# thanhndv212/figaroh-plus

Measured on AMD Instinct MI355X. Metric: samples/sec regressor build + TSQR solve, UR10 6-DoF, higher is better.
Workload: dtype f64

## Files before the change

### figaroh_plus_amd/_lib.py

```python
from __future__ import annotations

import ctypes as C
import os

import numpy as np

_HERE = os.path.dirname(os.path.abspath(__file__))
LIB_PATH = os.environ.get("FIGH_LIB_PATH") or os.path.join(_HERE, "libfigh.so")

ABI_VERSION = 113

FIGH_OK = 0
ERR_INVALID, ERR_NO_DEVICE, ERR_ALLOC, ERR_UNSUPPORTED, ERR_COMM = -1, -2, -3, -4, -5

MODE_JOINT_TORQUE, MODE_EXT_WRENCH = 0, 1
FLAG_FRICTION, FLAG_ACT_INERTIA, FLAG_OFFSET, FLAG_TX40, FLAG_GENERIC, FLAG_BLOCKED_INPUTS = 1, 2, 4, 8, 256, 512
FLAG_COMPACT_BLOCKS = 2048
FLAG_FORCE_COMPACT = 8192
FLAG_LINK_COMPACT = 4096
FLAG_ZEROS_PRESENT = 1024

_c_double_p = C.POINTER(C.c_double)
_c_int32_p = C.POINTER(C.c_int32)

SIGNATURES = {
    "figh_version": (C.c_int, []),
    "figh_last_error": (C.c_char_p, []),
    "figh_device_count": (C.c_int, [C.POINTER(C.c_int)]),
    "figh_device_set": (C.c_int, [C.c_int]),
    "figh_host_wait_mode": (C.c_int, [C.c_int]),
    "figh_tsqr_null_pivot_tol": (C.c_int, [C.c_double]),
    "figh_device_pci_bus_id": (C.c_int, [C.c_int, C.c_char_p, C.c_int]),
    "figh_device_info": (C.c_int, [C.c_char_p, C.c_int, C.POINTER(C.c_int), C.POINTER(C.c_size_t)]),
    "figh_malloc": (C.c_int, [C.POINTER(C.c_void_p), C.c_size_t]),
    "figh_free": (C.c_int, [C.c_void_p]),
    "figh_memcpy_h2d": (C.c_int, [C.c_void_p, C.c_void_p, C.c_size_t]),
    "figh_memcpy_d2h": (C.c_int, [C.c_void_p, C.c_void_p, C.c_size_t]),
    "figh_host_alloc": (C.c_int, [C.POINTER(C.c_void_p), C.c_size_t]),
    "figh_host_free": (C.c_int, [C.c_void_p]),
    "figh_memcpy_d2d": (C.c_int, [C.c_void_p, C.c_void_p, C.c_size_t]),
    "figh_memset": (C.c_int, [C.c_void_p, C.c_int, C.c_size_t]),
    "figh_synchronize": (C.c_int, []),
    "figh_profile_enable": (C.c_int, [C.c_int]),
    "figh_profile_reset": (C.c_int, []),
    "figh_profile_get": (C.c_int, [C.c_char_p, C.POINTER(C.c_int), _c_double_p]),
    "figh_model_create": (C.c_int, [C.c_int, _c_int32_p, _c_int32_p, _c_double_p, _c_double_p, _c_int32_p,
                                    _c_int32_p, _c_double_p, _c_int32_p, C.POINTER(C.c_void_p)]),
    "figh_model_destroy": (C.c_int, [C.c_void_p]),
    "figh_regressor_shape": (C.c_int, [C.c_void_p, C.c_int, C.c_int, C.POINTER(C.c_int), C.POINTER(C.c_int)]),
    "figh_regressor_build": (C.c_int, [C.c_void_p, C.c_int, C.c_int, C.c_int, C.c_int64, C.c_void_p, C.c_void_p,
                                       C.c_void_p, C.c_void_p, C.c_int64, C.c_void_p]),
    "figh_regressor_build_padded": (C.c_int, [C.c_void_p, C.c_int, C.c_int, C.c_int, C.c_int64, C.c_void_p, C.c_void_p,
                                              C.c_void_p, C.c_void_p, C.c_int64, C.c_void_p]),
    "figh_regressor_apply": (C.c_int, [C.c_void_p, C.c_int, C.c_int, C.c_int, C.c_int64, C.c_void_p, C.c_void_p, C.c_void_p,
                                       C.c_void_p, C.c_void_p]),
    "figh_repack_samples": (C.c_int, [C.c_void_p, C.c_int64, C.c_int, C.c_void_p]),
    "figh_coupling_tx40": (C.c_int, [C.c_int64, C.c_int, C.c_void_p, C.c_void_p, C.c_void_p]),
    "figh_colsq": (C.c_int, [C.c_void_p, C.c_int64, C.c_int, C.c_int64, C.c_void_p]),
    "figh_gather_cols": (C.c_int, [C.c_void_p, C.c_int64, C.c_int64, C.c_void_p, C.c_int, C.c_void_p, C.c_int64]),
    "figh_place_block": (C.c_int, [C.c_void_p, C.c_int64, C.c_int64, C.c_int64, C.c_double, C.c_void_p, C.c_int64]),
    "figh_matvec": (C.c_int, [C.c_void_p, C.c_int64, C.c_int64, C.c_void_p, C.c_int, C.c_void_p, C.c_void_p]),
    "figh_block_sqnorm": (C.c_int, [C.c_void_p, C.c_void_p, C.c_int64, C.c_int, C.c_void_p]),
    "figh_tsqr": (C.c_int, [C.c_void_p, C.c_int64, C.c_int64, C.c_void_p, C.c_int, C.c_void_p, _c_double_p, C.c_int,
                            C.c_void_p]),
    "figh_tsqr_structured": (C.c_int, [C.c_void_p, C.c_int64, C.c_int64, C.c_void_p, C.c_int, C.c_void_p, _c_double_p,
                                       C.c_int, _c_int32_p, C.c_int, C.c_void_p]),
    "figh_tsqr_merge": (C.c_int, [C.c_void_p, C.c_int, C.c_int, C.c_void_p]),
    "figh_select_columns": (C.c_int, [C.c_void_p, C.c_int, C.c_double, C.c_int, C.c_void_p]),
    "figh_tsqr_selected_wrench": (C.c_int, [C.c_void_p, C.c_int64, C.c_int64, C.c_void_p, C.c_int, C.c_double, C.c_int,
                                            C.c_int, C.c_int, C.c_void_p, C.c_double, C.c_void_p, C.c_void_p, C.c_void_p,
                                            C.c_int64]),
    "figh_regressor_force_layout": (C.c_int, [C.c_void_p, C.c_int, C.c_int, C.c_int, C.POINTER(C.c_int64)]),
    "figh_model_set_active_rows": (C.c_int, [C.c_void_p, _c_int32_p, C.c_int]),
    "figh_regressor_link_layout": (C.c_int, [C.c_void_p, C.c_int, C.c_int, C.c_int, _c_int32_p, C.POINTER(C.c_int)]),
    "figh_tsqr_selected_blocks": (C.c_int, [C.c_void_p, C.c_int64, C.c_int64, C.c_void_p, C.c_int, C.c_double, C.c_int,
                                            C.c_int, C.c_int, C.c_void_p, C.c_void_p, C.c_void_p, C.c_void_p, C.c_void_p,
                                            C.c_void_p, C.c_double, C.c_void_p, C.c_void_p, C.c_void_p]),
    "figh_block_rows_residuals": (C.c_int, [C.c_void_p, C.c_int, _c_int32_p, C.c_int, C.c_void_p, C.c_void_p]),
    "figh_tsqr_selected": (C.c_int, [C.c_void_p, C.c_int64, C.c_int64, C.c_void_p, C.c_int, C.c_double, C.c_int, C.c_int,
                                     C.c_int, C.c_void_p, C.c_double, C.c_void_p, C.c_void_p]),
    "figh_regressor_tsqr_fused": (C.c_int, [C.c_void_p, C.c_int, C.c_int64, C.c_void_p, C.c_void_p, C.c_void_p, C.c_void_p,
                                            C.c_int64, C.c_void_p, C.c_void_p, C.c_int, C.c_void_p, C.c_double,
                                            C.c_void_p]),
    "figh_chain_host_tail": (C.c_int, [C.c_void_p]),
    "figh_chain_pass_fused": (C.c_int, [C.c_void_p, C.c_int, C.c_int64, C.c_void_p, C.c_void_p, C.c_void_p, C.c_void_p,
                                        C.c_int64, C.c_void_p, C.c_int, C.c_void_p, C.c_double, C.c_double, C.c_void_p,
                                        C.c_void_p, C.c_size_t, C.c_void_p, C.POINTER(C.c_int), C.c_void_p]),
    "figh_tsqr_merge_base": (C.c_int, [C.c_void_p, C.c_int, C.c_int, C.c_int, C.c_double, C.c_void_p]),
    "figh_compact_rows": (C.c_int, [C.c_void_p, C.c_int64, C.c_int, C.c_int64, C.c_void_p, C.c_int, C.c_double, C.c_void_p,
                                    C.c_int64, C.c_void_p, C.POINTER(C.c_int64)]),
    "figh_base_permutation": (C.c_int, [C.c_void_p, C.c_int, C.c_int, C.c_double, C.c_void_p]),
    "figh_regressor_colsq": (C.c_int, [C.c_void_p, C.c_int, C.c_int, C.c_int, C.c_int64, C.c_void_p, C.c_void_p,
                                       C.c_void_p, C.c_int64, C.c_void_p]),
    "figh_regressor_tsqr": (C.c_int, [C.c_void_p, C.c_int, C.c_int, C.c_int, C.c_int64, C.c_void_p, C.c_void_p,
                                      C.c_void_p, C.c_void_p, C.c_int, C.c_void_p, _c_double_p, C.c_int, C.c_int64,
                                      C.c_void_p]),
    "figh_regressor_tsqr_norms": (C.c_int, [C.c_void_p, C.c_int, C.c_int, C.c_int, C.c_int64, C.c_void_p, C.c_void_p,
                                            C.c_void_p, C.c_void_p, C.c_int, C.c_void_p, _c_double_p, C.c_int, C.c_int64,
                                            C.c_void_p, C.c_void_p]),
    "figh_regressor_tsqr_batch": (C.c_int, [C.c_void_p, C.c_int, C.c_int, C.c_int, C.c_int64, C.c_int64, C.c_void_p,
                                            C.c_void_p, C.c_void_p, C.c_void_p, C.c_int, C.c_void_p, C.c_void_p]),
    "figh_regressor_tsqr_batch_fused": (C.c_int, [C.c_void_p, C.c_int, C.c_int64, C.c_int64, C.c_void_p, C.c_void_p,
                                                  C.c_void_p, C.c_void_p, C.c_int, C.c_void_p, C.c_void_p]),
    "figh_regressor_gram": (C.c_int, [C.c_void_p, C.c_int, C.c_int, C.c_int, C.c_int64, C.c_void_p, C.c_void_p,
                                      C.c_void_p, C.c_void_p, C.c_int, C.c_void_p, C.c_int64, _c_double_p, _c_double_p,
                                      _c_double_p]),
    "figh_filtfilt_cols": (C.c_int, [C.c_void_p, C.c_int64, C.c_int, C.c_int64, C.c_int, C.c_int, _c_double_p, _c_double_p,
                                     C.c_int, C.c_int, _c_double_p, C.c_int, C.c_int, C.c_void_p, C.c_int64,
                                     C.POINTER(C.c_int64)]),
    "figh_medfilt_cols": (C.c_int, [C.c_void_p, C.c_int64, C.c_int, C.c_int64, C.c_int, C.c_int, C.c_void_p, C.c_int64]),
    "figh_joint_difference": (C.c_int, [C.c_void_p, C.c_int64, C.c_void_p, C.c_double, C.c_void_p, C.c_void_p]),
    "figh_gradient_cols": (C.c_int, [C.c_void_p, C.c_int64, C.c_int, C.c_int64, C.c_int, C.c_double, C.c_void_p, C.c_void_p,
                                     C.c_int64]),
    "figh_spline_sample": (C.c_int, [C.c_void_p, C.c_int64, C.c_int, C.c_int, C.c_int64, C.c_double, _c_int32_p, _c_int32_p,
                                     _c_double_p, C.c_void_p, C.c_void_p, C.c_int64, C.c_void_p, C.c_int64, C.c_void_p,
                                     C.c_void_p, C.c_int64, C.c_void_p, C.c_void_p, C.c_int64]),
    "figh_excitation_constraints": (C.c_int, [C.c_void_p, C.c_int64, C.c_int64, C.c_int, _c_int32_p, _c_int32_p, C.c_int,
                                              _c_int32_p, C.c_void_p, C.c_int64, C.c_void_p, C.c_int64, C.c_void_p,
                                              C.c_void_p, C.c_int64]),
    "figh_kinematic_regressor": (C.c_int, [C.c_void_p, C.c_int64, C.c_void_p, C.c_int64, C.c_int, _c_double_p, C.c_int,
                                           _c_double_p, _c_int32_p, C.c_int, C.c_int, C.c_void_p, C.c_int64, C.c_void_p,
                                           C.c_int64, C.c_void_p, C.c_void_p]),
    "figh_calib_fkm_batch": (C.c_int, [C.c_void_p, C.c_int64, C.c_int64, C.c_void_p, C.c_int64, C.c_int, _c_int32_p,
                                       C.c_void_p, C.c_void_p, C.c_void_p, C.c_int, _c_double_p, C.c_int, _c_double_p,
                                       C.c_int, C.c_void_p, C.c_int64]),
    "figh_gather_rows": (C.c_int, [C.c_void_p, C.c_int64, C.c_int, C.c_void_p, C.c_int64, C.c_void_p, C.c_int64]),
    "figh_design_gram": (C.c_int, [C.c_void_p, C.c_int64, C.c_int64, C.c_int, C.c_int, C.c_void_p, _c_double_p]),
    "figh_design_scores": (C.c_int, [C.c_void_p, C.c_int64, C.c_int64, C.c_int, C.c_int, _c_double_p, C.c_void_p, C.c_void_p,
                                     C.c_void_p]),
    "figh_comm_available": (C.c_int, []),
    "figh_comm_unique_id": (C.c_int, [C.c_void_p]),
    "figh_comm_init": (C.c_int, [C.c_int, C.c_int, C.c_void_p]),
    "figh_comm_destroy": (C.c_int, []),
    "figh_comm_allgather": (C.c_int, [C.c_void_p, C.c_void_p, C.c_int64]),
    "figh_comm_allreduce_sum": (C.c_int, [C.c_void_p, C.c_int64]),
}


class FighError(RuntimeError):
    def __init__(self, code, msg):
        super().__init__("libfigh error %d: %s" % (code, msg))
        self.code = code


_lib = None


def load():
    global _lib
    if _lib is None:
        if not os.path.exists(LIB_PATH):
            raise ImportError(
                "libfigh.so not found at %s -- build the HIP extension first "
                "(python -c 'import __graft_entry__ as g; g.build()'); there is no CPU fallback" % LIB_PATH)
        lib = C.CDLL(LIB_PATH)
        for name, (res, args) in SIGNATURES.items():
            fn = getattr(lib, name)
            fn.restype = res
            fn.argtypes = args
        have = lib.figh_version()
        if have != ABI_VERSION:
            raise ImportError("%s implements ABI %d, this package is written against %d (include/figh.h FIGH_ABI_VERSION): "
                              "rebuild it (make -C figaroh_plus_amd/csrc)" % (LIB_PATH, have, ABI_VERSION))
        _lib = lib
    return _lib


def check(rc):
    if rc != FIGH_OK:
        msg = load().figh_last_error()
        raise FighError(rc, msg.decode() if msg else "")
    return rc


def device_count():
    n = C.c_int(0)
    check(load().figh_device_count(C.byref(n)))
    return n.value


def device_info():
    name = C.create_string_buffer(256)
    cus = C.c_int(0)
    mem = C.c_size_t(0)
    check(load().figh_device_info(name, 256, C.byref(cus), C.byref(mem)))
    return {"name": name.value.decode(), "cu_count": cus.value, "hbm_bytes": mem.value}


def synchronize():
    check(load().figh_synchronize())


class DeviceArray:

    def __init__(self, shape, dtype=np.float64):
        self.shape = (shape,) if np.isscalar(shape) else tuple(int(s) for s in shape)
        self.dtype = np.dtype(dtype)
        self.size = int(np.prod(self.shape)) if len(self.shape) else 1
        self.nbytes = self.size * self.dtype.itemsize
        p = C.c_void_p()
        check(load().figh_malloc(C.byref(p), max(self.nbytes, 8)))
        self.ptr = p.value

    @classmethod
    def from_host(cls, arr, dtype=None):
        arr = np.ascontiguousarray(arr, dtype=dtype if dtype is not None else arr.dtype)
        d = cls(arr.shape, arr.dtype)
        if arr.nbytes:
            check(load().figh_memcpy_h2d(d.ptr, arr.ctypes.data, arr.nbytes))
        return d

    def to_host(self, out=None):
        if out is None:
            out = np.empty(self.shape, dtype=self.dtype)
        assert out.nbytes == self.nbytes and out.flags["C_CONTIGUOUS"]
        if self.nbytes:
            check(load().figh_memcpy_d2h(out.ctypes.data, self.ptr, self.nbytes))
        return out

    def zero_(self):
        check(load().figh_memset(self.ptr, 0, self.nbytes))
        return self

    def free(self):
        if getattr(self, "ptr", None):
            load().figh_free(self.ptr)
            self.ptr = None

    def __del__(self):
        try:
            self.free()
        except Exception:
            pass


_null_tol = 0.0


def tsqr_null_pivot_tol(tol):
    global _null_tol
    check(load().figh_tsqr_null_pivot_tol(float(tol)))
    prev, _null_tol = _null_tol, float(tol)
    return prev


class null_pivots:

    def __init__(self, tol_qr):
        self.tol = None if tol_qr is None else max(float(tol_qr), 0.0) / 64.0

    def __enter__(self):
        self.prev = None if self.tol is None else tsqr_null_pivot_tol(self.tol)
        return self

    def __exit__(self, *exc):
        if self.prev is not None:
            tsqr_null_pivot_tol(self.prev)
        return False


def profile_enable(on=True, level=2):
    check(load().figh_profile_enable(int(level) if on else 0))


def profile_reset():
    check(load().figh_profile_reset())


def profile_get(name):
    n = C.c_int(0)
    ms = C.c_double(0.0)
    check(load().figh_profile_get(name.encode(), C.byref(n), C.byref(ms)))
    return n.value, ms.value


def _i32(a):
    return np.ascontiguousarray(a, dtype=np.int32)


def _f64(a):
    return np.ascontiguousarray(a, dtype=np.float64)


class ModelHandle:

    def __init__(self, flat):
        n = int(flat["njoints"])
        self.njoints, self.nq, self.nv = n, int(flat["nq"]), int(flat["nv"])
        parents, jtype = _i32(flat["parents"]), _i32(flat["jtype"])
        idx_q, idx_v = _i32(flat["idx_q"]), _i32(flat["idx_v"])
        axis, placement, gravity = _f64(flat["axis"]), _f64(flat["placement"]), _f64(flat["gravity"])
        body_mask = _i32(np.asarray(flat["mass"], dtype=float) != 0.0)
        h = C.c_void_p()
        check(load().figh_model_create(
            n, parents.ctypes.data_as(_c_int32_p), jtype.ctypes.data_as(_c_int32_p),
            axis.ctypes.data_as(_c_double_p), placement.ctypes.data_as(_c_double_p),
            idx_q.ctypes.data_as(_c_int32_p), idx_v.ctypes.data_as(_c_int32_p),
            gravity.ctypes.data_as(_c_double_p), body_mask.ctypes.data_as(_c_int32_p), C.byref(h)))
        self.handle = h.value
        self._chain = n - 1 <= 8 and all(int(jtype[i]) == 0 and int(parents[i]) == i - 1 for i in range(1, n))

    def is_chain(self):
        return self._chain

    def set_active_rows(self, rows=None):
        if rows is None or len(rows) == 0:
            check(load().figh_model_set_active_rows(self.handle, None, 0))
        else:
            arr = np.ascontiguousarray(rows, dtype=np.int32)
            check(load().figh_model_set_active_rows(self.handle, arr.ctypes.data_as(_c_int32_p), len(arr)))

    def shape(self, mode, flags):
        r, c = C.c_int(0), C.c_int(0)
        check(load().figh_regressor_shape(self.handle, mode, flags, C.byref(r), C.byref(c)))
        return r.value, c.value

    def destroy(self):
        if getattr(self, "handle", None):
            load().figh_model_destroy(self.handle)
            self.handle = None

    def __del__(self):
        try:
            self.destroy()
        except Exception:
            pass


def regressor_build(model, mode, flags, ft_mask, N, d_q, d_v, d_a, d_W, ldw, d_colsq=None):
    check(load().figh_regressor_build(model.handle, mode, flags, ft_mask, N, d_q.ptr, d_v.ptr, d_a.ptr, d_W.ptr, ldw,
                                      d_colsq.ptr if d_colsq is not None else None))


def regressor_build_padded(model, mode, flags, ft_mask, N, d_q, d_v, d_a, d_W, ldw, d_colsq=None):
    check(load().figh_regressor_build_padded(model.handle, mode, flags, ft_mask, N, d_q.ptr, d_v.ptr, d_a.ptr,
                                             d_W.ptr if d_W is not None else None, ldw,
                                             d_colsq.ptr if d_colsq is not None else None))


APPLY_WAVES_PER_CU = 8


def regressor_apply_waves(N):
    return max(1, min((int(N) + 63) // 64, APPLY_WAVES_PER_CU * device_info()["cu_count"]))


def regressor_apply(model, mode, flags, ft_mask, N, d_q, d_v, d_a, d_phi, d_tau):
    rc = load().figh_regressor_apply(model.handle if model is not None else None, mode, flags, ft_mask, N, d_q.ptr, d_v.ptr,
                                     d_a.ptr, d_phi.ptr, d_tau.ptr)
    if rc == ERR_UNSUPPORTED:
        return False
    check(rc)
    return True


def coupling_tx40(N, nv, d_v, d_a, d_out):
    check(load().figh_coupling_tx40(N, nv, d_v.ptr, d_a.ptr, d_out.ptr))


def colsq(d_W, rows, cols, ldw, d_out):
    check(load().figh_colsq(d_W.ptr, rows, cols, ldw, d_out.ptr))


def gather_cols(d_W, rows, ldw, d_idx, n, d_out, ldo):
    check(load().figh_gather_cols(d_W.ptr, rows, ldw, d_idx.ptr, n, d_out.ptr, ldo))


def place_block(src_ptr, ld_src, rows, cols, scale, dst_ptr, ld_dst):
    check(load().figh_place_block(src_ptr, ld_src, rows, cols, scale, dst_ptr, ld_dst))


def matvec(d_W, rows, ldw, d_idx, n, d_x, d_y):
    check(load().figh_matvec(d_W.ptr, rows, ldw, d_idx.ptr if d_idx is not None else None, n, d_x.ptr, d_y.ptr))


def block_sqnorm(d_a, d_b, rows, nblocks, d_out):
    check(load().figh_block_sqnorm(d_a.ptr, d_b.ptr if d_b is not None else None, rows, nblocks, d_out.ptr))


def tsqr(d_W, rows, ldw, d_idx, n, d_tau, block_weight, d_R, first_cols=None):
    bw = None
    nb = 0
    if block_weight is not None:
        bwa = _f64(block_weight)
        bw = bwa.ctypes.data_as(_c_double_p)
        nb = len(bwa)
    if first_cols is not None:
        fc = _i32(first_cols)
        check(load().figh_tsqr_structured(d_W.ptr, rows, ldw, d_idx.ptr if d_idx is not None else None, n,
                                          d_tau.ptr if d_tau is not None else None, bw, nb,
# ... 15 lines not shown
        bwa = _f64(block_weight)
        bw, nb = bwa.ctypes.data_as(_c_double_p), len(bwa)
    args = (model.handle, mode, flags, ft_mask, N, d_q.ptr, d_v.ptr, d_a.ptr, d_idx.ptr if d_idx is not None else None, n,
            d_tau.ptr if d_tau is not None else None, bw, nb, chunk_samples, d_R.ptr)
    if d_colsq is not None:
        check(load().figh_regressor_tsqr_norms(*args, d_colsq.ptr))
    else:
        check(load().figh_regressor_tsqr(*args))


class PinnedArray:

    def __init__(self, n):
        self._ptr = C.c_void_p()
        check(load().figh_host_alloc(C.byref(self._ptr), 8 * int(n)))
        self.size = int(n)
        self.array = np.ctypeslib.as_array(C.cast(self._ptr, C.POINTER(C.c_double)), shape=(self.size,))

    def free(self):
        if self._ptr:
            self.array = None
            check(load().figh_host_free(self._ptr))
            self._ptr = C.c_void_p()

    def __del__(self):
        try:
            self.free()
        except Exception:
            pass


def regressor_tsqr_batch(model, mode, flags, ft_mask, B, n_per, d_q, d_v, d_a, d_idx, n, d_R_stack, d_R):
    check(load().figh_regressor_tsqr_batch(model.handle, mode, flags, ft_mask, B, n_per, d_q.ptr, d_v.ptr, d_a.ptr,
                                           d_idx.ptr if d_idx is not None else None, n,
                                           d_R_stack.ptr if d_R_stack is not None else None, d_R.ptr))


def regressor_tsqr_batch_fused(model, flags, B, n_per, d_q, d_v, d_a, d_idx, n, d_R_stack, d_R):
    rc = load().figh_regressor_tsqr_batch_fused(model.handle, flags, B, n_per, d_q.ptr, d_v.ptr, d_a.ptr, d_idx.ptr, n,
                                                d_R_stack.ptr if d_R_stack is not None else None, d_R.ptr)
    if rc == ERR_UNSUPPORTED:
        return False
    check(rc)
    return True


def regressor_gram(model, mode, flags, ft_mask, N, d_q, d_v, d_a, d_idx, n, d_tau=None, chunk_samples=0):
    G = np.empty((n, n))
    g = np.empty(n) if d_tau is not None else None
    tt = C.c_double(0.0)
    check(load().figh_regressor_gram(model.handle, mode, flags, ft_mask, N, d_q.ptr, d_v.ptr, d_a.ptr,
                                     d_idx.ptr if d_idx is not None else None, n,
                                     d_tau.ptr if d_tau is not None else None, chunk_samples,
                                     G.ctypes.data_as(_c_double_p),
                                     g.ctypes.data_as(_c_double_p) if g is not None else None,
                                     C.byref(tt) if d_tau is not None else None))
    return G, g, (tt.value if d_tau is not None else None)


def filtfilt_cols(d_X, rows, cols, ldx, nblocks, form, b, a, zi, padlen, q, d_Y, ldy):
    b, a, zi = _f64(b), _f64(a), _f64(zi)
    nsec = b.shape[0] if form == 0 else 1
    order = 2 if form == 0 else b.size - 1
    out = C.c_int64(0)
    check(load().figh_filtfilt_cols(d_X.ptr, rows, cols, ldx, nblocks, form, b.ctypes.data_as(_c_double_p),
                                    a.ctypes.data_as(_c_double_p), nsec, order, zi.ctypes.data_as(_c_double_p), padlen, q,
                                    d_Y.ptr, ldy, C.byref(out)))
    return out.value


def medfilt_cols(X_ptr, rows, cols, ldx, nblocks, kernel_size, Y_ptr, ldy):
    check(load().figh_medfilt_cols(X_ptr, rows, cols, ldx, nblocks, kernel_size, Y_ptr, ldy))


def joint_difference_tile(nq, nv):
    per_row = 8 * ((nq | 1) + (nv | 1))
    return 64 * min(4, (65536 - 8 * (nq | 1)) // (64 * per_row))


def joint_difference(model, N, q_ptr, ts, dt_ptr, dq_ptr):
    check(load().figh_joint_difference(model.handle, N, q_ptr, float(ts), dt_ptr, dq_ptr))


def gradient_cols(F_ptr, rows, cols, ld, ncols_active, h, h_ptr, G_ptr, ldg):
    check(load().figh_gradient_cols(F_ptr, rows, cols, ld, ncols_active, float(h), h_ptr, G_ptr, ldg))


def spline_sample(model, B, n_wps, n_per, freq, act_idxq, act_idxv, tps, d_wps, d_vel_wps, vel_stride, d_acc_wps, acc_stride,
                  d_q0, q_ptr, ldq, v_ptr, a_ptr, ldv):
    iq, iv, tps = _i32(act_idxq), _i32(act_idxv), _f64(tps).reshape(-1)
    if len(tps) != n_wps or len(iv) != len(iq) or d_wps.size < B * len(iq) * n_wps or d_q0.size < model.nq:
        raise ValueError("spline_sample: %d time points, %d / %d active indices and %d waypoint entries for B = %d, n_wps = %d"
                         % (len(tps), len(iq), len(iv), d_wps.size, B, n_wps))
    for d, stride in ((d_vel_wps, vel_stride), (d_acc_wps, acc_stride)):
        if d.size < (B - 1) * stride + len(iq) * n_wps:
            raise ValueError("spline_sample: a velocity / acceleration waypoint buffer is shorter than its stride asks for")
    check(load().figh_spline_sample(model.handle, B, n_wps, len(iq), n_per, float(freq), iq.ctypes.data_as(_c_int32_p),
                                    iv.ctypes.data_as(_c_int32_p), tps.ctypes.data_as(_c_double_p), d_wps.ptr, d_vel_wps.ptr,
                                    vel_stride, d_acc_wps.ptr, acc_stride, d_q0.ptr, q_ptr, ldq, v_ptr, a_ptr, ldv))


def excitation_constraints(model, B, n_per, act_idxq, act_idxv, idx_waypoints, q_ptr, ldq, v_ptr, ldv, d_tau, out_ptr, ld_out):
    iq, iv, iw = _i32(act_idxq), _i32(act_idxv), _i32(idx_waypoints).reshape(-1)
    if len(iv) != len(iq) or d_tau.size < model.nv * B * n_per:
        raise ValueError("excitation_constraints: %d / %d active indices, tau of %d entries for %d x %d samples of %d efforts"
                         % (len(iq), len(iv), d_tau.size, B, n_per, model.nv))
    check(load().figh_excitation_constraints(model.handle, B, n_per, len(iq), iq.ctypes.data_as(_c_int32_p),
                                             iv.ctypes.data_as(_c_int32_p), len(iw), iw.ctypes.data_as(_c_int32_p), q_ptr, ldq,
                                             v_ptr, ldv, d_tau.ptr, out_ptr, ld_out))


def _ptr(x):
    return x.ptr if hasattr(x, "ptr") else x


def kinematic_regressor(model, N, q_ptr, ldq, end_joint, end_placement, start_joint, start_placement, support, meas_mask,
                        R_ptr, ldr, J_ptr, ldj, rowsq_R_ptr=None, rowsq_J_ptr=None):
    ep = _f64(end_placement).reshape(-1)
    sp = _f64(start_placement).reshape(-1) if start_placement is not None else None
    sup = _i32(support).reshape(-1)
    if ep.size != 12 or (sp is not None and sp.size != 12):
        raise ValueError("kinematic_regressor: a placement is 12 doubles (rotation row-major, translation)")
    check(load().figh_kinematic_regressor(model.handle, N, _ptr(q_ptr), ldq, int(end_joint), ep.ctypes.data_as(_c_double_p),
                                          int(start_joint), sp.ctypes.data_as(_c_double_p) if sp is not None else None,
                                          sup.ctypes.data_as(_c_int32_p), len(sup), int(meas_mask), _ptr(R_ptr), ldr,
                                          _ptr(J_ptr), ldj, _ptr(rowsq_R_ptr), _ptr(rowsq_J_ptr)))


def calib_fkm_batch(model, B, N, q_ptr, ldq, chain, d_placements, d_wMo, d_eeMf, end_joint, end_placement, start_joint,
                    start_placement, meas_mask, out_ptr, ld_out):
    ep = _f64(end_placement).reshape(-1)
    sp = _f64(start_placement).reshape(-1) if start_placement is not None else None
    ch = _i32(chain).reshape(-1)
    if ep.size != 12 or (sp is not None and sp.size != 12):
        raise ValueError("calib_fkm_batch: a placement is 12 doubles (rotation row-major, translation)")
    if d_placements.size < B * len(ch) * 12 or d_wMo.size < 12 * B or d_eeMf.size < 12 * B:
        raise ValueError("calib_fkm_batch: placements / wMo / eeMf hold fewer than B x n_chain x 12 / B x 12 doubles")
    check(load().figh_calib_fkm_batch(model.handle, B, N, _ptr(q_ptr), ldq, len(ch), ch.ctypes.data_as(_c_int32_p),
                                      d_placements.ptr, d_wMo.ptr, d_eeMf.ptr, int(end_joint),
                                      ep.ctypes.data_as(_c_double_p), int(start_joint),
                                      sp.ctypes.data_as(_c_double_p) if sp is not None else None, int(meas_mask),
                                      _ptr(out_ptr), ld_out))


def gather_rows(W_ptr, ldw, cols, d_idx, n, out_ptr, ld_out):
    if d_idx.size < n:
        raise ValueError("gather_rows: %d indices for n = %d" % (d_idx.size, n))
    check(load().figh_gather_rows(_ptr(W_ptr), ldw, cols, d_idx.ptr, n, _ptr(out_ptr), ld_out))


def design_gram(R_ptr, ldr, N, c, n, w_ptr=None):
    M = np.empty((max(int(n), 0), max(int(n), 0)))
    check(load().figh_design_gram(_ptr(R_ptr), ldr, N, c, n, _ptr(w_ptr), M.ctypes.data_as(_c_double_p)))
    return M


def design_scores(R_ptr, ldr, N, c, n, L, trace_ptr, det_add_ptr, det_rm_ptr):
    L = _f64(L)
    if L.shape != (n, n):
        raise ValueError("design_scores: L is %r, expected (%d, %d)" % (L.shape, n, n))
    check(load().figh_design_scores(_ptr(R_ptr), ldr, N, c, n, L.ctypes.data_as(_c_double_p), _ptr(trace_ptr),
                                    _ptr(det_add_ptr), _ptr(det_rm_ptr)))


def compact_rows(W_ptr, rows, cols, ldw, tau_ptr, key_col, threshold, Wout_ptr, ld_out, tauout_ptr):
    out = C.c_int64(0)
    check(load().figh_compact_rows(W_ptr, rows, cols, ldw, tau_ptr, key_col, threshold, Wout_ptr, ld_out, tauout_ptr,
                                   C.byref(out)))
    return out.value


def base_permutation(d_R, nc, n, tol_qr, d_perm):
    check(load().figh_base_permutation(d_R.ptr, nc, n, tol_qr, d_perm.ptr))


def tsqr_merge(d_Rs, count, nc, d_R):
    check(load().figh_tsqr_merge(d_Rs.ptr, count, nc, d_R.ptr))


def select_columns(d_colsq, ncols, tol_e, link_stride, d_sel):
    check(load().figh_select_columns(d_colsq.ptr, ncols, tol_e, link_stride, d_sel.ptr))


def tsqr_selected(d_W, rows, ldw, d_colsq, ncols, tol_e, link_stride, nblocks, n_expected, d_tau, tol_qr, d_sel, d_R):
    check(load().figh_tsqr_selected(d_W.ptr, rows, ldw, d_colsq.ptr, ncols, tol_e, link_stride, nblocks, n_expected,
                                    d_tau.ptr if d_tau is not None else None, tol_qr, d_sel.ptr,
                                    d_R.ptr if d_R is not None else None))


def tsqr_selected_wrench(d_W, rows, ldw, d_colsq, ncols, tol_e, link_stride, n_expected, nf_expected, d_tau, tol_qr, d_sel,
                         d_R, d_link_pos=None, ld_force=0):
    check(load().figh_tsqr_selected_wrench(d_W.ptr, rows, ldw, d_colsq.ptr, ncols, tol_e, link_stride, n_expected,
                                           nf_expected, d_tau.ptr if d_tau is not None else None, tol_qr, d_sel.ptr,
                                           d_R.ptr if d_R is not None else None,
                                           d_link_pos.ptr if d_link_pos is not None else None, int(ld_force)))


def regressor_force_layout(model, mode, flags, ft_mask):
    ldf = C.c_int64(0)
    rc = load().figh_regressor_force_layout(model.handle, mode, flags, ft_mask, C.byref(ldf))
    if rc == ERR_UNSUPPORTED:
        return 0
    check(rc)
    return int(ldf.value)


def regressor_link_layout(model, mode, flags, ft_mask):
    nlinks = model.njoints - 1
    pos = np.zeros(nlinks, dtype=np.int32)
    nlive = C.c_int(0)
    rc = load().figh_regressor_link_layout(model.handle, mode, flags, ft_mask, pos.ctypes.data_as(_c_int32_p), C.byref(nlive))
    if rc == ERR_UNSUPPORTED:
        return None
    check(rc)
    return pos, int(nlive.value)


def tsqr_selected_blocks(d_W, rows, ldw, d_colsq, ncols, tol_e, link_stride, n_expected, counts, d_cols, d_pos, d_tau,
                         tol_qr, d_sel, d_R, block_off=None, block_ld=None, d_block_tri=None):
    counts = np.ascontiguousarray(counts, dtype=np.int32)
    off = ld = None
    if block_off is not None:
        off = np.ascontiguousarray(block_off, dtype=np.int64)
        ld = np.ascontiguousarray(block_ld, dtype=np.int32)
    check(load().figh_tsqr_selected_blocks(d_W.ptr, rows, ldw, d_colsq.ptr, ncols, tol_e, link_stride, n_expected,
                                           len(counts), counts.ctypes.data, d_cols.ptr, d_pos.ptr,
                                           off.ctypes.data if off is not None else None,
                                           ld.ctypes.data if ld is not None else None,
                                           d_tau.ptr if d_tau is not None else None, tol_qr, d_sel.ptr, d_R.ptr,
                                           d_block_tri.ptr if d_block_tri is not None else None))


def block_rows_residuals(d_rows, row_off, nc, d_v, d_r2):
    ro = _i32(row_off)
    check(load().figh_block_rows_residuals(d_rows.ptr, len(ro) - 1, ro.ctypes.data_as(_c_int32_p), nc, d_v.ptr, d_r2.ptr))


def regressor_tsqr_fused(model, flags, N, d_q, d_v, d_a, d_W, ldw, d_colsq, d_kept, n, d_tau, tol_qr, d_R):
    rc = load().figh_regressor_tsqr_fused(model.handle, flags, N, d_q.ptr, d_v.ptr, d_a.ptr, d_W.ptr, ldw, d_colsq.ptr,
                                          d_kept.ptr, n, d_tau.ptr if d_tau is not None else None, tol_qr, d_R.ptr)
    if rc == ERR_UNSUPPORTED:
        return False
    check(rc)
    return True


TAIL_OK, TAIL_SINGULAR = 0, 1


class _HostTailStruct(C.Structure):
    _fields_ = [("rows_k", C.c_void_p), ("n", C.c_int32), ("with_tau", C.c_int32), ("tol_qr", C.c_double),
                ("total_rows", C.c_int64), ("pieces", C.c_int64), ("null_rule", C.c_int32), ("n_cached_base", C.c_int32),
                ("cached_base", C.c_void_p), ("bounds", C.c_void_p), ("idx", C.c_void_p), ("absdiag", C.c_void_p),
                ("beta", C.c_void_p), ("phi_ls", C.c_void_p), ("phi_b", C.c_void_p), ("residual_norm", C.c_double),
                ("n_base", C.c_int32), ("status", C.c_int32), ("certified", C.c_int32), ("bounds_recomputed", C.c_int32)]


class HostTail:

    def __init__(self, n, with_tau):
        self.n, self.with_tau = int(n), bool(with_tau)
        self.idx = np.zeros(self.n, dtype=np.int32)
        self.cached_base = np.zeros(self.n, dtype=np.int32)
        self.absdiag, self.phi_ls, self.phi_b = np.zeros(self.n), np.zeros(self.n), np.zeros(self.n)
        self.beta = np.zeros(self.n * self.n)
        self.bounds = np.zeros(self.n + 2)
        self.cache_of = None
        s = self.s = _HostTailStruct()
        s.n, s.with_tau, s.n_cached_base = self.n, int(self.with_tau), -1
        for name in ("cached_base", "bounds", "idx", "absdiag", "beta", "phi_ls", "phi_b"):
            setattr(s, name, getattr(self, name).ctypes.data)
        self.ref = C.addressof(s)

    def keep_bounds(self, owner):
        r = self.s.n_base
        self.cached_base[:r] = self.idx[:r]
        self.s.n_cached_base = r
        self.cache_of = owner

    def bounds_tuple(self):
        if self.bounds[self.n + 1] == 0.0:
            return None
        r = self.s.n_base
        return self.bounds[:r].copy(), self.bounds[r:self.n].copy(), float(self.bounds[self.n])


def chain_host_tail(tail, rows_k):
    tail.s.rows_k = rows_k.ctypes.data
    check(load().figh_chain_host_tail(tail.ref))


def chain_pass_fused(model, flags, N, d_q, d_v, d_a, d_W, ldw, d_kept, n, d_tau, tol_qr, tol_e, d_pack, h_pack, pack_bytes,
                     kept_mask_u8, tail):
    changed = C.c_int(0)
    rc = load().figh_chain_pass_fused(model.handle, flags, N, d_q.ptr, d_v.ptr, d_a.ptr, d_W.ptr, ldw, d_kept.ptr, n,
                                      d_tau.ptr if d_tau is not None else None, tol_qr, tol_e, d_pack.ptr, h_pack, pack_bytes,
                                      kept_mask_u8.ctypes.data, C.byref(changed), tail.ref)
    if rc == ERR_UNSUPPORTED:
        return None
    check(rc)
    return not changed.value


def tsqr_merge_base(d_Rs, count, nc, n_free, tol_qr, d_Rk):
    check(load().figh_tsqr_merge_base(d_Rs.ptr, count, nc, n_free, tol_qr, d_Rk.ptr))


def repack_samples(d_src, N, width):
    d_dst = DeviceArray((((N + 63) // 64) * 64 * width,), np.float64)
    check(load().figh_repack_samples(d_src.ptr, N, width, d_dst.ptr))
    return d_dst
```

### figaroh_plus_amd/csrc/figh_fused.hip

```cpp
#include <algorithm>
#include <cmath>
#include <cstdlib>
#include <string>
#include <type_traits>

#include "figh_internal.h"
#include "figh_spatial.h"
#include "figh_chain.h"
#include "figh_wave.h"
#include "figh_tsqr_narrow.h"

namespace figh {

typedef double f64x2 __attribute__((ext_vector_type(2)));

struct FusedCtrl {
    int produced;
    int taken;
    int claimed;
    int pad[5];
};

__device__ __forceinline__ int lds_peek(const int *p) {
    return __hip_atomic_load(p, __ATOMIC_RELAXED, __HIP_MEMORY_SCOPE_WORKGROUP);
}
__device__ __forceinline__ void lds_post(int *p, int v) {
    asm volatile("" ::: "memory");
    __hip_atomic_store(p, v, __ATOMIC_RELAXED, __HIP_MEMORY_SCOPE_WORKGROUP);
    asm volatile("" ::: "memory");
}

__device__ __forceinline__ double opaque_s(double x) {
    asm volatile("" : "+s"(x));
    return x;
}

__device__ __forceinline__ double opaque_v(double x) {
    asm volatile("" : "+v"(x));
    return x;
}

template <int NJ>
constexpr int fused_row_of(int jo) { return (jo & 1) ? NJ - 1 - (jo >> 1) : (jo >> 1); }

template <int NJ>
struct FusedGeom {
    static constexpr int NC = 14 * NJ;
    static constexpr int LDT = NC + 2;
    static constexpr int CH = NC / 2;
    static constexpr int NPROD = 2;
    static constexpr int TILE = 64 * LDT;
    static constexpr int TAU0 = TILE;
    static constexpr int QD0 = TAU0 + 64 * NJ;
    static constexpr int CS0 = QD0 + 2 * 64 * NJ;
    static constexpr int CTRL0 = CS0 + ((NC + 7) / 8) * 8;
    static constexpr int PSIZE = CTRL0 + (int)(sizeof(FusedCtrl) / sizeof(double));
    static constexpr int CONS0 = NPROD * PSIZE;
};

template <int NJ, bool TRAJ = false>
__global__ __launch_bounds__(512) void fused_chain_tsqr_kernel(
    const ChainParams<NJ> P, const int flags, const long N, const double *__restrict__ q, const double *__restrict__ v,
    const double *__restrict__ a, double *__restrict__ W, const double *__restrict__ tau, const int *__restrict__ col_idx,
    const int n, const int nc, double *__restrict__ colsq_part, double *__restrict__ Rws, const int ncons,
    const int tri_doubles, const double null2) {
    using G = FusedGeom<NJ>;
    constexpr int NC = G::NC, LDT = G::LDT, CH = G::CH;
    constexpr int NCC = 4, NRC = 4, RPL = 16;
    extern __shared__ __attribute__((aligned(16))) double lds[];
    const int lane = threadIdx.x & 63;
    const int wave = __builtin_amdgcn_readfirstlane((int)(threadIdx.x >> 6));
    const long ntiles_s = (N + 63) / 64;
    const long b = blockIdx.x, Gd = gridDim.x;
    long wg = b;
    if constexpr (TRAJ) {
        const long first = (long)blockIdx.y * N * NJ;
        q += first;
        v += first;
        a += first;
        wg = (long)blockIdx.y * Gd + b;
    }
    const long count_s = b < ntiles_s ? (ntiles_s - b + Gd - 1) / Gd : 0;
    const int T0 = (int)(((count_s + 1) / 2) * NJ), T1 = (int)((count_s / 2) * NJ);

    for (int pz = 0; pz < G::NPROD; ++pz)
        for (int e = pz * G::PSIZE + G::CS0 + threadIdx.x; e < (pz + 1) * G::PSIZE; e += blockDim.x) lds[e] = 0.0;
    for (int e = G::CONS0 + threadIdx.x; e < G::CONS0 + ncons * tri_doubles; e += blockDim.x) lds[e] = 0.0;
    __syncthreads();

    if (wave < G::NPROD) {
        __builtin_amdgcn_s_setprio(3);
        const bool fric = flags & FIGH_FLAG_FRICTION, actin = flags & FIGH_FLAG_ACT_INERTIA, offs = flags & FIGH_FLAG_OFFSET;
        double *tile = lds + wave * G::PSIZE;
        FusedCtrl *ctrl = reinterpret_cast<FusedCtrl *>(tile + G::CTRL0);
        double *my = tile + lane * LDT;
        double *stau = tile + G::TAU0, *sqd = tile + G::QD0, *cacc = tile + G::CS0;
        int t = 0;
        auto sample_tile = [&](auto FAST_T, const long s) {
            constexpr bool FAST = decltype(FAST_T)::value;
            const long i0 = s * 64;
            const int nvalid = FAST ? 64 : (int)((N - i0) < 64 ? (N - i0) : 64);
            const bool live = FAST || lane < nvalid;
            const long is = i0 + (live ? lane : nvalid - 1);
            double cs[NJ], sn[NJ];
            double acc[NJ][3], dw[NJ][3], w[NJ][3];
            {
                double pq[NJ], pqd[NJ], pqdd[NJ];
#pragma unroll
                for (int k = 0; k < NJ; ++k) {
                    pq[k] = q[is * NJ + k];
                    pqd[k] = v[is * NJ + k];
                    pqdd[k] = a[is * NJ + k];
                }
                if (!TRAJ && tau) {
#pragma unroll
                    for (int j = 0; j < NJ; ++j) {
                        const double tv = tau[(long)j * N + is];
                        stau[64 * j + lane] = live ? tv : 0.0;
                    }
                }
#pragma unroll
                for (int k = 0; k < NJ; ++k) {
                    sqd[64 * (2 * k) + lane] = pqd[k];
                    sqd[64 * (2 * k + 1) + lane] = pqdd[k];
                }
                double vl[3] = {0, 0, 0}, om[3] = {0, 0, 0}, da[3] = {0, 0, 0};
                double al[3] = {opaque_v(-P.g[0]), opaque_v(-P.g[1]), opaque_v(-P.g[2])};
#pragma unroll
                for (int k = 0; k < NJ; ++k) {
                    double s_, c_;
                    sincos_angle(pq[k], &s_, &c_);
                    cs[k] = c_;
                    sn[k] = s_;
                    double Rj[9], R[9];
                    const double ax[3] = {opaque_s(P.axis[k][0]), opaque_s(P.axis[k][1]), opaque_s(P.axis[k][2])};
                    rodrigues(ax, c_, s_, Rj);
                    matmul3(P.Rp[k], Rj, R);
                    double t1[3], t2[3], nvl[3], nom[3], nal[3], nda[3];
                    cross3(P.pp[k], om, t1);
#pragma unroll
                    for (int d = 0; d < 3; ++d) t2[d] = vl[d] - t1[d];
                    rotT(R, t2, nvl);
                    rotT(R, om, nom);
                    cross3(P.pp[k], da, t1);
#pragma unroll
                    for (int d = 0; d < 3; ++d) t2[d] = al[d] - t1[d];
                    rotT(R, t2, nal);
                    rotT(R, da, nda);
                    double vj[3] = {P.axis[k][0] * pqd[k], P.axis[k][1] * pqd[k], P.axis[k][2] * pqd[k]};
#pragma unroll
                    for (int d = 0; d < 3; ++d) nom[d] += vj[d];
                    cross3(nvl, vj, t1);
                    cross3(nom, vj, t2);
#pragma unroll
                    for (int d = 0; d < 3; ++d) {
                        nal[d] += t1[d];
                        nda[d] += P.axis[k][d] * pqdd[k] + t2[d];
                        vl[d] = nvl[d];
                        om[d] = nom[d];
                        al[d] = nal[d];
                        da[d] = nda[d];
                    }
                    cross3(om, vl, t1);
#pragma unroll
                    for (int d = 0; d < 3; ++d) {
                        acc[k][d] = al[d] + t1[d];
                        dw[k][d] = da[d];
                        w[k][d] = om[d];
                    }
                }
            }
#pragma unroll
            for (int jo = 0; jo < NJ; ++jo) {
                const int j = fused_row_of<NJ>(jo), jprev = fused_row_of<NJ>(jo == 0 ? NJ - 1 : jo - 1);
                while (lds_peek(&ctrl->taken) < t) __builtin_amdgcn_s_sleep(1);
                asm volatile("" ::: "memory");
                if (j > jprev) {
#pragma unroll
                    for (int c = 14 * jprev; c < 14 * j; c += 2) *reinterpret_cast<f64x2 *>(my + c) = f64x2{0.0, 0.0};
                }
                double Jl[3] = {0, 0, 0}, Ja[3] = {opaque_v(P.axis[j][0]), opaque_v(P.axis[j][1]), opaque_v(P.axis[j][2])};
#pragma unroll
                for (int k = j; k < NJ; ++k) {
                    if (k > j) {
                        asm volatile("" : "+v"(cs[k]), "+v"(sn[k]));
                        double Rj[9], R[9];
                        const double ax[3] = {opaque_s(P.axis[k][0]), opaque_s(P.axis[k][1]), opaque_s(P.axis[k][2])};
                        rodrigues(ax, cs[k], sn[k], Rj);
                        matmul3(P.Rp[k], Rj, R);
                        double t1[3], t2[3], nJl[3], nJa[3];
                        cross3(P.pp[k], Ja, t1);
#pragma unroll
                        for (int d = 0; d < 3; ++d) t2[d] = Jl[d] - t1[d];
                        rotT(R, t2, nJl);
                        rotT(R, Ja, nJa);
#pragma unroll
                        for (int d = 0; d < 3; ++d) {
                            Jl[d] = nJl[d];
                            Ja[d] = nJa[d];
                        }
                    }
                    double o[14];
                    o[9] = Jl[0] * acc[k][0] + Jl[1] * acc[k][1] + Jl[2] * acc[k][2];
                    double h1[3], h2[3], h3[3], h4[3];
                    cross3(Jl, dw[k], h1);
                    cross3(w[k], Jl, h2);
                    cross3(w[k], h2, h3);
                    cross3(acc[k], Ja, h4);
                    o[6] = h1[0] + h3[0] + h4[0];
                    o[7] = h1[1] + h3[1] + h4[1];
                    o[8] = h1[2] + h3[2] + h4[2];
                    double u[3];
                    cross3(w[k], Ja, u);
                    const double *x = dw[k], *z = w[k];
                    o[0] = x[0] * Ja[0] - z[0] * u[0];
                    o[1] = x[1] * Ja[0] + x[0] * Ja[1] - (z[1] * u[0] + z[0] * u[1]);
                    o[3] = x[1] * Ja[1] - z[1] * u[1];
                    o[2] = x[2] * Ja[0] + x[0] * Ja[2] - (z[2] * u[0] + z[0] * u[2]);
                    o[4] = x[2] * Ja[1] + x[1] * Ja[2] - (z[2] * u[1] + z[1] * u[2]);
                    o[5] = x[2] * Ja[2] - z[2] * u[2];
                    if (k == j) {
                        const double qdk = sqd[64 * (2 * k) + lane], qddk = sqd[64 * (2 * k + 1) + lane];
                        o[10] = actin ? qddk : 0.0;
                        o[11] = fric ? qdk : 0.0;
                        o[12] = fric ? sgn(qdk) : 0.0;
                        o[13] = offs ? 1.0 : 0.0;
                    } else {
                        o[10] = o[11] = o[12] = o[13] = 0.0;
                    }
                    double *dst = my + 14 * k;
#pragma unroll
                    for (int c = 0; c < 14; ++c) dst[c] = live ? o[c] : 0.0;
                }
                if constexpr (!TRAJ) my[NC] = tau ? stau[64 * j + lane] : 0.0;
                lds_post(&ctrl->produced, t + 1);
                ++t;
                if constexpr (TRAJ) continue;

                double *dstW = W + ((long)j * N + i0) * NC;
                const char *tbase = reinterpret_cast<const char *>(tile);
                if constexpr (FAST) {
                    constexpr int RG = 128 / CH;
                    constexpr int NG = 64 / RG;
                    constexpr int LEFT = 64 - NG * RG;
                    static_assert(CH <= 64 && RG * CH > 64 && 128 - RG * CH <= CH && LEFT <= 1, "R rows per two passes");
                    constexpr int ROWB = LDT * 8;
                    const unsigned sa = lane, sb = lane + 64;
                    const unsigned ra = sa / CH, rb = sb / CH;
                    const unsigned la = ra * ROWB + 16u * (sa - ra * CH);
                    const unsigned lb = rb * ROWB + 16u * (sb - rb * CH);
                    char *gbase = reinterpret_cast<char *>(dstW) + 16 * lane;
                    constexpr int GRP = RG * CH * 16;
                    constexpr int BATCH = NG % 3 == 0 ? 3 : 4;
                    static_assert(NG % BATCH == 0, "row groups per batch");
#pragma unroll
                    for (int g0 = 0; g0 < NG; g0 += BATCH) {
                        f64x2 va[BATCH], vb[BATCH];
#pragma unroll
                        for (int u = 0; u < BATCH; ++u) {
                            va[u] = *reinterpret_cast<const f64x2 *>(tbase + la + (g0 + u) * RG * ROWB);
                            vb[u] = *reinterpret_cast<const f64x2 *>(tbase + lb + (g0 + u) * RG * ROWB);
                        }
#pragma unroll
                        for (int u = 0; u < BATCH; ++u) {
                            *reinterpret_cast<f64x2 *>(gbase + (g0 + u) * GRP) = va[u];
                            if (LEFT > 0 || g0 + u + 1 < NG || sb < (unsigned)(RG * CH))
                                *reinterpret_cast<f64x2 *>(gbase + (g0 + u) * GRP + 1024) = vb[u];
                        }
                    }
                    if constexpr (LEFT > 0) {
                        if (lane < CH) {
                            const f64x2 vc = *reinterpret_cast<const f64x2 *>(tbase + 63 * ROWB + 16 * lane);
                            *reinterpret_cast<f64x2 *>(gbase + NG * GRP) = vc;
                        }
                    }
                } else {
                    constexpr unsigned MAGIC = ((1u << 20) + CH - 1) / CH;
                    static_assert(64 * CH <= 4096, "magic division range");
                    const int total = nvalid * CH;
                    for (int id = lane; id < total; id += 64) {
                        const unsigned r = ((unsigned)id * MAGIC) >> 20;
                        const double2 val = *reinterpret_cast<const double2 *>(tbase + 16u * (id + r));
                        *reinterpret_cast<double2 *>(reinterpret_cast<char *>(dstW) + 16 * id) = val;
                    }
                }
                {
                    const int lo = 14 * j, width = NC - lo;
                    constexpr int RB = NJ >= 6 ? 8 : 16;
                    auto column_sum = [&](const double *col) {
                        double t0 = 0.0, t1 = 0.0, t2 = 0.0, t3 = 0.0;
#pragma unroll
                        for (int r0 = 0; r0 < 64; r0 += RB) {
                            double x[RB];
#pragma unroll
                            for (int r = 0; r < RB; ++r) x[r] = col[(r0 + r) * LDT];
#pragma unroll
                            for (int r = 0; r < RB; ++r) asm volatile("" : "+v"(x[r]));
#pragma unroll
                            for (int r = 0; r < RB; r += 4) {
                                t0 += x[r] * x[r];
                                t1 += x[r + 1] * x[r + 1];
                                t2 += x[r + 2] * x[r + 2];
                                t3 += x[r + 3] * x[r + 3];
                            }
                        }
                        return (t0 + t1) + (t2 + t3);
                    };
                    if (lane < width) cacc[lo + lane] += column_sum(tile + lo + lane);
                    if (width > 64 && lane + 64 < width) cacc[lo + 64 + lane] += column_sum(tile + lo + 64 + lane);
                }
            }
        };
        for (long s = b + wave * Gd; s < ntiles_s; s += G::NPROD * Gd) {
            if ((s + 1) * 64 <= N) sample_tile(std::true_type{}, s);
            else sample_tile(std::false_type{}, s);
        }
        asm volatile("" ::: "memory");
        if constexpr (!TRAJ)
            for (int c = lane; c < NC; c += 64) colsq_part[(b * G::NPROD + wave) * NC + c] = cacc[c];
        return;
    }
    const int c_id = wave - G::NPROD;
    const int pad = 16 * NCC - nc;
    Tsqr2State<NCC, NRC, true> S;
    tsqr2_state_init(S, lds + G::CONS0 + c_id * tri_doubles, lane, nc, null2);
    bool wlive[NCC];
    int loff[NCC];
#pragma unroll
    for (int cc = 0; cc < NCC; ++cc) {
        const int col = 16 * cc + S.lane_c - pad;
        wlive[cc] = col >= 0 && col < nc;
        const int src = (col >= 0 && col < n) ? col_idx[col] : NC;
        loff[cc] = S.lane_g * LDT + src;
    }
    int fpos[NJ];
#pragma unroll
    for (int j = 0; j < NJ; ++j) fpos[j] = pad;
    for (int e = 0; e < n; ++e) {
        const int c = col_idx[e];
#pragma unroll
        for (int j = 1; j < NJ; ++j) fpos[j] += (c < 14 * j) ? 1 : 0;
    }
#pragma unroll
    for (int j = 0; j < NJ; ++j) fpos[j] = __builtin_amdgcn_readfirstlane(fpos[j]);
    FusedCtrl *ctrl0 = reinterpret_cast<FusedCtrl *>(lds + G::CTRL0);
    FusedCtrl *ctrl1 = reinterpret_cast<FusedCtrl *>(lds + G::PSIZE + G::CTRL0);

    int pref = c_id & 1;
    int absorbed = 0;
    for (;;) {
        int pick = -2, tpick = 0;
        while (pick == -2) {
            int res = -2, tres = 0;
            if (lane == 0) {
                bool done = true;
#pragma unroll
                for (int tr = 0; tr < 2; ++tr) {
                    const int pb = pref ^ tr;
                    FusedCtrl *cp = pb ? ctrl1 : ctrl0;
                    const int Tp = pb ? T1 : T0;
                    int cl = lds_peek(&cp->claimed);
                    if (cl < Tp) {
                        done = false;
                        if (res == -2 && lds_peek(&cp->produced) > cl &&
                            __hip_atomic_compare_exchange_strong(&cp->claimed, &cl, cl + 1, __ATOMIC_RELAXED, __ATOMIC_RELAXED,
                                                                 __HIP_MEMORY_SCOPE_WORKGROUP)) {
                            res = pb;
                            tres = cl;
                        }
                    }
                }
                if (done) res = -1;
            }
            pick = __builtin_amdgcn_readfirstlane(res);
            tpick = __builtin_amdgcn_readfirstlane(tres);
            if (pick == -2) __builtin_amdgcn_s_sleep(1);
        }
        if (pick < 0) break;
        pref = pick ^ 1;
        asm volatile("" ::: "memory");
        const double *tile = lds + pick * G::PSIZE;
        FusedCtrl *ctrl = pick ? ctrl1 : ctrl0;
        const int jrow = fused_row_of<NJ>(tpick % NJ);
        int first_nz = fpos[0];
#pragma unroll
        for (int j = 1; j < NJ; ++j) first_nz = jrow == j ? fpos[j] : first_nz;
        first_nz = __builtin_amdgcn_readfirstlane(first_nz);
#pragma unroll
        for (int cc = 0; cc < NCC; ++cc) {
#pragma unroll
            for (int i = 0; i < RPL; ++i) S.T[cc][i] = 0.0;
            if (wlive[cc] && 16 * cc + 15 >= first_nz) {
#pragma unroll
                for (int i = 0; i < RPL; ++i) S.T[cc][i] = tile[(16 * (i >> 2) + 4 * (i & 3)) * LDT + loff[cc]];
            }
        }
#pragma unroll
        for (int cc = 0; cc < NCC; ++cc)
#pragma unroll
            for (int i = 0; i < RPL; ++i) asm volatile("" : "+v"(S.T[cc][i]));
        lds_post(&ctrl->taken, tpick + 1);
        S.null2 = tsqr2_null2_at(absorbed, 64, nc, null2);
        ++absorbed;
        tsqr2_panels<0, NCC, NRC, false, true>(S, first_nz, [](auto) {});
    }
    tsqr2_store_triangle(S, Rws + (wg * ncons + c_id) * (long)nc * nc, nc, pad, lane);
}

__global__ __launch_bounds__(512) void fused_batch_merge_kernel(const double *__restrict__ Rs, const long rows,
                                                                const double *__restrict__ extra, const int nc,
                                                                double *__restrict__ Rout) {
    const double *mine = Rs + (long)blockIdx.y * rows * nc;
    const long rows_all = rows + (extra ? nc : 0);
    double *Rg = Rout + ((long)blockIdx.y * gridDim.x + blockIdx.x) * nc * nc;
    tsqr_coop_factor<4, 8>((long)blockIdx.x, nc, Rg, [&](const long row, const int col) {
        const bool ok = row < rows_all && col >= 0;
        const double *src = row < rows ? mine + row * nc : extra + (row - rows) * nc;
        return ok ? src[col] : 0.0;
    });
}

template <int NJ>
struct FusedPlan {
    ChainParams<NJ> P;
    int tri, ncons;
    size_t lds;
};

template <int NJ, bool TRAJ>
static int fused_plan(const figh_model_s *m, int nc, FusedPlan<NJ> *plan) {
    constexpr size_t fixed = FusedGeom<NJ>::CONS0, budget = (160 * 1024) / sizeof(double);
    const size_t tri = (size_t)tsqr2_tri_doubles(4, nc, true);
    const int ncons = (int)std::min<size_t>(6, (budget - fixed) / tri);
    if (ncons < 3) {
        set_error(std::string(TRAJ ? "fused batch regressor + TSQR" : "fused regressor + TSQR") +
                  ": the triangles of three consumer waves do not fit next to the tile");
        return FIGH_ERR_UNSUPPORTED;
    }
    static bool attr_set = false;
    if (!attr_set) {
        FIGH_HIP(hipFuncSetAttribute(reinterpret_cast<const void *>(&fused_chain_tsqr_kernel<NJ, TRAJ>),
                                     hipFuncAttributeMaxDynamicSharedMemorySize, 160 * 1024));
        attr_set = true;
    }
    plan->P = chain_params<NJ>(m);
    plan->tri = (int)tri;
    plan->ncons = ncons;
    plan->lds = sizeof(double) * (fixed + (size_t)ncons * tri);
    return FIGH_OK;
}

template <int NJ>
static int launch_fused(const figh_model_s *m, int flags, long N, const double *q, const double *v, const double *a,
                        double *W, const double *tau, const int *d_kept, int n, double *d_colsq, double **Rws_out,
                        long *count_out) {
    using G = FusedGeom<NJ>;
    const int nc = n + (tau ? 1 : 0);
    FusedPlan<NJ> pl;
    if (int rc = fused_plan<NJ, false>(m, nc, &pl)) return rc;
    const int cus = cu_count(), ncons = pl.ncons;
    const long ntiles_s = (N + 63) / 64;
    long grid = cus < ntiles_s / 2 ? cus : ntiles_s / 2;
    double *part = static_cast<double *>(workspace(sizeof(double) * grid * G::NPROD * G::NC, kWsRegressorNorms));
    double *Rws = static_cast<double *>(workspace(sizeof(double) * (size_t)nc * nc * (grid * ncons + 1), kWsLevel0TriOrWrench));
    if (!part || !Rws) return FIGH_ERR_ALLOC;
    {
        ProfileScope scope("fused_chain_tsqr", true);
        FIGH_LAUNCH_TIMED((fused_chain_tsqr_kernel<NJ, false>), dim3((unsigned)grid), dim3(64 * (G::NPROD + ncons)), pl.lds,
                          pl.P, flags, N, q, v, a, W, tau, d_kept, n, nc, part, Rws, ncons, pl.tri, null_pivot_sq());
    }
    launch_reduce_partials(part, (int)(grid * G::NPROD), G::NC, d_colsq);
    FIGH_HIP(hipGetLastError());
    *Rws_out = Rws;
    *count_out = grid * ncons;
    return FIGH_OK;
}

static long fused_batch_slices(long B, long n_per, int cus) {
    const long tiles = (n_per + 63) / 64;
    return std::max(1L, std::min(tiles, (long)cus / B));
}

template <int NJ>
static int launch_fused_batch(const figh_model_s *m, int flags, long B, long n_per, const double *q, const double *v,
                              const double *a, const int *d_cols, int n, const double *d_R_stack, double *d_R_out) {
    using G = FusedGeom<NJ>;
    const int nc = n;
    FusedPlan<NJ> pl;
    if (int rc = fused_plan<NJ, true>(m, nc, &pl)) return rc;
    const int ncons = pl.ncons;
    const long S = fused_batch_slices(B, n_per, cu_count());
    const size_t tsz = sizeof(double) * (size_t)nc * nc;
    double *Rws = static_cast<double *>(workspace(tsz * (size_t)(B * S * ncons), kWsFusedBatchTri));
    if (!Rws) return FIGH_ERR_ALLOC;
    {
        ProfileScope scope("fused_chain_tsqr_batch", true);
        FIGH_LAUNCH_TIMED((fused_chain_tsqr_kernel<NJ, true>), dim3((unsigned)S, (unsigned)B), dim3(64 * (G::NPROD + ncons)),
                          pl.lds, pl.P, flags, n_per, q, v, a, (double *)nullptr, (const double *)nullptr, d_cols, n, nc,
                          (double *)nullptr, Rws, ncons, pl.tri, null_pivot_sq());
    }
    FIGH_HIP(hipGetLastError());
    const double *cur = Rws, *extra = d_R_stack;
    long cnt = S * ncons;
    WorkspaceSlot slot = kWsMergeA;
    for (;;) {
        ProfileScope scope("tsqr_reduce");
        const long rows = cnt * nc;
        const long nb = (rows + (extra ? nc : 0) + 511) / 512;
        double *dst = nb == 1 ? d_R_out : static_cast<double *>(workspace(tsz * (size_t)(B * nb), slot));
        if (!dst) return FIGH_ERR_ALLOC;
        hipLaunchKernelGGL(fused_batch_merge_kernel, dim3((unsigned)nb, (unsigned)B), dim3(512), 0, stream(), cur, rows, extra,
                           nc, dst);
        FIGH_HIP(hipGetLastError());
        if (nb == 1) return FIGH_OK;
        cur = dst;
        cnt = nb;
        extra = nullptr;
        slot = slot == kWsMergeA ? kWsMergeB : kWsMergeA;
    }
}

}

using namespace figh;

static int fused_pass_launch(figh_model_t model, int flags, int64_t N, const double *d_q, const double *d_v, const double *d_a,
                             double *d_W, int64_t ldw, double *d_colsq, const int32_t *d_kept, int n, const double *d_tau,
                             double **Rws, long *count) {
    FIGH_REQUIRE(N >= 0 && n >= 1, "bad shape");
    const DevModel &h = model->host;
    const int nc = n + (d_tau ? 1 : 0);
    const int ncols = 14 * h.nlinks;
    if (!model->is_chain || (flags & (FIGH_FLAG_TX40 | FIGH_FLAG_GENERIC | FIGH_FLAG_BLOCKED_INPUTS)) || ldw != ncols ||
        (reinterpret_cast<uintptr_t>(d_W) % 16) != 0 || nc > 64 || n > ncols || N < 4096) {
        set_error("fused regressor + TSQR: serial chain, joint-torque mode, packed 16-byte aligned W, at most 64 columns "
                  "(tau included) and at least 4096 samples");
        return FIGH_ERR_UNSUPPORTED;
    }
    if (int rc = ensure_device()) return rc;
    const int f = flags & 7;
    switch (h.nlinks) {
        case 5:
            return launch_fused<5>(model, f, (long)N, d_q, d_v, d_a, d_W, d_tau, d_kept, n, d_colsq, Rws, count);
        case 6:
            return launch_fused<6>(model, f, (long)N, d_q, d_v, d_a, d_W, d_tau, d_kept, n, d_colsq, Rws, count);
        case 7:
            return launch_fused<7>(model, f, (long)N, d_q, d_v, d_a, d_W, d_tau, d_kept, n, d_colsq, Rws, count);
        default:
            set_error("fused regressor + TSQR: serial chains of 5 to 7 joints (LDS: two tile buffers + three consumer triangles)");
            return FIGH_ERR_UNSUPPORTED;
    }
}

extern "C" int figh_regressor_tsqr_fused(figh_model_t model, int flags, int64_t N, const double *d_q, const double *d_v,
                                         const double *d_a, double *d_W, int64_t ldw, double *d_colsq,
                                         const int32_t *d_kept, int n, const double *d_tau, double tol_qr,
                                         double *d_R_out) {
    FIGH_REQUIRE(model && d_q && d_v && d_a && d_W && d_colsq && d_kept && d_R_out, "NULL pointer");
    double *Rws = nullptr;
    long count = 0;
    if (int rc = fused_pass_launch(model, flags, N, d_q, d_v, d_a, d_W, ldw, d_colsq, d_kept, n, d_tau, &Rws, &count))
        return rc;
    return tsqr_reduce_stack(Rws, count, n + (d_tau ? 1 : 0), n, tol_qr, d_R_out);
}

extern "C" int figh_chain_pass_fused(figh_model_t model, int flags, int64_t N, const double *d_q, const double *d_v,
                                     const double *d_a, double *d_W, int64_t ldw, const int32_t *d_kept, int n,
                                     const double *d_tau, double tol_qr, double tol_e, double *d_pack, double *h_pack,
                                     size_t pack_bytes, const uint8_t *h_kept_mask, int *changed, figh_host_tail_t *tail) {
    FIGH_REQUIRE(model && d_q && d_v && d_a && d_W && d_kept && d_pack && h_pack && h_kept_mask && changed && tail,
                 "NULL pointer");
    FIGH_REQUIRE(tol_qr >= 0.0, "figh_chain_pass_fused: the rank decision needs tol_qr >= 0");
    const int ncols = 14 * model->host.nlinks, nc = n + (d_tau ? 1 : 0);
    const size_t sel_words = (size_t)(2 + 2 * ncols + 1) / 2;
    const size_t words = (size_t)ncols + sel_words + (size_t)(nc > 0 ? (nc + 1) * nc : 0);
    FIGH_REQUIRE(n >= 1 && pack_bytes >= sizeof(double) * words, "figh_chain_pass_fused: the pack is [colsq | sel | rows]");
    FIGH_REQUIRE(tail->n == n && (tail->with_tau != 0) == (d_tau != nullptr), "figh_chain_pass_fused: tail of another shape");
    double *d_colsq = d_pack, *d_rows = d_pack + ncols + sel_words;
    int32_t *d_sel = reinterpret_cast<int32_t *>(d_pack + ncols);
    double *Rws = nullptr;
    long count = 0;
    if (int rc = fused_pass_launch(model, flags, N, d_q, d_v, d_a, d_W, ldw, d_colsq, d_kept, n, d_tau, &Rws, &count)) return rc;
    if (int rc = tsqr_reduce_stack(Rws, count, nc, n, tol_qr, d_rows)) return rc;
    if (int rc = figh_select_columns(d_colsq, ncols, tol_e, 14, d_sel)) return rc;
    FIGH_HIP(hipMemcpyAsync(h_pack, d_pack, sizeof(double) * words, hipMemcpyDeviceToHost, stream()));
    FIGH_HIP(hipStreamSynchronize(stream()));
    const int32_t *mask_now = reinterpret_cast<const int32_t *>(h_pack + ncols) + 2 + ncols;
    *changed = 0;
    for (int c = 0; c < ncols; ++c)
        if ((mask_now[c] != 0) != (h_kept_mask[c] != 0)) {
            *changed = 1;
            return FIGH_OK;
        }
    tail->rows_k = h_pack + ncols + sel_words;
    return figh_chain_host_tail(tail);
}

static constexpr int64_t kFusedBatchMinSamples = 64;

extern "C" int figh_regressor_tsqr_batch_fused(figh_model_t model, int flags, int64_t B, int64_t n_per, const double *d_q,
                                               const double *d_v, const double *d_a, const int32_t *d_col_idx, int n,
                                               const double *d_R_stack, double *d_R_out) {
    FIGH_REQUIRE(model && d_q && d_v && d_a && d_col_idx && d_R_out, "NULL pointer");
    FIGH_REQUIRE(B >= 1 && n_per >= 1 && n >= 1, "figh_regressor_tsqr_batch_fused: at least one trajectory, sample and column");
    const DevModel &h = model->host;
    if (!model->is_chain || h.nlinks < 5 || h.nlinks > 7) {
        set_error("fused batch regressor + TSQR: serial chains of 5 to 7 joints (LDS: two tile buffers + three consumer triangles)");
        return FIGH_ERR_UNSUPPORTED;
    }
    if (flags & (FIGH_FLAG_TX40 | FIGH_FLAG_GENERIC | FIGH_FLAG_BLOCKED_INPUTS)) {
        set_error("fused batch regressor + TSQR: joint-torque mode of the chain kernel only (no TX40 coupling, generic kernel or "
                  "tile-blocked inputs)");
        return FIGH_ERR_UNSUPPORTED;
    }
    if (n > 64) {
        set_error("fused batch regressor + TSQR: at most 64 columns");
        return FIGH_ERR_UNSUPPORTED;
    }
    if (n_per < kFusedBatchMinSamples) {
        set_error("fused batch regressor + TSQR: at least 64 samples (one full sample tile) per trajectory");
        return FIGH_ERR_UNSUPPORTED;
    }
    if (B > 65535) {
        set_error("fused batch regressor + TSQR: at most 65535 trajectories (one grid row each)");
        return FIGH_ERR_UNSUPPORTED;
    }
    if (int rc = ensure_device()) return rc;
    const int f = flags & 7;
    switch (h.nlinks) {
        case 5:
            return launch_fused_batch<5>(model, f, (long)B, (long)n_per, d_q, d_v, d_a, d_col_idx, n, d_R_stack, d_R_out);
        case 6:
            return launch_fused_batch<6>(model, f, (long)B, (long)n_per, d_q, d_v, d_a, d_col_idx, n, d_R_stack, d_R_out);
        case 7:
            return launch_fused_batch<7>(model, f, (long)B, (long)n_per, d_q, d_v, d_a, d_col_idx, n, d_R_stack, d_R_out);
        default:
            return FIGH_ERR_UNSUPPORTED;
    }
}
```

### figaroh_plus_amd/csrc/figh_host_tail.hip

```cpp
#include <cmath>
#include <cstring>

#include "figh_internal.h"

namespace figh {

static constexpr int kTailMax = 80;
static constexpr double kNullRuleFold = 64.0;

static inline double round6(double x) { return std::nearbyint(x * 1e6) / 1e6; }

static inline double tail_triangles(int64_t rows, int64_t pieces) {
    const int64_t t = (rows + 31) / 32 + (pieces > 1 ? pieces : 1);
    return (double)(t > 1 ? t : 1);
}

int host_tail(figh_host_tail_t *t) {
    FIGH_REQUIRE(t && t->rows_k && t->idx && t->absdiag && t->beta && t->phi_ls && t->phi_b && t->bounds,
                 "figh_chain_host_tail: NULL pointer");
    const int n = t->n, with_tau = t->with_tau ? 1 : 0, nc = n + with_tau;
    FIGH_REQUIRE(n >= 1 && n <= kTailMax, "figh_chain_host_tail: 1 .. 80 columns");
    FIGH_REQUIRE(t->n_cached_base < 0 || t->cached_base, "figh_chain_host_tail: cached bounds without their base columns");
    const double *rows = t->rows_k, *diag = rows + (size_t)nc * nc;
    const double tol = t->tol_qr;
    int base[kTailMax], rest[kTailMax], r = 0, d = 0;
    for (int k = 0; k < n; ++k) {
        const double a = std::fabs(diag[k]);
        t->absdiag[k] = a;
        if (a > tol) base[r++] = k;
        else rest[d++] = k;
    }
    for (int k = 0; k < r; ++k) t->idx[k] = base[k];
    for (int k = 0; k < d; ++k) t->idx[r + k] = rest[k];
    t->n_base = r;
    t->status = FIGH_TAIL_OK;
    t->certified = 0;
    t->bounds_recomputed = 0;
    t->residual_norm = with_tau ? std::fabs(rows[(size_t)n * nc + n]) : 0.0;

    static thread_local double U[kTailMax * kTailMax], X[kTailMax * kTailMax], B[kTailMax * (kTailMax + 1)];
    const int nb = d + with_tau;
    for (int a = 0; a < r; ++a) {
        const double *row = rows + (size_t)base[a] * nc;
        for (int b = a; b < r; ++b) U[a * kTailMax + b] = row[base[b]];
        for (int c = 0; c < d; ++c) B[a * (kTailMax + 1) + c] = row[rest[c]];
        if (with_tau) B[a * (kTailMax + 1) + d] = row[n];
    }
    auto R1 = [&](int a, int b) { return U[a * kTailMax + b]; };
    bool singular = false, finite = true;
    for (int k = 0; k < r; ++k) singular = singular || R1(k, k) == 0.0;
    if (!singular) {
        for (int j = 0; j < r; ++j) {
            double *x = X + (size_t)j * kTailMax;
            x[j] = 1.0 / R1(j, j);
            for (int i = j - 1; i >= 0; --i) {
                const double *u = U + i * kTailMax;
                double s = 0.0;
                for (int k = i + 1; k <= j; ++k) s += u[k] * x[k];
                x[i] = -s / u[i];
            }
            for (int i = 0; i <= j; ++i) finite = finite && std::isfinite(x[i]);
        }
    }
    auto Xe = [&](int i, int j) { return X[(size_t)j * kTailMax + i]; };
    auto product_row = [&](int i, double *out) {
        for (int c = 0; c < nb; ++c) out[c] = 0.0;
        for (int k = i; k < r; ++k) {
            const double x = Xe(i, k);
            const double *b = B + k * (kTailMax + 1);
            for (int c = 0; c < nb; ++c) out[c] += x * b[c];
        }
    };

    double *A_base = t->bounds, *A_dep = t->bounds + r, *xnorm = t->bounds + n, *valid = t->bounds + n + 1;
    if (t->null_rule) {
        bool cached = t->n_cached_base == r;
        for (int k = 0; cached && k < r; ++k) cached = t->cached_base[k] == base[k];
        if (!cached) {
            t->bounds_recomputed = 1;
            if (singular || !finite) {
                *valid = 0.0;
            } else {
                double rowsum[kTailMax];
                for (int i = 0; i < r; ++i) rowsum[i] = 0.0;
                for (int k = 0; k < r; ++k) {
                    double s = 0.0;
                    for (int i = 0; i < k; ++i) s += std::fabs(Xe(i, k));
                    A_base[k] = std::fabs(R1(k, k)) * s;
                    for (int i = 0; i <= k; ++i) rowsum[i] += std::fabs(Xe(i, k));
                }
                double xn = 0.0;
                for (int i = 0; i < r; ++i) xn = rowsum[i] > xn ? rowsum[i] : xn;
                double prod[kTailMax + 1];
                for (int c = 0; c < d; ++c) A_dep[c] = 0.0;
                for (int i = 0; i < r; ++i) {
                    product_row(i, prod);
                    for (int c = 0; c < d; ++c) A_dep[c] += std::fabs(prod[c]);
                }
                *xnorm = r ? xn : 0.0;
                *valid = 1.0;
            }
        }
    }
    if (singular) {
        t->status = FIGH_TAIL_SINGULAR;
        return FIGH_OK;
    }

    for (int i = 0; i < r; ++i) {
        double prod[kTailMax + 1];
        product_row(i, prod);
        for (int c = 0; c < d; ++c) t->beta[(size_t)i * d + c] = round6(prod[c]);
        if (with_tau) {
            t->phi_ls[i] = prod[d];
            t->phi_b[i] = round6(prod[d]);
        }
    }

    if (!t->null_rule) return FIGH_OK;
    if (*valid == 0.0) return FIGH_OK;
    const double fold = 2.0 * tol / kNullRuleFold;
    if (with_tau) {
        double sum = 0.0, mx = 0.0;
        for (int i = 0; i < r; ++i) {
            const double p = std::fabs(t->phi_ls[i]);
            if (!std::isfinite(p)) return FIGH_OK;
            sum += p;
            mx = p > mx ? p : mx;
        }
        if (*xnorm * (tol / kNullRuleFold) * sum > 1e-7 * (mx > 1.0 ? mx : 1.0)) return FIGH_OK;
    }
    for (int k = 0; k < n; ++k)
        if (!std::isfinite(t->absdiag[k])) return FIGH_OK;
    for (int c = 0; c < d; ++c)
        if (t->absdiag[rest[c]] > tol / 8.0) return FIGH_OK;
    const double fold_base = fold * std::sqrt(tail_triangles(t->total_rows, t->pieces));
    for (int k = 0; k < r; ++k)
        if (!(t->absdiag[base[k]] - tol > (1.0 + A_base[k]) * fold_base)) return FIGH_OK;
    for (int c = 0; c < d; ++c)
        if (!(tol - t->absdiag[rest[c]] > (1.0 + A_dep[c]) * fold)) return FIGH_OK;
    t->certified = 1;
    return FIGH_OK;
}

}

extern "C" int figh_chain_host_tail(figh_host_tail_t *t) { return figh::host_tail(t); }
```

### figaroh_plus_amd/csrc/figh_internal.h

```cpp
#pragma once

#include <hip/hip_runtime.h>
#include <hip/hip_ext.h>

#include <cstdint>
#include <cstdio>
#include <string>

#include "figh.h"

namespace figh {

constexpr int kMaxJoints = 64;

struct DevModel {
    int njoints, nq, nv, nlinks;
    int parents[kMaxJoints];
    int jtype[kMaxJoints];
    int idx_q[kMaxJoints];
    int idx_v[kMaxJoints];
    int body_mask[kMaxJoints];
    int depth[kMaxJoints];
    double axis[kMaxJoints][3];
    double placement[kMaxJoints][12];
    double gravity[3];
};

}

struct figh_model_s {
    figh::DevModel host;
    figh::DevModel *dev = nullptr;
    bool is_chain = false;
    int max_depth = 0;
    unsigned long long active_rows = ~0ull;
};

namespace figh {

void set_error(const std::string &msg);
double null_pivot_sq();
hipStream_t stream();
int ensure_device();
int cu_count();

struct ProfileScope {
    explicit ProfileScope(const char *name, bool at_launch = false);
    ~ProfileScope();
    const char *name_;
    hipEvent_t e0_ = nullptr, e1_ = nullptr;
    bool at_launch_ = false;
};
struct LaunchEvents {
    hipEvent_t start = nullptr, stop = nullptr;
};
LaunchEvents take_launch_events();

#define FIGH_LAUNCH_TIMED(kernel, grid, block, lds, ...)                                                        \
    do {                                                                                                        \
        const figh::LaunchEvents ev_ = figh::take_launch_events();                                              \
        hipExtLaunchKernelGGL(kernel, grid, block, lds, figh::stream(), ev_.start, ev_.stop, 0, __VA_ARGS__);    \
    } while (0)

enum WorkspaceSlot {
    kWsRegressorNorms,
    kWsColsqParts,
    kWsMergeA,
    kWsMergeB,
    kWsBlockWeights,
    kWsLevel0TriOrWrench,
    kWsHintFirst,
    kWsChunkW,
    kWsChunkNormsOrCols,
    kWsChunkTau,
    kWsChunkStack,
    kWsGramR,
    kWsWideBlkOrFilter,
    kWsTileHint,
    kWsZeroHint,
    kWsOneTri,
    kWsRevealPerm,
    kWsRevealR,
    kWsSelectedHint,
    kWsBatchPair,
    kWsChunkNormsFused,
    kWsForceCols,
    kWsForceOrBlockTri,
    kWsForceOrBlockR,
    kWsChunkForceStack,
    kWsBlockStack,
    kWsCompactCounts,
    kWsCompactTotal,
    kWsGroupTri,
    kWsGroupJobs,
    kWsGroupZeros,
    kWsStacksA,
    kWsStacksB,
    kWsStacksBlk,
    kWsStacksJobs,
    kWsBlocksWideTri,
    kWsLinkPos,
    kWsBlocksMidTri,
    kWsFusedBatchTri,
    kWsDynamicsState,
    kWsSplineTable,
    kWsConstraintIdx,
    kWsKinematicJacobian,
    kWsDesignPartials,
    kWsDesignGram,
    kWsDesignFactor,
    kWorkspaceSlots
};

inline unsigned capped_grid(const long items, const long per_group, const long cap) {
    const long g = (items + per_group - 1) / per_group;
    return (unsigned)(g < 1 ? 1 : g > cap ? cap : g);
}
inline unsigned capped_grid_rows(const long batch) { return (unsigned)(batch < 65535 ? batch : 65535); }

void *workspace(size_t bytes, WorkspaceSlot slot);

struct SideStream {
    SideStream();
    ~SideStream();
    hipEvent_t finish();
    bool ok() const { return ok_; }
    bool ok_ = false, open_ = false;
    hipStream_t main_ = nullptr;
};
void stream_wait(hipEvent_t ev);

struct Level0Options {
    const int *hint = nullptr;
    long chain_wgs = 0;
    int chain_flags = 0;
};
int tsqr_level0(const double *d_W, int64_t rows, int64_t ldw, const int32_t *d_col_idx, int n, const double *d_tau,
                const double *h_block_weight, int nblocks, double *d_tri_out, int64_t capacity, int64_t *count_out,
                double **ws_out, const Level0Options &opt = {});
int64_t tsqr_level0_capacity(int nc);
int tile_hint(const int32_t *h_first_col, int nfirst, int64_t rows, int n, int nc, const int **out);

void launch_reduce_partials(const double *part, int nblocks, int ncols, double *out);

int launch_regressor_tree(const figh_model_s *m, int mode, int flags, int ft_mask, long N, const double *q,
                          const double *v, const double *a, double *W, long ldw, int ncols, int link_stride,
                          double *d_colsq, int *colsq_done);
void forget_tapes(const figh_model_s *m);
int launch_inverse_dynamics(const figh_model_s *m, int mode, int flags, int ft_mask, long N, const double *q, const double *v,
                            const double *a, const double *phi, double *tau);
int tree_link_positions(const figh_model_s *m, int mode, int flags, int ft_mask, int *pos);
long tree_force_ld(const figh_model_s *m, int mode, int flags, int ft_mask);

long tsqr_wide_workgroups(int nc, int cus);
int launch_tsqr_wide(const double *W, long rows, long ldw, const int *col_idx, int n, const double *tau,
                     const double *d_blkw, long rows_per_blk, int nc, long nwg, double *Rws_out, int chain_flags = 0);
int split_force_columns(const int *d_kept, int n, int link_stride, int *d_fsel, int force_compact = 0);
int embed_force_triangle(const double *d_Rf, int ncf, int nf, const int *d_fpos, int nc, int n, double *d_out);
struct Tsqr2Job {
    const double *W;
    const double *tau;
    const int *col_idx;
    const int *pos;
    double *tri;
    double *lvl[3];
    double *out;
    long rows, ldw;
    int n, nc;
    int wave0, nwaves;
    int wg0[3], nb[3];
    int nlevels;
    int tall;
};
struct WyPairJob {
    const double *stack;
    double *Rblk;
    double *Rout;
    long count;
    int nc;
    int wg0;
};
}
#include <vector>
namespace figh {
struct WyPairStack {
    const double *tri;
    long count;
    int nc;
    double *out;
};
int reduce_wide_stacks(std::vector<WyPairStack> &stacks);
struct GroupEmbed {
    const void *jobs = nullptr;
    int njobs = 0, ncfull = 0, nfull = 0;
};
int launch_tsqr_group(std::vector<Tsqr2Job> &jobs, int ncfull, int nfull, int cus, GroupEmbed *later = nullptr);
int launch_tsqr_group_embed(const GroupEmbed &e);
int tsqr_reduce_stack(const double *d_Rs, long count, int nc, int n_free, double tol_qr, double *d_out);
int launch_tsqr_wide_pairs(const double *stack, long count, int nc, double *Rws_out);
int launch_tsqr_wide_single(const double *W, long rows, long ldw, const int *col_idx, int n, int nc, double *R_out);
int launch_tsqr_wide_batch(const double *W, long ldw, const int *col_idx, int n, int nc, long B, long n_per, int rps,
                           long seg_stride, long wgs, double *Rws_out);
int tsqr_wide_tile_rows(int nc);
int launch_tsqr_wide_chain(const double *W, long rows, long ldw, const int *col_idx, int n, const double *tau,
                           const double *d_blkw, long rows_per_blk, int nc, long nwg, double *Rws_out);

int launch_tsqr_tree(const double *Rs, long count, int nc, int n_free, double tol, double *d_out, double *d_rows_out);

int launch_tsqr_stream(const double *Rs, long count, int nc, int n_free, double tol, double *d_out, double *d_rows_out);

#define FIGH_HIP(expr)                                                                          \
    do {                                                                                        \
        hipError_t _e = (expr);                                                                 \
        if (_e != hipSuccess) {                                                                 \
            figh::set_error(std::string(#expr) + ": " + hipGetErrorString(_e));                 \
            return FIGH_ERR_NO_DEVICE;                                                          \
        }                                                                                       \
    } while (0)

#define FIGH_REQUIRE(cond, msg)              \
    do {                                     \
        if (!(cond)) {                       \
            figh::set_error(msg);            \
            return FIGH_ERR_INVALID;         \
        }                                    \
    } while (0)

}
```

### figaroh_plus_amd/csrc/figh_linalg.hip

```cpp
#include <cstdlib>
#include <algorithm>
#include <cstdio>
#include <type_traits>
#include <vector>

#include "figh_internal.h"
#include "figh_wave.h"
#include "figh_tsqr_narrow.h"
#include "figh_tsqr_narrow_kernel.h"

namespace figh {


template <int NCC, int NRC, bool LDSRED, bool RLAST = false>
__global__ __launch_bounds__(64, (NCC <= 4 || RLAST) ? 2 : 1) void tsqr2_kernel(
    const double *__restrict__ W, const long rows, const long ldw, const int *__restrict__ col_idx, const int n,
    const double *__restrict__ tau, const double *__restrict__ blkw, const long rows_per_blk,
    double *__restrict__ Rws, const int nc, const int *__restrict__ tile_first, const double null2) {
    tsqr2_level0_body<NCC, NRC, LDSRED, RLAST>(W, rows, ldw, col_idx, n, tau, blkw, rows_per_blk, Rws, nc, tile_first,
                                        (long)blockIdx.x, (long)gridDim.x, null2);
}



template <int NCC, int NW>
__global__ __launch_bounds__(64 * NW) void tsqr_coop_kernel(const double *__restrict__ Rs, const long rows, const int nc,
                                                            double *__restrict__ Rout) {
    tsqr_coop_factor<NCC, NW>((long)blockIdx.x, nc, Rout + (long)blockIdx.x * nc * nc, CoopStackRows{Rs, rows, nc});
}


__global__ __launch_bounds__(256) void colsq_kernel(const double *__restrict__ W, long rows, int cols, long ldw,
                                                    long rows_per_block, double *__restrict__ part) {
    const long rb = (long)blockIdx.x * rows_per_block;
    const long re = rb + rows_per_block < rows ? rb + rows_per_block : rows;
    for (int c = threadIdx.x; c < cols; c += blockDim.x) {
        double s0 = 0.0, s1 = 0.0;
        long r = rb;
        for (; r + 1 < re; r += 2) {
            const double x0 = W[r * ldw + c], x1 = W[(r + 1) * ldw + c];
            s0 += x0 * x0;
            s1 += x1 * x1;
        }
        if (r < re) {
            const double x0 = W[r * ldw + c];
            s0 += x0 * x0;
        }
        part[(long)blockIdx.x * cols + c] = s0 + s1;
    }
}

__global__ __launch_bounds__(256) void reduce_partials_kernel(const double *__restrict__ part, int nblocks, int ncols,
                                                              double *__restrict__ out) {
    __shared__ double sm[256];
    const int c = blockIdx.x;
    double s = 0.0;
    for (int b = threadIdx.x; b < nblocks; b += 256) s += part[(long)b * ncols + c];
    sm[threadIdx.x] = s;
    __syncthreads();
    for (int w = 128; w > 0; w >>= 1) {
        if ((int)threadIdx.x < w) sm[threadIdx.x] += sm[threadIdx.x + w];
        __syncthreads();
    }
    if (threadIdx.x == 0) out[c] = sm[0];
}

void launch_reduce_partials(const double *part, int nblocks, int ncols, double *out) {
    hipLaunchKernelGGL(reduce_partials_kernel, dim3(ncols), dim3(256), 0, stream(), part, nblocks, ncols, out);
}

__global__ __launch_bounds__(256) void gather_cols_kernel(const double *__restrict__ W, long rows, long ldw,
                                                          const int *__restrict__ col_idx, int n,
                                                          double *__restrict__ out, long ldo) {
    const long total = rows * n;
    for (long e = (long)blockIdx.x * blockDim.x + threadIdx.x; e < total; e += (long)gridDim.x * blockDim.x) {
        const long r = e / n;
        const int c = (int)(e - r * n);
        out[r * ldo + c] = W[r * ldw + col_idx[c]];
    }
}

__global__ __launch_bounds__(256) void place_block_kernel(const double *__restrict__ src, long lds, long rows, long cols,
                                                          double scale, double *__restrict__ dst, long ldd) {
    const long total = rows * cols;
    for (long e = (long)blockIdx.x * blockDim.x + threadIdx.x; e < total; e += (long)gridDim.x * blockDim.x) {
        const long r = e / cols;
        const long c = e - r * cols;
        dst[r * ldd + c] = scale * src[r * lds + c];
    }
}

__global__ __launch_bounds__(64) void base_permutation_kernel(const double *__restrict__ R, const int nc, const int n,
                                                              const double tol, int *__restrict__ perm) {
    const int lane = threadIdx.x;
    int nbase = 0;
    for (int i0 = 0; i0 < n; i0 += 64) {
        const int i = i0 + lane;
        const bool big = i < n && fabs(R[(long)i * nc + i]) > tol;
        nbase += __popcll(__ballot(big));
    }
    int pb = 0, pr = nbase;
    for (int i0 = 0; i0 < n; i0 += 64) {
        const int i = i0 + lane;
        const bool in = i < n;
        const bool big = in && fabs(R[(long)i * nc + i]) > tol;
        const unsigned long long mb = __ballot(big), mr = __ballot(in && !big);
        const unsigned long long below = (1ull << lane) - 1ull;
        if (big) perm[pb + __popcll(mb & below)] = i;
        else if (in) perm[pr + __popcll(mr & below)] = i;
        pb += __popcll(mb);
        pr += __popcll(mr);
    }
    for (int i = n + lane; i < nc; i += 64) perm[i] = i;
}

__global__ __launch_bounds__(256) void matvec_kernel(const double *__restrict__ W, long rows, long ldw,
                                                     const int *__restrict__ col_idx, int n,
                                                     const double *__restrict__ x, double *__restrict__ y) {
    const int lane = threadIdx.x & 63;
    const long wave = ((long)blockIdx.x * blockDim.x + threadIdx.x) >> 6;
    const long nwaves = ((long)gridDim.x * blockDim.x) >> 6;
    for (long r = wave; r < rows; r += nwaves) {
        double s = 0.0;
        for (int c = lane; c < n; c += 64) s += W[r * ldw + (col_idx ? col_idx[c] : c)] * x[c];
#pragma unroll
        for (int off = 32; off > 0; off >>= 1) s += __shfl_down(s, off, 64);
        if (lane == 0) y[r] = s;
    }
}

__global__ __launch_bounds__(256) void block_sqnorm_kernel(const double *__restrict__ a, const double *__restrict__ b,
                                                           long rows_per_block, double *__restrict__ out) {
    __shared__ double sm[256];
    const long base = (long)blockIdx.x * rows_per_block;
    double s = 0.0;
    for (long r = threadIdx.x; r < rows_per_block; r += 256) {
        const double d = a[base + r] - (b ? b[base + r] : 0.0);
        s += d * d;
    }
    sm[threadIdx.x] = s;
    __syncthreads();
    for (int w = 128; w > 0; w >>= 1) {
        if ((int)threadIdx.x < w) sm[threadIdx.x] += sm[threadIdx.x + w];
        __syncthreads();
    }
    if (threadIdx.x == 0) out[blockIdx.x] = sm[0];
}

__global__ __launch_bounds__(256) void select_columns_kernel(const double *__restrict__ colsq, const int ncols,
                                                             const double tol_e, const int link_stride, const int nblocks,
                                                             const long rows, const long rows_per_block,
                                                             const long ntiles, int *__restrict__ sel,
                                                             int *__restrict__ tile_first,
                                                             const int *__restrict__ link_pos = nullptr) {
    __shared__ int kept[1024];
    __shared__ int first[kMaxJoints];
    const int tid = threadIdx.x;
    for (int c = tid; c < ncols; c += 256) kept[c] = !(colsq[c] < tol_e);
    __syncthreads();
    if (tile_first) {
        for (int b = tid; b < nblocks; b += 256) {
            const int lim = 14 * b < ncols ? 14 * b : ncols;
            int f = 0;
            for (int c = 0; c < lim; ++c) f += kept[c];
            first[b] = f;
        }
        __syncthreads();
        const long t = (long)blockIdx.x * 256 + tid;
        if (t < ntiles) {
            const long r0 = t * 64, r1 = (r0 + 63 < rows ? r0 + 63 : rows - 1);
            int f = first[r0 / rows_per_block];
            for (long b = r0 / rows_per_block + 1; b <= r1 / rows_per_block; ++b) f = min(f, first[b]);
            tile_first[t] = f;
        }
    }
    if (blockIdx.x != 0) return;
    int total = 0;
    for (int c = 0; c < ncols; ++c) total += kept[c];
    for (int c = tid; c < ncols; c += 256) {
        int pos = 0;
        for (int e = 0; e < c; ++e) pos += kept[e];
        if (kept[c]) sel[2 + pos] = (link_pos ? max(link_pos[c / 14], 0) : c / 14) * link_stride + c % 14;
        if (c >= total) sel[2 + c] = 0;
        sel[2 + ncols + c] = kept[c];
    }
    if (tid == 0) {
        sel[0] = total;
        sel[1] = ncols;
    }
}

__global__ __launch_bounds__(256) void split_force_columns_kernel(const int *__restrict__ kept, const int n,
                                                                  const int link_stride, int *__restrict__ fsel,
                                                                  const int force_compact) {
    __shared__ int flag[1024];
    const int tid = threadIdx.x;
    for (int c = tid; c < n; c += 256) flag[c] = (kept[c] % link_stride) >= 6;
    __syncthreads();
    for (int c = tid; c < n; c += 256) {
        if (!flag[c]) continue;
        int pos = 0;
        for (int e = 0; e < c; ++e) pos += flag[e];
        const int p = kept[c] / link_stride, s = kept[c] % link_stride;
        fsel[pos] = force_compact ? 16 * (p >> 2) + 4 * (p & 3) + (s - 6) : kept[c];
        fsel[n + pos] = c;
    }
}

__global__ __launch_bounds__(1024) void embed_force_triangle_kernel(const double *__restrict__ Rf, const int ncf,
                                                                    const int nf, const int *__restrict__ fpos,
                                                                    const int nc, const int n, double *__restrict__ out) {
    for (int e = threadIdx.x; e < nc * nc; e += 1024) out[e] = 0.0;
    __syncthreads();
    for (int e = threadIdx.x; e < ncf * ncf; e += 1024) {
        const int r = e / ncf, c = e - r * ncf;
        if (c < r) continue;
        int col = c < nf ? fpos[c] : n;
        col = col < 0 ? 0 : (col >= nc ? nc - 1 : col);
        out[(long)r * nc + col] = Rf[e];
    }
}

int split_force_columns(const int *d_kept, int n, int link_stride, int *d_fsel, int force_compact) {
    FIGH_HIP(hipMemsetAsync(d_fsel, 0, sizeof(int) * 2 * (size_t)n, stream()));
    hipLaunchKernelGGL(split_force_columns_kernel, dim3(1), dim3(256), 0, stream(), d_kept, n, link_stride, d_fsel, force_compact);
    FIGH_HIP(hipGetLastError());
    return FIGH_OK;
}
int embed_force_triangle(const double *d_Rf, int ncf, int nf, const int *d_fpos, int nc, int n, double *d_out) {
    hipLaunchKernelGGL(embed_force_triangle_kernel, dim3(1), dim3(1024), 0, stream(), d_Rf, ncf, nf, d_fpos, nc, n, d_out);
    FIGH_HIP(hipGetLastError());
    return FIGH_OK;
}

__global__ __launch_bounds__(256) void scatter_regrouped_kernel(const double *__restrict__ R, const double *__restrict__ Rr,
                                                                const int *__restrict__ perm, const int nc, const int n,
                                                                const double tol, double *__restrict__ out) {
    if (blockIdx.x == gridDim.x - 1) {
        if (n != nc - 1) return;
        __shared__ double part[256];
        __shared__ int cnt[256];
        int c = 0;
        for (int k = threadIdx.x; k < n; k += 256) c += fabs(R[(long)k * nc + k]) > tol;
        cnt[threadIdx.x] = c;
        __syncthreads();
        for (int s = 128; s > 0; s >>= 1) {
            if ((int)threadIdx.x < s) cnt[threadIdx.x] += cnt[threadIdx.x + s];
            __syncthreads();
        }
        const int r = cnt[0];
        double ss = 0.0;
        for (int k = r + threadIdx.x; k < nc; k += 256) ss += Rr[(long)k * nc + n] * Rr[(long)k * nc + n];
        part[threadIdx.x] = ss;
        __syncthreads();
        for (int s = 128; s > 0; s >>= 1) {
            if ((int)threadIdx.x < s) part[threadIdx.x] += part[threadIdx.x + s];
            __syncthreads();
        }
        if (threadIdx.x == 0) out[(long)perm[nc - 1] * nc + perm[nc - 1]] = sqrt(part[0]);
        return;
    }
    const int nb = gridDim.x - 1;
    for (int e = blockIdx.x * 256 + threadIdx.x; e < nc * nc; e += nb * 256) {
        const int i = e / nc, j = e - i * nc;
        const int pi = perm[i], pj = perm[j];
        const bool base_row = pi >= n || fabs(R[(long)pi * nc + pi]) > tol;
        const double val = (base_row && j >= i) ? Rr[e] : 0.0;
        if (!(n == nc - 1 && e == nc * nc - 1)) out[(long)pi * nc + pj] = val;
        if (i == 0) out[(long)nc * nc + j] = R[(long)j * nc + j];
    }
}

__global__ __launch_bounds__(256) void compact_count_kernel(const double *__restrict__ W, const long rows, const long ldw,
                                                            const int key_col, const double thr, int *__restrict__ cnt) {
    const long r = (long)blockIdx.x * 256 + threadIdx.x;
    const bool keep = r < rows && fabs(W[r * ldw + key_col]) >= thr;
    const unsigned long long m = __ballot(keep);
    if ((threadIdx.x & 63) == 0) cnt[r >> 6] = __popcll(m);
}
__global__ __launch_bounds__(1024) void compact_scan_kernel(int *__restrict__ cnt, const long ngroups, long *__restrict__ total) {
    __shared__ long part[1024];
    const long per = (ngroups + 1023) / 1024;
    const long lo = threadIdx.x * per, hi = lo + per < ngroups ? lo + per : ngroups;
    long s = 0;
    for (long i = lo; i < hi; ++i) s += cnt[i];
    part[threadIdx.x] = s;
    __syncthreads();
    if (threadIdx.x == 0) {
        long run = 0;
        for (int i = 0; i < 1024; ++i) {
            const long v = part[i];
            part[i] = run;
            run += v;
        }
        *total = run;
    }
    __syncthreads();
    long run = part[threadIdx.x];
    for (long i = lo; i < hi; ++i) {
        const int v = cnt[i];
        cnt[i] = (int)run;
        run += v;
    }
}
__global__ __launch_bounds__(256) void compact_copy_kernel(const double *__restrict__ W, const long rows, const int cols,
                                                           const long ldw, const double *__restrict__ tau, const int key_col,
                                                           const double thr, const int *__restrict__ off,
                                                           double *__restrict__ Wo, const long ldo, double *__restrict__ tauo) {
    const int lane = threadIdx.x & 63;
    const long grp = ((long)blockIdx.x * 256 + threadIdx.x) >> 6;
    const long r = grp * 64 + lane;
    if (grp * 64 >= rows) return;
    const bool keep = r < rows && fabs(W[r * ldw + key_col]) >= thr;
    unsigned long long m = __ballot(keep);
    long dst = off[grp];
    if (keep && tau) tauo[dst + __popcll(m & ((1ull << lane) - 1ull))] = tau[r];
    while (m) {
        const int src = __ffsll((long long)m) - 1;
        m &= m - 1;
        const double *in = W + (grp * 64 + src) * ldw;
        double *out = Wo + dst * ldo;
        for (int c = lane; c < cols; c += 64) out[c] = in[c];
        ++dst;
    }
}

static size_t tsqr2_lds_bytes(int ncc, int nc, bool rlast = false) { return sizeof(double) * tsqr2_tri_doubles(ncc, nc, rlast); }

__global__ __launch_bounds__(256) void tile_hint_kernel(const int *__restrict__ first, const long hint_rows,
                                                        const long rows, const long ntiles, int *__restrict__ out) {
    const long t = (long)blockIdx.x * 256 + threadIdx.x;
    if (t >= ntiles) return;
    const long r0 = t * 64, r1 = (r0 + 63 < rows ? r0 + 63 : rows - 1);
    int f = first[r0 / hint_rows];
    for (long b = r0 / hint_rows + 1; b <= r1 / hint_rows; ++b) f = min(f, first[b]);
    out[t] = f;
}

static const int *zero_tile_hint(long ntiles) {
    static size_t zeroed = 0;
    const size_t need = sizeof(int) * (size_t)(ntiles + 1);
    int *z = static_cast<int *>(workspace(need, kWsZeroHint));
    if (z && zeroed < need) {
        if (hipMemsetAsync(z, 0, need, stream()) != hipSuccess) return nullptr;
        zeroed = need;
    }
    return z;
}

static int tsqr_level(const double *W, long rows, long ldw, const int *col_idx, int n, const double *tau,
                      const double *d_blkw, long rows_per_blk, int nc, long target_wgs, double *Rws_out, long *nw_out,
                      const int *hint, long chain_wgs = 0, int chain_flags = 0) {
    const long ntiles = (rows + 63) / 64;
    long nw = target_wgs < ntiles ? target_wgs : ntiles;
    if (nw < 1) nw = 1;
    if (nc > 80 && chain_wgs > 0) nw = chain_wgs;
    *nw_out = nw;
    if (nc > 80)
        return launch_tsqr_wide(W, rows, ldw, col_idx, n, tau, d_blkw, rows_per_blk, nc, nw, Rws_out,
                                chain_wgs > 0 ? chain_flags : 0);
    if (nw > 8 && nw % 8 == 0) nw -= 1;
    *nw_out = nw;
    const int *th = hint ? hint : zero_tile_hint(ntiles);
    if (!th) return FIGH_ERR_ALLOC;
    dim3 grid((unsigned)nw), block(64);
    const bool tall48 = nc > 64 && !hint && rows >= 6L * nc * cu_count() * 8;
    if (nc <= 64)
        FIGH_LAUNCH_TIMED((tsqr2_kernel<4, 4, true>), grid, block, tsqr2_lds_bytes(4, nc), W, rows, ldw, col_idx, n, tau,
                          d_blkw, rows_per_blk, Rws_out, nc, th, null_pivot_sq());
    else if (!tall48)
        FIGH_LAUNCH_TIMED((tsqr2_kernel<5, 4, false>), grid, block, tsqr2_lds_bytes(5, nc), W, rows, ldw, col_idx, n, tau,
// ... 670 lines not shown
```

### figaroh_plus_amd/pipeline.py

```python
import numpy as np

from . import _lib
from .device import GpuMatrix
from .tools import qrdecomposition as qrd
from .tools.regressor import build_regressor_device


class Exchange:

    world_size = 1
    rank = 0

    @property
    def collective(self):
        return self.world_size > 1

    def sum_columns(self, d_colsq, ncols):
        return d_colsq.to_host()

    def sum_columns_device(self, d_colsq, ncols):
        if self.world_size > 1:
            total = np.ascontiguousarray(self.sum_columns(d_colsq, ncols), dtype=np.float64)
            _lib.check(_lib.load().figh_memcpy_h2d(d_colsq.ptr, total.ctypes.data, total.nbytes))

    def stack_triangles(self, d_R, nc):
        return d_R, 1


class _View:

    def __init__(self, base, byte_offset):
        self.ptr = base.ptr + int(byte_offset)


from ._host import relative_percent as _relative_percent
from ._host import single_threaded_blas as _single_threaded_blas


def _grown(buf, size, alloc):
    return buf if buf is not None and buf.size >= size else alloc(size)


def _dtrtri(R1):
    from scipy.linalg.lapack import dtrtri
    return dtrtri(R1, lower=0)


_dtrsm = None


def _solve_upper(R1, B):
    global _dtrsm
    if _dtrsm is None:
        from scipy.linalg.blas import dtrsm
        _dtrsm = dtrsm
    if R1.shape[0] and not np.diag(R1).all():
        raise np.linalg.LinAlgError("Singular matrix")
    return _dtrsm(1.0, R1, B, side=0, lower=0, trans_a=0, diag=0)


class IdentificationPipeline:

    def __init__(self, robot, param, params_std=None, coupling=False, tol_e=1e-6, tol_qr=qrd.TOL_QR, exchange=None,
                 chunk_samples=None, placement_trials=1, structural_zeros="every-pass", w_layout="dense", fuse=True, null_pivots=True,
                 row_blocks=None, native_tail=True):
        self.chunk_samples = chunk_samples
        self.native_tail = bool(native_tail)
        self.row_blocks = None if row_blocks is None else [int(b) for b in row_blocks]
        self._fuse_requested = bool(fuse)
        self._null_pivots_requested = bool(null_pivots)
        if structural_zeros not in ("every-pass", "once"):
            raise ValueError("structural_zeros must be 'every-pass' or 'once'")
        self.structural_zeros = structural_zeros
        if w_layout not in ("dense", "block-compact", "link-padded", "link-compact"):
            raise ValueError("w_layout must be 'dense', 'block-compact', 'link-padded' or 'link-compact'")
        self.w_layout = w_layout
        self.placement_trials = max(1, int(placement_trials))
        self.robot, self.param, self.coupling = robot, param, coupling
        self.tol_e, self.tol_qr = tol_e, tol_qr
        self.params_std = params_std if params_std is not None else robot.get_standard_parameters(param)
        self.names = list(self.params_std.keys())
        self.exchange = exchange or Exchange()
        self._init_samples()
        self._init_layout()
        self.forget()
        self._init_pass()
        self._host_pack = self._d_kept_buf = self._d_block_tri = self._host_tail = self._own_handle = None
        self._dc_colsq = self._dc_idx = self._dc_R = self._d_tailpack = self._host_tailpack = None
        self._strings_memo = self._force_slot_mask = self._ancestors = None
        self._scratch = {}
        self.fused_passes = self.prefix_passes = self.null_rule_fallbacks = self.strings_memo_hits = 0
        self.placement_report = self._cert_failed = None
        self._no_force_compact = False

    def _init_samples(self, N=0, d_q=None, d_v=None, d_a=None, d_tau=None, in_flags=0, repack_ms=0.0):
        self.N, self.d_q, self.d_v, self.d_a, self.d_tau = N, d_q, d_v, d_a, d_tau
        self._in_flags, self.repack_ms = in_flags, repack_ms
        self.fuse = self._fuse_requested
        self.null_pivots = self._null_pivots_requested
        self._force_compact_ok = False

    def _init_layout(self):
        self.W = self._compact = self._link_pos = self._d_link_pos = None
        self._padded = self._zeros_once = self._wrench_split = self._tree_blocks = False
        self._force_ld = self._sel_words = self._hint_blocks = self._padded_flags = 0
        self._d_pack = self._d_colsq = self._d_sel = self._d_rows = self._d_R = None

    def _init_pass(self):
        self._have_block_tri, self._beta_later, self._cert_args = False, None, None

    def _collective(self):
        ex = self.exchange
        return getattr(ex, "collective", True)

    def _handle(self):
        if self.row_blocks is None:
            return self.robot.device_model()
        if self._own_handle is None:
            m = self.robot.model
            if sorted(set(self.row_blocks)) != sorted(self.row_blocks) or not all(0 <= b < m.nv for b in self.row_blocks):
                raise ValueError("row_blocks must be distinct dof indices in [0, %d)" % m.nv)
            self._own_handle = _lib.ModelHandle(m.to_flat())
            self._own_handle.set_active_rows(self.row_blocks)
        return self._own_handle

    def set_samples(self, q, v, a, tau=None):
        from .tools.regressor import _samples_to_device, regressor_flags
        mode, _, _ = regressor_flags(self.param, self.coupling)
        rps = self.robot.model.nv if mode == _lib.MODE_JOINT_TORQUE else 6
        if self.row_blocks is not None:
            if mode != _lib.MODE_JOINT_TORQUE or self.coupling or self.chunk_samples:
                raise NotImplementedError("row_blocks: joint-torque regressor of a tree, W resident (no chunk_samples)")
            rps_in = len(self.row_blocks)
        else:
            rps_in = rps
        tau_resident = tau is not None and (isinstance(tau, _lib.DeviceArray) or hasattr(tau, "ptr"))
        if tau_resident and self.row_blocks is not None:
            raise NotImplementedError("row_blocks: tau is re-laid per active dof on the host; pass a host array")
        if tau is not None:
            if not tau_resident:
                tau = np.ascontiguousarray(tau, dtype=np.float64).reshape(-1)
            if int(tau.size) != rps_in * len(q):
                raise ValueError("tau must have rows_per_sample * N = %d * %d = %d entries; got %d"
                                 % (rps_in, len(q), rps_in * len(q), int(tau.size)))
            if self.row_blocks is not None:
                full = np.zeros(rps * len(q))
                for i, b in enumerate(self.row_blocks):
                    full[b * len(q):(b + 1) * len(q)] = tau[i * len(q):(i + 1) * len(q)]
                tau = full
        N, d_q, d_v, d_a = _samples_to_device(self.robot.model, q, v, a)
        d_tau = None if tau is None else tau if tau_resident else _lib.DeviceArray.from_host(tau)
        borrowed = [x.buf for x in (q, v, a) if isinstance(x, GpuMatrix)]
        in_flags, repack_ms = 0, 0.0
        m = self.robot.model
        if N > 0 and not (self._handle().is_chain() and mode == _lib.MODE_JOINT_TORQUE) and not self.coupling:
            import time
            _lib.synchronize()
            t0 = time.perf_counter()
            blocked = [_lib.repack_samples(d, N, w) for d, w in ((d_q, m.nq), (d_v, m.nv), (d_a, m.nv))]
            _lib.synchronize()
            repack_ms = 1e3 * (time.perf_counter() - t0)
            for d in (d_q, d_v, d_a):
                if not any(d is b for b in borrowed):
                    d.free()
            d_q, d_v, d_a = blocked
            in_flags = _lib.FLAG_BLOCKED_INPUTS
            if self.chunk_samples:
                self.chunk_samples = max(64, (int(self.chunk_samples) // 64) * 64)
        self._init_samples(N, d_q, d_v, d_a, d_tau, in_flags, repack_ms)
        self._init_layout()
        self._cert_cache = None
        ncols_ref = self._handle().shape(mode, self._flags()[1])[1] if N > 0 else 0
        self._force_compact_ok = N >= 64 and 3 * N >= 16 * (ncols_ref + 1)
        ex = self.exchange
        if self._collective() and ex.world_size > 1:
            flag = _lib.DeviceArray.from_host(np.array([0.0 if N >= 4096 else 1.0, 0.0 if self._force_compact_ok else 1.0]))
            agreed = np.asarray(ex.sum_columns(flag, 2)).reshape(-1)
            self.fuse = self.fuse and float(agreed[0]) == 0.0
            self._force_compact_ok = float(agreed[1]) == 0.0
            flag.free()

    def _flags(self):
        from .tools.regressor import regressor_flags
        mode, flags, ft_mask = regressor_flags(self.param, self.coupling)
        return mode, flags | self._in_flags, ft_mask

    def _chunks(self):
        c = self.chunk_samples
        return [(lo, min(lo + c, self.N)) for lo in range(0, self.N, c)]

    def _chunked(self):
        return bool(self.chunk_samples) and self.N > self.chunk_samples

    def _build_chunk(self, lo, hi, W, d_colsq):
        mode, flags, ft_mask = self._flags()
        m = self.robot.model
        _lib.regressor_build(self.robot.device_model(), mode, flags, ft_mask, hi - lo, _View(self.d_q, lo * m.nq * 8),
                             _View(self.d_v, lo * m.nv * 8), _View(self.d_a, lo * m.nv * 8), W.buf, W.ld, d_colsq)

    def _tau_chunk(self, lo, hi, rps, d_out, scatter=False):
        lib, nch = _lib.load(), hi - lo
        for j in range(rps):
            full, part = self.d_tau.ptr + (j * self.N + lo) * 8, d_out.ptr + j * nch * 8
            _lib.check(lib.figh_memcpy_d2d(full, part, nch * 8) if scatter else lib.figh_memcpy_d2d(part, full, nch * 8))

    def set_tau_from_parameters(self, phi, noise_std=0.0, seed=0):
        if self._chunked():
            mode, flags, _ = self._flags()
            rps, ncols = self.robot.device_model().shape(mode, flags)
            d_phi = _lib.DeviceArray.from_host(np.ascontiguousarray(phi, dtype=np.float64))
            self.d_tau = _lib.DeviceArray((rps * self.N,), np.float64)
            Wc = GpuMatrix.empty(rps * self.chunk_samples, ncols)
            d_t = _lib.DeviceArray((rps * self.chunk_samples,), np.float64)
            for lo, hi in self._chunks():
                self._build_chunk(lo, hi, Wc, None)
                _lib.matvec(Wc.buf, rps * (hi - lo), Wc.ld, None, ncols, d_phi, d_t)
                self._tau_chunk(lo, hi, rps, d_t, scatter=True)
            self.d_tau = self._with_noise(self.d_tau, noise_std, seed)
            return self.d_tau
        W, _ = build_regressor_device(self.robot, self.d_q, self.d_v, self.d_a, self.N, self.param, self.coupling,
                                      extra_flags=self._in_flags)
        d_phi = _lib.DeviceArray.from_host(np.ascontiguousarray(phi, dtype=np.float64))
        d_tau = _lib.DeviceArray((W.rows,), np.float64)
        _lib.matvec(W.buf, W.rows, W.ld, None, W.cols, d_phi, d_tau)
        self.d_tau = d_tau = self._with_noise(d_tau, noise_std, seed)
        W.buf.free()
        return d_tau

    @staticmethod
    def _with_noise(d_tau, noise_std, seed):
        if noise_std > 0.0:
            tau = d_tau.to_host()
            tau += np.random.default_rng(seed).standard_normal(tau.shape[0]) * noise_std
            d_tau = _lib.DeviceArray.from_host(tau)
        return d_tau

    def _run_chunked(self, strings):
        ex, lib = self.exchange, _lib.load()
        mode, flags, ft_mask = self._flags()
        dm = self.robot.device_model()
        rps, ncols = dm.shape(mode, flags)
        if self._dc_colsq is None or self._dc_colsq.size != ncols:
            cap = ncols + 1
            self._dc_colsq = _lib.DeviceArray((ncols,), np.float64)
            self._dc_idx = _lib.DeviceArray((cap,), np.int32)
            self._dc_R = _lib.DeviceArray((cap * cap,), np.float64)
            self._chunk_kept = None
        with_tau = self.d_tau is not None
        d_R = self._dc_R
        cached = self._chunk_kept
        if cached is not None and cached[0] == ncols:
            kept = cached[1]
            n = len(kept)
            _lib.regressor_tsqr(dm, mode, flags, ft_mask, self.N, self.d_q, self.d_v, self.d_a, self._dc_idx, n,
                                self.d_tau if with_tau else None, None, d_R, chunk_samples=self.chunk_samples,
                                d_colsq=self._dc_colsq)
            col_norm = ex.sum_columns(self._dc_colsq, ncols)
            if np.array_equal(np.flatnonzero(~(col_norm < self.tol_e)), cached[2]):
                nc = n + (1 if with_tau else 0)
                idx_e, params_r = list(cached[3]), list(cached[4])
                d_stack, count = ex.stack_triangles(d_R, nc)
                return self._tail(d_stack, count, n, nc, params_r, idx_e, col_norm, with_tau,
                                  rps * self.N * ex.world_size, strings)
            self._chunk_kept = None
        _lib.regressor_colsq(dm, mode, flags, ft_mask, self.N, self.d_q, self.d_v, self.d_a, self._dc_colsq,
                             chunk_samples=self.chunk_samples)
        col_norm = ex.sum_columns(self._dc_colsq, ncols)
        idx_e = [i for i in range(ncols) if col_norm[i] < self.tol_e]
        kept = [i for i in range(ncols) if not col_norm[i] < self.tol_e]
        params_r = [self.names[i] for i in kept]
        n = len(kept)
        nc = n + (1 if with_tau else 0)
        kept_i32 = np.asarray(kept, dtype=np.int32)
        _lib.check(lib.figh_memcpy_h2d(self._dc_idx.ptr, kept_i32.ctypes.data, kept_i32.nbytes))
        self._chunk_kept = (ncols, kept, np.asarray(kept, dtype=np.int64), list(idx_e), list(params_r))
        _lib.regressor_tsqr(dm, mode, flags, ft_mask, self.N, self.d_q, self.d_v, self.d_a, self._dc_idx, n,
                            self.d_tau if with_tau else None, None, d_R, chunk_samples=self.chunk_samples)
        d_stack, count = ex.stack_triangles(d_R, nc)
        return self._tail(d_stack, count, n, nc, params_r, idx_e, col_norm, with_tau, rps * self.N * ex.world_size, strings)

    def run(self, strings=True, wls=False):
        for _ in range(2):
            fused_before = self.fused_passes
            with _lib.null_pivots(self.tol_qr if self.null_pivots else None):
                out = self._run_once(strings, wls)
            if self.null_pivots and not out.get("null_rule_certified", True):
                self.null_pivots = False
                self.fused_passes = fused_before
                self.null_rule_fallbacks += 1
                self._cert_failed = (self._cert_cache, out["absdiagR"].copy(), list(out["idx_base"]))
                self._cert_cache = None
                continue
            return out
        return out

    def _run_once(self, strings, wls):
        self._init_pass()
        if self._chunked():
            if wls:
                raise NotImplementedError("wls=True needs the regressor resident in HBM (no chunk_samples)")
            return self._run_chunked(strings)
        if wls and not self._no_force_compact:
            self._no_force_compact = True
            if self._force_ld and self.W is not None:
                self._drop_resident()
        out = self._run_resident(strings and not wls, wls)
        if wls and out.get("null_rule_certified", True):
            self._wls(out, strings)
        return out

    def _drop_resident(self):
        self.W.buf.free()
        self._init_layout()

    def _allocate_resident(self, handle, mode, flags, ft_mask):
        self._init_layout()
        self._forget_columns()
        rows_per_sample, ncols = handle.shape(mode, flags)
        self._padded = not (handle.is_chain() and mode == _lib.MODE_JOINT_TORQUE) and not self.coupling
        m = self.robot.model
        wcols = 16 * (m.njoints - 1) if self._padded else ncols
        if self._padded and self.w_layout != "link-padded":
            layout = _lib.regressor_link_layout(handle, mode, flags & 7, ft_mask)
            if layout is not None and 0 < layout[1] < m.njoints - 1:
                self._link_pos = layout[0].astype(np.int64)
                self._d_link_pos = _lib.DeviceArray.from_host(layout[0])
                wcols = 16 * layout[1]
        if (self._padded and self.w_layout in ("dense", "block-compact") and not self._no_force_compact
                and self._force_compact_ok):
            self._force_ld = _lib.regressor_force_layout(handle, mode, flags & 7, ft_mask)
        if (self.w_layout == "block-compact" and self._padded and mode == _lib.MODE_JOINT_TORQUE
                and m.nv == m.njoints - 1 and self.N >= 64):
            sizes = self._subtree_sizes()
            j, k = np.nonzero(self._ancestor_matrix())
            if not ((j <= k) & (k < j + sizes[j])).all():
                raise RuntimeError("block-compact W needs depth-first joint numbering")
            ld = 16 * sizes
            if self.row_blocks is not None:
                keep = np.zeros(m.nv, dtype=bool)
                keep[self.row_blocks] = True
                ld = np.where(keep, ld, 0)
            off = self.N * np.concatenate([[0], np.cumsum(ld)[:-1]])
            self._compact = (off.astype(np.int64), ld.astype(np.int32))
            self.W = GpuMatrix(_lib.DeviceArray((int(self.N * ld.sum()),), np.float64), rows_per_sample * self.N, wcols,
                               wcols)
            self.W.compact = self._compact
        elif self._force_ld:
            half = (rows_per_sample // 2) * self.N
            self.W = GpuMatrix(_lib.DeviceArray((half * (self._force_ld + wcols),), np.float64), rows_per_sample * self.N,
                               wcols, wcols)
            self.W.force_ld = self._force_ld
        else:
            self.W = self._place_W(rows_per_sample * self.N, wcols, handle, mode, flags, ft_mask)
        self.W.ref_cols = ncols
        self._zeros_once = (self.structural_zeros == "once" and self._padded and mode == _lib.MODE_JOINT_TORQUE
                            and self._compact is None)
        if self._zeros_once:
            _lib.check(_lib.load().figh_memset(self.W.buf.ptr, 0, self.W.rows * self.W.ld * 8))
        self._padded_flags = (flags | (_lib.FLAG_ZEROS_PRESENT if self._zeros_once else 0)
                              | (_lib.FLAG_COMPACT_BLOCKS if self._compact is not None else 0)
                              | (_lib.FLAG_LINK_COMPACT if self._link_pos is not None else 0)
                              | (_lib.FLAG_FORCE_COMPACT if self._force_ld else 0))
        cap = ncols + 1
        self._sel_words = (2 + 2 * ncols + 1) // 2
        self._d_pack = _lib.DeviceArray((ncols + self._sel_words + (cap + 1) * cap,), np.float64)
        self._d_colsq = _View(self._d_pack, 0)
        self._d_sel = _View(self._d_pack, ncols * 8)
        self._d_rows = _View(self._d_pack, (ncols + self._sel_words) * 8)
        self._d_R = _lib.DeviceArray((cap * cap,), np.float64)
        structured = mode == _lib.MODE_JOINT_TORQUE and m.nv == m.njoints - 1 and self.N >= 64
        self._hint_blocks = m.nv if structured else 0
        from .model import JT_FREEFLYER
        self._wrench_split = (mode == _lib.MODE_EXT_WRENCH and rows_per_sample == 6 and len(m.joints) > 1 and
                              m.joints[1].jtype == JT_FREEFLYER and not self.coupling)
        self._tree_blocks = bool(structured and self._padded)
        if self._compact is not None and not self._tree_blocks:
            raise RuntimeError("block-compact W needs the per-row-block TSQR")
        if self.row_blocks is not None and not self._tree_blocks:
            raise NotImplementedError("row_blocks needs the per-row-block TSQR: joint-torque regressor of a tree of "
                                      "single-dof joints with at least 64 samples")

    def _run_resident(self, strings, wls):
        ex = self.exchange
        mode, flags, ft_mask = self._flags()
        handle = self._handle()
        if self.W is None:
            self._allocate_resident(handle, mode, flags, ft_mask)
        W, d_colsq = self.W, self._d_colsq
        if (self.fuse and self._fused_kept is None and not self._padded and self.N >= 4096
                and handle.is_chain() and mode == _lib.MODE_JOINT_TORQUE and not self.coupling):
            self._learn_kept_set(handle, mode, flags, ft_mask)
        if self.fuse and self._fused_kept is not None and not self._padded:
            out = self._run_fused(handle, flags, strings)
            if out is not None:
                return out
        if self._padded:
            _lib.regressor_build_padded(handle, mode, self._padded_flags, ft_mask, self.N, self.d_q, self.d_v, self.d_a,
                                        W.buf, W.ld, d_colsq)
        else:
            _lib.regressor_build(handle, mode, flags, ft_mask, self.N, self.d_q, self.d_v, self.d_a, W.buf, W.ld, d_colsq)
        ex.sum_columns_device(d_colsq, W.ref_cols)
        ncols, with_tau = W.ref_cols, self.d_tau is not None
        stride = 16 if self._padded else 14
        split, local = self._wrench_split, not self._collective()
        tol_rank, d_out = (self.tol_qr, self._d_rows) if local else (-1.0, self._d_R)
        for attempt in range(4):
            n = self._n_expected
            nf = self._nf_expected if split else 0
            nc = n + (1 if with_tau else 0)
            blocks = None
            if self._tree_blocks and (nc > 80 or self._compact is not None or self.row_blocks is not None):
                blocks = self._block_lists(ncols, stride)
                if blocks is None and self.row_blocks is not None and n > 0:
                    raise RuntimeError("row_blocks: no kept mask to build the column lists from")
            if self._compact is not None and blocks is None and n > 0:
                raise RuntimeError("block-compact W: no kept mask to build the column lists from")
            if split or self._link_pos is not None or self._force_ld:
                try:
                    _lib.tsqr_selected_wrench(W.buf, W.rows, W.ld, d_colsq, ncols, self.tol_e, stride, n, nf, self.d_tau,
                                              tol_rank, self._d_sel, d_out, d_link_pos=self._d_link_pos, ld_force=self._force_ld)
                except _lib.FighError as e:
                    if not (self._force_ld and e.code == _lib.ERR_UNSUPPORTED):
                        raise
                    self._no_force_compact = True
                    self._drop_resident()
                    return self._run_resident(strings, wls)
            elif blocks is not None:
                coff, cld = self._compact if self._compact is not None else (None, None)
                _lib.tsqr_selected_blocks(W.buf, W.rows, W.ld, d_colsq, ncols, self.tol_e, stride, n, blocks[1],
                                          blocks[4] if coff is not None else blocks[2], blocks[3], self.d_tau, tol_rank,
                                          self._d_sel, d_out, block_off=coff, block_ld=cld,
                                          d_block_tri=self._block_tri(wls, len(blocks[1]), nc))
            else:
                _lib.tsqr_selected(W.buf, W.rows, W.ld, d_colsq, ncols, self.tol_e, stride, self._hint_blocks, n, self.d_tau,
                                   tol_rank, self._d_sel, d_out)
            self._have_block_tri = bool(wls and blocks is not None and not split)
            if not local:
                if n > 0:
                    d_stack, count = ex.stack_triangles(self._d_R, nc)
                    _lib.tsqr_merge_base(d_stack, count, nc, n, self.tol_qr, self._d_rows)
            norms, sel, mask_now, rows_k = self._fetch_pack(ncols, n, nc)
            nf_now = 0
            if split:
                nf_now = int(np.count_nonzero(sel[2 + ncols:2 + 2 * ncols][self._force_slots(ncols)]))
            if int(sel[0]) == n and nf_now == nf and (blocks is None or np.array_equal(mask_now, blocks[0])):
                break
            self._mask_expected = mask_now.copy()
            self._n_expected = int(sel[0])
            self._nf_expected = nf_now
            if self._n_expected == 0:
                raise ValueError("every column of the regressor was eliminated")
        else:
            raise RuntimeError("the number of kept columns did not settle")
        col_norm = norms.copy()
        kept_mask = mask_now
        idx_e, params_r = self._kept_lists(kept_mask)
        if self.fuse and not self._padded and self._compact is None and (
                self._fused_kept is None or not np.array_equal(self._fused_kept[0], kept_mask)):
            self._remember_fused_kept(kept_mask, ncols)
        rows_mine = W.rows if self.row_blocks is None else len(self.row_blocks) * self.N
        return self._finish(rows_k, n, nc, params_r, idx_e, col_norm, with_tau, rows_mine * ex.world_size, strings,
                            defer_beta=wls and with_tau)

    def forget(self):
        self._forget_columns()
        self._fused_kept = self._chunk_kept = self._cert_cache = None

    def _forget_columns(self):
        self._kept_cache = self._mask_expected = self._block_cache = None
        self._n_expected = self._nf_expected = -1

    def _fetch_pack(self, ncols, n, nc):
        words = ncols + self._sel_words + ((nc + 1) * nc if n > 0 else 0)
        host = self._landing().array[:words]
        _lib.check(_lib.load().figh_memcpy_d2h(host.ctypes.data, self._d_pack.ptr, host.nbytes))
        sel = host[ncols:ncols + self._sel_words].view(np.int32)
        rows_k = host[ncols + self._sel_words:].reshape(nc + 1, nc) if n > 0 else None
        return host[:ncols], sel, sel[2 + ncols:2 + 2 * ncols] != 0, rows_k

    def _landing(self):
        pin = self._host_pack = _grown(self._host_pack, self._d_pack.size, _lib.PinnedArray)
        return pin

    def _kept_lists(self, mask):
        cached = self._kept_cache
        if cached is None or not np.array_equal(cached[0], mask):
            idx_e = np.flatnonzero(~mask).tolist()
            params_r = [self.names[i] for i in np.flatnonzero(mask).tolist()]
            cached = self._kept_cache = (mask.copy(), idx_e, params_r)
        return list(cached[1]), list(cached[2])

    def _remember_fused_kept(self, mask, ncols):
        kept = np.flatnonzero(mask).astype(np.int32)
        buf = self._d_kept_buf = _grown(self._d_kept_buf, ncols, lambda k: _lib.DeviceArray((k,), np.int32))
        _lib.check(_lib.load().figh_memcpy_h2d(buf.ptr, kept.ctypes.data, kept.nbytes))
        self._fused_kept = (mask.copy(), buf, len(kept))

    PREFIX_SAMPLES = 4096

    def _learn_kept_set(self, handle, mode, flags, ft_mask):
        ex, W = self.exchange, self.W
        n0 = min(self.N, self.PREFIX_SAMPLES)
        _lib.regressor_build(handle, mode, flags, ft_mask, n0, self.d_q, self.d_v, self.d_a, W.buf, W.ld, self._d_colsq)
        ex.sum_columns_device(self._d_colsq, W.ref_cols)
        _lib.select_columns(self._d_colsq, W.ref_cols, self.tol_e, 14, self._d_sel)
        sel = np.empty(2 + 2 * W.ref_cols, dtype=np.int32)
        _lib.check(_lib.load().figh_memcpy_d2h(sel.ctypes.data, self._d_sel.ptr, sel.nbytes))
        mask = sel[2 + W.ref_cols:] != 0
        if not mask.any():
            return
        self._remember_fused_kept(mask, W.ref_cols)
        self.prefix_passes += 1

    def _run_fused(self, handle, flags, strings):
        ex, W = self.exchange, self.W
        self._have_block_tri = False
        mask, d_kept, n = self._fused_kept
        ncols, with_tau = W.ref_cols, self.d_tau is not None
        nc = n + (1 if with_tau else 0)
        local = not self._collective()
        if local and self.native_tail and nc <= 80:
            return self._run_fused_native(handle, flags, strings, mask, d_kept, n, nc, with_tau)
        if not _lib.regressor_tsqr_fused(handle, flags, self.N, self.d_q, self.d_v, self.d_a, W.buf, W.ld, self._d_colsq,
                                         d_kept, n, self.d_tau, self.tol_qr if local else -1.0,
                                         self._d_rows if local else self._d_R):
            self.fuse = False
            return None
        ex.sum_columns_device(self._d_colsq, ncols)
        _lib.select_columns(self._d_colsq, ncols, self.tol_e, 14, self._d_sel)
        if not local:
            d_stack, count = ex.stack_triangles(self._d_R, nc)
            _lib.tsqr_merge_base(d_stack, count, nc, n, self.tol_qr, self._d_rows)
        norms, _, mask_now, rows_k = self._fetch_pack(ncols, n, nc)
        if not np.array_equal(mask_now, mask):
            self._fused_kept = None
            return None
        self.fused_passes += 1
        self._n_expected = n
        idx_e, params_r = self._kept_lists(mask)
        return self._finish(rows_k, n, nc, params_r, idx_e, norms.copy(), with_tau, W.rows * ex.world_size, strings)

    def _run_fused_native(self, handle, flags, strings, mask, d_kept, n, nc, with_tau):
        ex, W = self.exchange, self.W
        ncols = W.ref_cols
        pin = self._landing()
        total_rows = W.rows * ex.world_size
        tail = self._tail_args(n, with_tau, total_rows)
        ok = _lib.chain_pass_fused(handle, flags, self.N, self.d_q, self.d_v, self.d_a, W.buf, W.ld, d_kept, n, self.d_tau,
                                   self.tol_qr, self.tol_e, self._d_pack, pin.array.ctypes.data, 8 * pin.size,
                                   mask.view(np.uint8), tail)
        if ok is None:
            self.fuse = False
            return None
        if not ok:
            self._fused_kept = None
            return None
        self.fused_passes += 1
        self._n_expected = n
        idx_e, params_r = self._kept_lists(mask)
        out = self._native_out(tail, n, params_r, idx_e, pin.array[:ncols].copy(), with_tau, total_rows, strings)
        with _single_threaded_blas(n):
            pass
        return out

    def _tail_args(self, n, with_tau, total_rows):
        tail = self._host_tail
        if tail is None or tail.n != n or tail.with_tau != bool(with_tau):
            tail = self._host_tail = _lib.HostTail(n, with_tau)
        s = tail.s
        s.tol_qr, s.total_rows, s.pieces = self.tol_qr, int(total_rows), self._level0_pieces(total_rows)
        s.null_rule = int(self.null_pivots)
        if self._cert_cache is None or tail.cache_of is not self._cert_cache:
            s.n_cached_base = -1
        return tail

    def _native_out(self, tail, n, params_r, idx_e, col_norm, with_tau, total_rows, strings):
        s = tail.s
        r = s.n_base
        assert len(params_r) == n, "params_r does not have same length with R"
        if self.null_pivots and s.bounds_recomputed:
            self._cert_cache = ((n, tail.idx[:r].astype(np.int64).tobytes()), tail.bounds_tuple())
            tail.keep_bounds(self._cert_cache)
        if s.status == _lib.TAIL_SINGULAR:
            raise np.linalg.LinAlgError("Singular matrix")
        idx = tail.idx.tolist()
        idx_base, idx_regroup = idx[:r], idx[r:]
        beta = tail.beta[:r * (n - r)].reshape(r, n - r).copy()
        absdiag = tail.absdiag.copy()
        out = {
            "idx_e": idx_e, "params_r": params_r, "idx_base": idx_base, "beta": beta,
            "col_norm": col_norm, "absdiagR": absdiag, "rows": total_rows,
        }
        if self.null_pivots:
            from . import _host
            self._cert_args = (absdiag.copy(), idx_base, idx_regroup, self._cert_cache[1])
            out["null_rule_certified"] = _host.null_rule_certified(*self._cert_args, self.tol_qr, rows=total_rows, pieces=s.pieces,
                                                                   native_verdict=s.certified)
        if strings:
            out["params_base"] = self._expressions_memo(params_r, tail.idx.tobytes() + bytes((r,)), idx_base, idx_regroup, beta)
        if with_tau:
            out["phi_b"] = tail.phi_b[:r].copy()
            out["phi_ls"] = tail.phi_ls[:r].copy()
            out["residual_norm"] = float(s.residual_norm)
        return out

    def _expressions_memo(self, params_r, idx_key, idx_base, idx_regroup, beta):
        memo = self._strings_memo
        beta_key = (beta + 0.0).tobytes()
        if memo is not None and memo[1] == idx_key and memo[2] == beta_key and memo[0] == params_r:
            self.strings_memo_hits += 1
            return list(memo[3])
        exprs = qrd._expressions([params_r[i] for i in idx_base], [params_r[i] for i in idx_regroup], beta)
        self._strings_memo = (list(params_r), idx_key, beta_key, list(exprs))
        return exprs

    def _block_tri(self, wls, nblocks, nc):
        if not wls:
            return None
        need = (nblocks + 2) * nc * nc
        buf = self._d_block_tri = _grown(self._d_block_tri, need, lambda k: _lib.DeviceArray((k,), np.float64))
        return buf

    def _sb(self, name, count, dtype=np.float64):
        pool = self._scratch
        buf = pool.get(name)
        if buf is None or buf.size != int(count) or buf.dtype != np.dtype(dtype):
            if buf is not None:
                buf.free()
            buf = pool[name] = _lib.DeviceArray((int(count),), dtype)
        return buf

    def _up(self, name, host):
        host = np.ascontiguousarray(host)
        buf = self._sb(name, host.size, host.dtype)
        _lib.check(_lib.load().figh_memcpy_h2d(buf.ptr, host.ctypes.data, host.nbytes))
        return buf

    def _wls(self, out, strings=False):
        if self.d_tau is None:
            raise ValueError("wls=True needs tau")
        ex, W = self.exchange, self.W
        n = len(out["params_r"])
        nc = n + 1
        base = np.asarray(out["idx_base"], dtype=np.int64)
        nb_par = len(base)
        phi_b = np.ascontiguousarray(out["phi_b"], dtype=np.float64)
        mode, _, _ = self._flags()
        nblocks = self.robot.model.nv if mode == _lib.MODE_JOINT_TORQUE else 6
        rows_blk = W.rows // nblocks
        d_r2 = self._sb("wls_r2", nblocks + 1)
        _rows = np.array([float(rows_blk)])
        _lib.check(_lib.load().figh_memcpy_h2d(d_r2.ptr + 8 * nblocks, _rows.ctypes.data, 8))
        d_Rw = self._sb("wls_Rw", (nb_par + 1) * (nb_par + 1))
        kept = np.flatnonzero(self._kept_cache[0])
        if self._have_block_tri:
            tri = self._d_block_tri
            counts = np.asarray(self._block_cache[1], dtype=np.int64) + 1
            row_off = np.concatenate([[0], np.cumsum(counts)])
            v = np.zeros(nc)
            v[base] = phi_b
            v[n] = -1.0
            _lib.block_rows_residuals(tri, row_off, nc, self._up("wls_v", v), d_r2)
            r2 = np.asarray(ex.sum_columns(d_r2, nblocks + 1))
            sig2 = r2[:nblocks] / r2[nblocks]
            if self.row_blocks is not None:
                inactive = counts == 0
                sig2 = np.where(inactive, 1.0, sig2)
            d_cols = self._up("wls_cols", np.r_[base, n].astype(np.int32))
            _lib.tsqr(tri, int(row_off[-1]), nc, d_cols, nb_par + 1, None, np.repeat(1.0 / np.sqrt(sig2), counts), d_Rw)
            if self.row_blocks is not None:
                sig2 = sig2[self.row_blocks]
            source = "per-row-block triangles"
        else:
            if self._compact is not None or self.row_blocks is not None:
                raise RuntimeError("block-compact W / row_blocks without per-row-block triangles")
            d_cols = self._up("wls_cols", np.asarray(self.device_columns(kept[base]), dtype=np.int32))
            d_est = self._sb("wls_est", W.rows)
            _lib.matvec(W.buf, W.rows, W.ld, d_cols, nb_par, self._up("wls_phi", phi_b), d_est)
            _lib.block_sqnorm(self.d_tau, d_est, W.rows, nblocks, d_r2)
            r2 = np.asarray(ex.sum_columns(d_r2, nblocks + 1))
            sig2 = r2[:nblocks] / r2[nblocks]
            _lib.tsqr(W.buf, W.rows, W.ld, d_cols, nb_par, self.d_tau, 1.0 / np.sqrt(sig2), d_Rw)
            source = "second pass over W"
        if self._collective() and ex.world_size > 1:
            d_stack, count = ex.stack_triangles(d_Rw, nb_par + 1)
            d_one = self._sb("wls_one", (nb_par + 1) * (nb_par + 1))
            _lib.tsqr_merge(d_stack, count, nb_par + 1, d_one)
            d_Rw = d_one
        self._finish_beta(out)
        if strings and "params_base" not in out:
            params_r = out["params_r"]
            regroup = np.setdiff1d(np.arange(n), base).tolist()
            out["params_base"] = qrd._expressions([params_r[i] for i in base.tolist()], [params_r[i] for i in regroup],
                                                  out["beta"])
        Rw = d_Rw.to_host().reshape(nb_par + 1, nb_par + 1)
        R, z = np.triu(Rw[:nb_par, :nb_par]), Rw[:nb_par, nb_par]
        with _single_threaded_blas(nb_par):
            phi = np.around(_solve_upper(np.asfortranarray(R), np.asfortranarray(z.reshape(-1, 1)))[:, 0], 6)
            R_inv, info = _dtrtri(np.ascontiguousarray(R))
            if info != 0:
                raise np.linalg.LinAlgError("Singular matrix")
            std = _relative_percent(np.sqrt(np.einsum("ij,ij->i", R_inv, R_inv)), phi)
        out["phi_wls"], out["std_wls"], out["sigma2_joint"], out["wls_source"] = phi, std, sig2, source
        return out

    def _finish_beta(self, out):
        later = self._beta_later
        if later is None or out.get("beta") is not None:
            return
        R1, R2, _, _ = later
        self._beta_later = None
        with _single_threaded_blas(len(R1)):
            out["beta"] = np.around(_solve_upper(R1, np.asfortranarray(R2)), 6)

    def _block_lists(self, ncols, stride):
        mask = self._mask_expected
        if mask is None or len(mask) != ncols:
            return None
        cached = self._block_cache
        if cached is not None and np.array_equal(cached[0], mask):
            return cached
        nb, anc = self.robot.model.nv, self._ancestor_matrix()
        kept = np.flatnonzero(mask)
        link, slot = kept // 14, kept % 14
        counts, cols, pos, ccols = [], [], [], []
        active = None if self.row_blocks is None else set(self.row_blocks)
        for j in range(nb):
            if active is not None and j not in active:
                counts.append(-1)
                continue
            in_block = (anc[j][np.minimum(link, nb - 1)] & (link < nb) & (slot < 10)) | ((link == j) & (slot >= 10))
            p = np.flatnonzero(in_block)
            counts.append(len(p))
            pos.append(p)
            cols.append(link[p] * stride + slot[p])
            ccols.append((link[p] - j) * 16 + slot[p])
        pad = [np.zeros(1, dtype=np.int64)]
        d_cols = _lib.DeviceArray.from_host(np.concatenate(cols + pad).astype(np.int32))
        d_pos = _lib.DeviceArray.from_host(np.concatenate(pos + pad).astype(np.int32))
        d_ccols = _lib.DeviceArray.from_host(np.concatenate(ccols + pad).astype(np.int32))
        self._block_cache = (mask.copy(), np.asarray(counts, dtype=np.int32), d_cols, d_pos, d_ccols)
        return self._block_cache

    def _subtree_sizes(self):
        return self._ancestor_matrix().sum(axis=1, dtype=np.int64)

    def _ancestor_matrix(self):
        anc = self._ancestors
        if anc is None:
            m = self.robot.model
            parents = list(m.parents)
            anc = self._ancestors = np.zeros((m.nv, m.nv), dtype=bool)
            for k in range(m.nv):
                jid = k + 1
                while jid > 0:
                    anc[jid - 1, k] = True
                    jid = parents[jid]
        return anc

    def _force_slots(self, ncols):
        m = self._force_slot_mask
        if m is None or len(m) != ncols:
            m = self._force_slot_mask = (np.arange(ncols) % 14) >= 6
        return m

    def device_columns(self, ref_cols):
        if self._compact is not None:
            raise ValueError("block-compact W has no global column numbering: row block j is its own N x 16 |subtree_j| "
                             "matrix (pipe.W.compact = (element offsets, leading dimensions))")
        c = np.asarray(ref_cols, dtype=np.int64)
        if self._force_ld:
            raise ValueError("force-compact W is two matrices (force rows: pipe.W.force_ld columns, torque rows behind them): "
                             "no single column numbering; IdentificationPipeline(w_layout='link-compact') keeps one")
        if self._link_pos is not None:
            pos = self._link_pos[c // 14]
            if (pos < 0).any():
                raise ValueError("link-compact W holds no columns for links without entries (structural zeros)")
            return pos * 16 + c % 14
        return (c // 14) * 16 + c % 14 if self._padded else c

    def _place_W(self, rows, cols, handle, mode, flags, ft_mask):
        import time
        nbytes = rows * cols * 8
        trials = self.placement_trials
        if trials > 1:
            trials = max(1, min(trials, int(0.5 * _lib.device_info()["hbm_bytes"] // max(nbytes, 1))))
        if trials <= 1:
            return GpuMatrix.empty(rows, cols)
        d_cs = _lib.DeviceArray((cols,), np.float64)
        build = _lib.regressor_build_padded if self._padded else _lib.regressor_build
        cands, times = [], []
        for _ in range(trials):
            W = GpuMatrix.empty(rows, cols)
            for rep in range(4):
                if rep == 1:
                    _lib.synchronize()
                    t0 = time.perf_counter()
                build(handle, mode, flags, ft_mask, self.N, self.d_q, self.d_v, self.d_a, W.buf, W.ld, d_cs)
            _lib.synchronize()
            cands.append(W)
            times.append((time.perf_counter() - t0) / 3)
        best = int(np.argmin(times))
        for i, W in enumerate(cands):
            if i != best:
                W.buf.free()
        self.placement_report = {"trials": trials, "k1_ms": [round(1e3 * t, 4) for t in times], "kept": best}
        return cands[best]

    def _tail(self, d_stack, count, n, nc, params_r, idx_e, col_norm, with_tau, total_rows, strings):
        lib = _lib.load()
        pack = self._d_tailpack = _grown(self._d_tailpack, (nc + 1) * nc, lambda k: _lib.DeviceArray((k,), np.float64))
        _lib.tsqr_merge_base(d_stack, count, nc, n, self.tol_qr, pack)
        pin = self._host_tailpack = _grown(self._host_tailpack, (nc + 1) * nc, _lib.PinnedArray)
        host = pin.array[:(nc + 1) * nc]
        _lib.check(lib.figh_memcpy_d2h(host.ctypes.data, pack.ptr, host.nbytes))
        return self._finish(host.reshape(nc + 1, nc), n, nc, params_r, idx_e, col_norm, with_tau, total_rows, strings)

    def _level0_pieces(self, total_rows):
        N = max(1, int(self.N))
        chunks = -(-N // int(self.chunk_samples)) if self.chunk_samples else 1
        return max(1, int(total_rows) // N) * chunks

    def _finish(self, rows_k, n, nc, params_r, idx_e, col_norm, with_tau, total_rows, strings, defer_beta=False):
        if self.native_tail and 1 <= n <= 80:
            tail = self._tail_args(n, with_tau, total_rows)
# ... 53 lines not shown
```

### include/figh.h

```cpp
#ifndef FIGH_H
#define FIGH_H

#include <stddef.h>
#include <stdint.h>

#ifdef __cplusplus
extern "C" {
#endif

typedef enum {
    FIGH_OK = 0,
    FIGH_ERR_INVALID = -1,
    FIGH_ERR_NO_DEVICE = -2,
    FIGH_ERR_ALLOC = -3,
    FIGH_ERR_UNSUPPORTED = -4,
    FIGH_ERR_COMM = -5
} figh_status;

enum { FIGH_JT_REVOLUTE = 0, FIGH_JT_PRISMATIC = 1, FIGH_JT_CONTINUOUS = 2, FIGH_JT_FREEFLYER = 3, FIGH_JT_UNIVERSE = -1 };
enum { FIGH_MODE_JOINT_TORQUE = 0, FIGH_MODE_EXT_WRENCH = 1 };
enum { FIGH_FLAG_FRICTION = 1, FIGH_FLAG_ACT_INERTIA = 2, FIGH_FLAG_OFFSET = 4, FIGH_FLAG_TX40 = 8, FIGH_FLAG_GENERIC = 256,
       FIGH_FLAG_BLOCKED_INPUTS = 512,
       FIGH_FLAG_ZEROS_PRESENT = 1024,
       FIGH_FLAG_COMPACT_BLOCKS = 2048,
       FIGH_FLAG_LINK_COMPACT = 4096,
       FIGH_FLAG_FORCE_COMPACT = 8192 };

typedef struct figh_model_s *figh_model_t;

#define FIGH_ABI_VERSION 113
int figh_version(void);
const char *figh_last_error(void);
int figh_device_count(int *count);
int figh_device_set(int device);
int figh_host_wait_mode(int blocking);
int figh_tsqr_null_pivot_tol(double tol);
int figh_device_pci_bus_id(int device, char *out, int out_len);
int figh_device_info(char *name, int name_len, int *cu_count, size_t *hbm_bytes);
int figh_malloc(void **d_ptr, size_t bytes);
int figh_free(void *d_ptr);
int figh_memcpy_h2d(void *d_dst, const void *h_src, size_t bytes);
int figh_memcpy_d2h(void *h_dst, const void *d_src, size_t bytes);
int figh_host_alloc(void **h_ptr, size_t bytes);
int figh_host_free(void *h_ptr);
int figh_memcpy_d2d(void *d_dst, const void *d_src, size_t bytes);
int figh_memset(void *d_dst, int value, size_t bytes);
int figh_synchronize(void);
int figh_profile_enable(int level);
int figh_profile_reset(void);
int figh_profile_get(const char *name, int *launches, double *total_ms);

int figh_model_create(int njoints, const int32_t *parents, const int32_t *jtype, const double *axis,
                      const double *placement, const int32_t *idx_q, const int32_t *idx_v, const double *gravity,
                      const int32_t *body_mask, figh_model_t *out);
int figh_model_destroy(figh_model_t model);
int figh_model_set_active_rows(figh_model_t model, const int32_t *h_rows, int n);
int figh_regressor_shape(figh_model_t model, int mode, int flags, int *rows_per_sample, int *ncols);

int figh_regressor_build(figh_model_t model, int mode, int flags, int ft_mask, int64_t N, const double *d_q,
                         const double *d_v, const double *d_a, double *d_W, int64_t ldw, double *d_colsq);

int figh_regressor_build_padded(figh_model_t model, int mode, int flags, int ft_mask, int64_t N, const double *d_q,
                                const double *d_v, const double *d_a, double *d_W, int64_t ldw, double *d_colsq);
int figh_regressor_link_layout(figh_model_t model, int mode, int flags, int ft_mask, int32_t *h_link_pos, int *nlive);
int figh_regressor_force_layout(figh_model_t model, int mode, int flags, int ft_mask, int64_t *ld_force);

int figh_regressor_apply(figh_model_t model, int mode, int flags, int ft_mask, int64_t N, const double *d_q,
                         const double *d_v, const double *d_a, const double *d_phi, double *d_tau_out);

int figh_repack_samples(const double *d_src, int64_t N, int width, double *d_dst);

int figh_coupling_tx40(int64_t N, int nv, const double *d_v, const double *d_a, double *d_out);

int figh_colsq(const double *d_W, int64_t rows, int cols, int64_t ldw, double *d_out);
int figh_gather_cols(const double *d_W, int64_t rows, int64_t ldw, const int32_t *d_col_idx, int n, double *d_out,
                     int64_t ldo);
int figh_place_block(const double *d_src, int64_t ld_src, int64_t rows, int64_t cols, double scale, double *d_dst,
                     int64_t ld_dst);
int figh_matvec(const double *d_W, int64_t rows, int64_t ldw, const int32_t *d_col_idx, int n, const double *d_x,
                double *d_y);
int figh_block_sqnorm(const double *d_a, const double *d_b, int64_t rows, int nblocks, double *d_out);

int figh_tsqr(const double *d_W, int64_t rows, int64_t ldw, const int32_t *d_col_idx, int n, const double *d_tau,
              const double *h_block_weight, int nblocks, double *d_R_out);
int figh_tsqr_structured(const double *d_W, int64_t rows, int64_t ldw, const int32_t *d_col_idx, int n,
                         const double *d_tau, const double *h_block_weight, int nblocks, const int32_t *h_first_col,
                         int nfirst, double *d_R_out);
int figh_compact_rows(const double *d_W, int64_t rows, int cols, int64_t ldw, const double *d_tau, int key_col,
                      double threshold, double *d_W_out, int64_t ld_out, double *d_tau_out, int64_t *h_count_out);
int figh_base_permutation(const double *d_R, int nc, int n, double tol_qr, int32_t *d_perm);
int figh_tsqr_merge(const double *d_Rs, int count, int nc, double *d_R_out);

int figh_select_columns(const double *d_colsq, int ncols, double tol_e, int link_stride, int32_t *d_sel);
int figh_tsqr_selected(const double *d_W, int64_t rows, int64_t ldw, const double *d_colsq, int ncols, double tol_e,
                       int link_stride, int nblocks, int n_expected, const double *d_tau, double tol_qr, int32_t *d_sel,
                       double *d_R_out);
int figh_regressor_tsqr_fused(figh_model_t model, int flags, int64_t N, const double *d_q, const double *d_v,
                              const double *d_a, double *d_W, int64_t ldw, double *d_colsq, const int32_t *d_kept, int n,
                              const double *d_tau, double tol_qr, double *d_R_out);
enum { FIGH_TAIL_OK = 0, FIGH_TAIL_SINGULAR = 1 };
typedef struct figh_host_tail_s {
    const double *rows_k;
    int32_t n, with_tau;
    double tol_qr;
    int64_t total_rows, pieces;
    int32_t null_rule;
    int32_t n_cached_base;
    const int32_t *cached_base;
    double *bounds;
    int32_t *idx;
    double *absdiag;
    double *beta;
    double *phi_ls, *phi_b;
    double residual_norm;
    int32_t n_base, status, certified, bounds_recomputed;
} figh_host_tail_t;
int figh_chain_host_tail(figh_host_tail_t *tail);
int figh_chain_pass_fused(figh_model_t model, int flags, int64_t N, const double *d_q, const double *d_v, const double *d_a,
                          double *d_W, int64_t ldw, const int32_t *d_kept, int n, const double *d_tau, double tol_qr,
                          double tol_e, double *d_pack, double *h_pack, size_t pack_bytes, const uint8_t *h_kept_mask,
                          int *changed, figh_host_tail_t *tail);
int figh_tsqr_selected_wrench(const double *d_W, int64_t rows, int64_t ldw, const double *d_colsq, int ncols, double tol_e,
                              int link_stride, int n_expected, int nf_expected, const double *d_tau, double tol_qr,
                              int32_t *d_sel, double *d_R_out, const int32_t *d_link_pos, int64_t ld_force);
int figh_tsqr_selected_blocks(const double *d_W, int64_t rows, int64_t ldw, const double *d_colsq, int ncols, double tol_e,
                              int link_stride, int n_expected, int nblocks, const int32_t *h_counts, const int32_t *d_cols,
                              const int32_t *d_pos, const int64_t *h_block_off, const int32_t *h_block_ld,
                              const double *d_tau, double tol_qr, int32_t *d_sel, double *d_R_out, double *d_block_tri);
int figh_block_rows_residuals(const double *d_rows, int nblocks, const int32_t *h_row_off, int nc, const double *d_v,
                              double *d_r2);
int figh_tsqr_merge_base(const double *d_Rs, int count, int nc, int n_free, double tol_qr, double *d_rows_out);

int figh_regressor_colsq(figh_model_t model, int mode, int flags, int ft_mask, int64_t N, const double *d_q,
                         const double *d_v, const double *d_a, int64_t chunk_samples, double *d_colsq);
int figh_regressor_tsqr(figh_model_t model, int mode, int flags, int ft_mask, int64_t N, const double *d_q,
                        const double *d_v, const double *d_a, const int32_t *d_col_idx, int n, const double *d_tau,
                        const double *h_block_weight, int nblocks, int64_t chunk_samples, double *d_R_out);
int figh_regressor_tsqr_norms(figh_model_t model, int mode, int flags, int ft_mask, int64_t N, const double *d_q,
                              const double *d_v, const double *d_a, const int32_t *d_col_idx, int n, const double *d_tau,
                              const double *h_block_weight, int nblocks, int64_t chunk_samples, double *d_R_out,
                              double *d_colsq_out);
int figh_regressor_tsqr_batch(figh_model_t model, int mode, int flags, int ft_mask, int64_t B, int64_t n_per,
                              const double *d_q, const double *d_v, const double *d_a, const int32_t *d_col_idx, int n,
                              const double *d_R_stack, double *d_R_out);
int figh_regressor_tsqr_batch_fused(figh_model_t model, int flags, int64_t B, int64_t n_per, const double *d_q,
                                    const double *d_v, const double *d_a, const int32_t *d_col_idx, int n,
                                    const double *d_R_stack, double *d_R_out);
int figh_regressor_gram(figh_model_t model, int mode, int flags, int ft_mask, int64_t N, const double *d_q,
                        const double *d_v, const double *d_a, const int32_t *d_col_idx, int n, const double *d_tau,
                        int64_t chunk_samples, double *h_G, double *h_g, double *h_tau_sq);

int figh_filtfilt_cols(const double *d_X, int64_t rows, int cols, int64_t ldx, int nblocks, int form, const double *h_b,
                       const double *h_a, int nsec, int order, const double *h_zi, int padlen, int q, double *d_Y,
                       int64_t ldy, int64_t *rows_out);

int figh_medfilt_cols(const double *d_X, int64_t rows, int cols, int64_t ldx, int nblocks, int kernel_size, double *d_Y,
                      int64_t ldy);
int figh_joint_difference(figh_model_t model, int64_t N, const double *d_q, double ts, const double *d_dt, double *d_dq);
int figh_gradient_cols(const double *d_F, int64_t rows, int cols, int64_t ld, int ncols_active, double h, const double *d_h,
                       double *d_G, int64_t ldg);

int figh_spline_sample(figh_model_t model, int64_t B, int n_wps, int n_act, int64_t n_per, double freq,
                       const int32_t *h_act_idxq, const int32_t *h_act_idxv, const double *h_tps, const double *d_wps,
                       const double *d_vel_wps, int64_t vel_stride, const double *d_acc_wps, int64_t acc_stride,
                       const double *d_q0, double *d_q, int64_t ldq, double *d_v, double *d_a, int64_t ldv);
int figh_excitation_constraints(figh_model_t model, int64_t B, int64_t n_per, int n_act, const int32_t *h_act_idxq,
                                const int32_t *h_act_idxv, int n_idx, const int32_t *h_idx_waypoints, const double *d_q,
                                int64_t ldq, const double *d_v, int64_t ldv, const double *d_tau, double *d_out,
                                int64_t ld_out);

int figh_kinematic_regressor(figh_model_t model, int64_t N, const double *d_q, int64_t ldq, int end_joint,
                             const double *h_end_placement, int start_joint, const double *h_start_placement,
                             const int32_t *h_support, int n_support, int meas_mask, double *d_R, int64_t ldr, double *d_J,
                             int64_t ldj, double *d_rowsq_R, double *d_rowsq_J);
int figh_calib_fkm_batch(figh_model_t model, int64_t B, int64_t N, const double *d_q, int64_t ldq, int n_chain,
                         const int32_t *h_chain, const double *d_placements, const double *d_wMo, const double *d_eeMf,
                         int end_joint, const double *h_end_placement, int start_joint, const double *h_start_placement,
                         int meas_mask, double *d_out, int64_t ld_out);
int figh_gather_rows(const double *d_W, int64_t ldw, int cols, const int32_t *d_row_idx, int64_t n, double *d_out,
                     int64_t ld_out);

#define FIGH_DESIGN_MAX_COLS 96
int figh_design_gram(const double *d_R, int64_t ldr, int64_t N, int c, int n, const double *d_w, double *h_M);
int figh_design_scores(const double *d_R, int64_t ldr, int64_t N, int c, int n, const double *h_L, double *d_trace,
                       double *d_det_add, double *d_det_rm);

int figh_comm_available(void);
int figh_comm_unique_id(void *h_id128);
int figh_comm_init(int nranks, int rank, const void *h_id128);
int figh_comm_destroy(void);
int figh_comm_allgather(const double *d_send, double *d_all, int64_t count_per_rank);
int figh_comm_allreduce_sum(double *d_buf, int64_t count);

#ifdef __cplusplus
}
#endif
#endif
```

Before: 717.4 million.

## Add base-only fused pass that factors base columns and bounds dependent residuals

Adds a fused regressor+TSQR path that factors only the learned base columns and, inside the producer waves, accumulates squared residuals of the dependent columns against their learned base coefficients. The host learns the base/dependent split from a previous pass (or a prefix pass) and reuses it as long as the kept mask is unchanged. It falls back to the full path if the residual bound is not certified. The aim is a narrower QR triangle, at the cost of extra residual arithmetic, more LDS, an extra prefix TSQR, and more complex fallback logic.

```diff
diff --git a/figaroh_plus_amd/_lib.py b/figaroh_plus_amd/_lib.py
--- a/figaroh_plus_amd/_lib.py
+++ b/figaroh_plus_amd/_lib.py
@@ -8,7 +8,7 @@
 _HERE = os.path.dirname(os.path.abspath(__file__))
 LIB_PATH = os.environ.get("FIGH_LIB_PATH") or os.path.join(_HERE, "libfigh.so")
 
-ABI_VERSION = 113
+ABI_VERSION = 114
 
 FIGH_OK = 0
 ERR_INVALID, ERR_NO_DEVICE, ERR_ALLOC, ERR_UNSUPPORTED, ERR_COMM = -1, -2, -3, -4, -5
@@ -86,6 +86,10 @@
     "figh_chain_pass_fused": (C.c_int, [C.c_void_p, C.c_int, C.c_int64, C.c_void_p, C.c_void_p, C.c_void_p, C.c_void_p,
                                         C.c_int64, C.c_void_p, C.c_int, C.c_void_p, C.c_double, C.c_double, C.c_void_p,
                                         C.c_void_p, C.c_size_t, C.c_void_p, C.POINTER(C.c_int), C.c_void_p]),
+    "figh_chain_base_tail": (C.c_int, [C.c_void_p]),
+    "figh_chain_pass_base_only": (C.c_int, [C.c_void_p, C.c_int, C.c_int64, C.c_void_p, C.c_void_p, C.c_void_p, C.c_void_p,
+                                            C.c_int64, C.c_void_p, C.c_void_p, C.c_double, C.c_double, C.c_void_p,
+                                            C.c_void_p, C.c_size_t, C.c_void_p, C.POINTER(C.c_int), C.c_void_p]),
     "figh_tsqr_merge_base": (C.c_int, [C.c_void_p, C.c_int, C.c_int, C.c_int, C.c_double, C.c_void_p]),
     "figh_compact_rows": (C.c_int, [C.c_void_p, C.c_int64, C.c_int, C.c_int64, C.c_void_p, C.c_int, C.c_double, C.c_void_p,
                                     C.c_int64, C.c_void_p, C.POINTER(C.c_int64)]),
@@ -707,6 +711,61 @@
     return not changed.value
 
 
+PASS_OK, PASS_CHANGED, PASS_NOT_CERTIFIED = 0, 1, 2
+BASE_ONLY_MAX_DEP = 16
+
+
+class _BaseTailStruct(C.Structure):
+    _fields_ = [("base", _HostTailStruct), ("n", C.c_int32), ("nd", C.c_int32), ("base_pos", C.c_void_p),
+                ("dep_pos", C.c_void_p), ("coef_ptr", C.c_void_p), ("coef_idx", C.c_void_p), ("coef_val", C.c_void_p),
+                ("bound", C.c_void_p), ("idx", C.c_void_p), ("absdiag", C.c_void_p), ("beta", C.c_void_p)]
+
+
+class BaseTail:
+
+    def __init__(self, base_pos, dep_pos, bhat, with_tau):
+        self.base_pos = np.ascontiguousarray(base_pos, dtype=np.int32)
+        self.dep_pos = np.ascontiguousarray(dep_pos, dtype=np.int32)
+        nb, nd = len(self.base_pos), len(self.dep_pos)
+        self.n, self.nd, self.with_tau = nb + nd, nd, bool(with_tau)
+        bhat = np.asarray(bhat, dtype=np.float64).reshape(nb, nd)
+        rows = [np.flatnonzero(bhat[:, k]) for k in range(nd)]
+        self.coef_ptr = np.concatenate([[0], np.cumsum([len(r) for r in rows])]).astype(np.int32)
+        self.coef_idx = np.concatenate(rows + [np.zeros(1, dtype=np.int64)]).astype(np.int32)
+        self.coef_val = np.concatenate([bhat[r, k] for k, r in enumerate(rows)] + [np.zeros(1)])
+        self.bound = np.zeros(max(nd, 1))
+        self.idx = np.zeros(self.n, dtype=np.int32)
+        self.absdiag, self.beta = np.zeros(self.n), np.zeros(max(nb * nd, 1))
+        self.inner = HostTail(nb, with_tau)
+        s = self.s = _BaseTailStruct()
+        self.bind()
+
+    def bind(self):
+        s = self.s
+        C.memmove(C.addressof(s.base), self.inner.ref, C.sizeof(_HostTailStruct))
+        s.n, s.nd = self.n, self.nd
+        for name in ("base_pos", "dep_pos", "coef_ptr", "coef_idx", "coef_val", "bound", "idx", "absdiag", "beta"):
+            setattr(s, name, getattr(self, name).ctypes.data)
+        self.ref = C.addressof(s)
+
+
+def chain_base_tail(tail, rows_k):
+    tail.s.base.rows_k = rows_k.ctypes.data
+    check(load().figh_chain_base_tail(tail.ref))
+
+
+def chain_pass_base_only(model, flags, N, d_q, d_v, d_a, d_W, ldw, kept_i32, d_tau, tol_qr, tol_e, d_pack, h_pack, pack_bytes,
+                         kept_mask_u8, tail):
+    status = C.c_int(0)
+    rc = load().figh_chain_pass_base_only(model.handle, flags, N, d_q.ptr, d_v.ptr, d_a.ptr, d_W.ptr, ldw,
+                                          kept_i32.ctypes.data, d_tau.ptr if d_tau is not None else None, tol_qr, tol_e,
+                                          d_pack.ptr, h_pack, pack_bytes, kept_mask_u8.ctypes.data, C.byref(status), tail.ref)
+    if rc == ERR_UNSUPPORTED:
+        return None
+    check(rc)
+    return status.value
+
+
 def tsqr_merge_base(d_Rs, count, nc, n_free, tol_qr, d_Rk):
     check(load().figh_tsqr_merge_base(d_Rs.ptr, count, nc, n_free, tol_qr, d_Rk.ptr))
 
diff --git a/figaroh_plus_amd/csrc/figh_fused.hip b/figaroh_plus_amd/csrc/figh_fused.hip
--- a/figaroh_plus_amd/csrc/figh_fused.hip
+++ b/figaroh_plus_amd/csrc/figh_fused.hip
@@ -1,6 +1,7 @@
 #include <algorithm>
 #include <cmath>
 #include <cstdlib>
+#include <cstring>
 #include <string>
 #include <type_traits>
 
@@ -58,12 +59,22 @@
     static constexpr int CONS0 = NPROD * PSIZE;
 };
 
-template <int NJ, bool TRAJ = false>
+struct FusedResid {
+    const int *__restrict__ dep;
+    const int *__restrict__ ptr;
+    const int *__restrict__ col;
+    const double *__restrict__ val;
+    int nd;
+    double *sums;
+};
+
+template <int NJ, bool TRAJ = false, bool RES = false>
 __global__ __launch_bounds__(512) void fused_chain_tsqr_kernel(
     const ChainParams<NJ> P, const int flags, const long N, const double *__restrict__ q, const double *__restrict__ v,
     const double *__restrict__ a, double *__restrict__ W, const double *__restrict__ tau, const int *__restrict__ col_idx,
     const int n, const int nc, double *__restrict__ colsq_part, double *__restrict__ Rws, const int ncons,
-    const int tri_doubles, const double null2) {
+    const int tri_doubles, const double null2, const FusedResid res) {
+    static_assert(!(TRAJ && RES), "the batched form has no dependent columns to bound");
     using G = FusedGeom<NJ>;
     constexpr int NC = G::NC, LDT = G::LDT, CH = G::CH;
     constexpr int NCC = 4, NRC = 4, RPL = 16;
@@ -86,6 +97,9 @@
     for (int pz = 0; pz < G::NPROD; ++pz)
         for (int e = pz * G::PSIZE + G::CS0 + threadIdx.x; e < (pz + 1) * G::PSIZE; e += blockDim.x) lds[e] = 0.0;
     for (int e = G::CONS0 + threadIdx.x; e < G::CONS0 + ncons * tri_doubles; e += blockDim.x) lds[e] = 0.0;
+    const int racc0 = G::CONS0 + ncons * tri_doubles;
+    if constexpr (RES)
+        for (int e = racc0 + threadIdx.x; e < racc0 + G::NPROD * res.nd * 64; e += blockDim.x) lds[e] = 0.0;
     __syncthreads();
 
     if (wave < G::NPROD) {
@@ -95,6 +109,7 @@
         FusedCtrl *ctrl = reinterpret_cast<FusedCtrl *>(tile + G::CTRL0);
         double *my = tile + lane * LDT;
         double *stau = tile + G::TAU0, *sqd = tile + G::QD0, *cacc = tile + G::CS0;
+        double *racc = lds + racc0 + wave * res.nd * 64 + lane;
         int t = 0;
         auto sample_tile = [&](auto FAST_T, const long s) {
             constexpr bool FAST = decltype(FAST_T)::value;
@@ -309,6 +324,21 @@
                     if (lane < width) cacc[lo + lane] += column_sum(tile + lo + lane);
                     if (width > 64 && lane + 64 < width) cacc[lo + 64 + lane] += column_sum(tile + lo + 64 + lane);
                 }
+                if constexpr (RES) {
+                    const int lo = 14 * j;
+#pragma unroll 1
+                    for (int k = 0; k < res.nd; ++k) {
+                        const int c = res.dep[k];
+                        if (c < lo) continue;
+                        double r = my[c];
+#pragma unroll 1
+                        for (int e = res.ptr[k]; e < res.ptr[k + 1]; ++e) {
+                            const int cb = res.col[e];
+                            if (cb >= lo) r -= res.val[e] * my[cb];
+                        }
+                        racc[64 * k] += r * r;
+                    }
+                }
             }
         };
         for (long s = b + wave * Gd; s < ntiles_s; s += G::NPROD * Gd) {
@@ -316,7 +346,16 @@
             else sample_tile(std::false_type{}, s);
         }
         asm volatile("" ::: "memory");
-        if constexpr (!TRAJ)
+        if constexpr (RES) {
+            double *row = colsq_part + (b * G::NPROD + wave) * (NC + res.nd);
+            for (int c = lane; c < NC; c += 64) row[c] = cacc[c];
+            if (lane < res.nd) {
+                const double *mine = racc - lane + 64 * lane;
+                double s = 0.0;
+                for (int l = 0; l < 64; ++l) s += mine[l];
+                row[NC + lane] = s;
+            }
+        } else if constexpr (!TRAJ)
             for (int c = lane; c < NC; c += 64) colsq_part[(b * G::NPROD + wave) * NC + c] = cacc[c];
         return;
     }
@@ -427,49 +466,55 @@
     size_t lds;
 };
 
-template <int NJ, bool TRAJ>
-static int fused_plan(const figh_model_s *m, int nc, FusedPlan<NJ> *plan) {
+template <int NJ, bool TRAJ, bool RES = false>
+static int fused_plan(const figh_model_s *m, int nc, FusedPlan<NJ> *plan, int nd = 0) {
     constexpr size_t fixed = FusedGeom<NJ>::CONS0, budget = (160 * 1024) / sizeof(double);
     const size_t tri = (size_t)tsqr2_tri_doubles(4, nc, true);
+    const size_t racc = RES ? (size_t)FusedGeom<NJ>::NPROD * nd * 64 : 0;
     const int ncons = (int)std::min<size_t>(6, (budget - fixed) / tri);
     if (ncons < 3) {
         set_error(std::string(TRAJ ? "fused batch regressor + TSQR" : "fused regressor + TSQR") +
                   ": the triangles of three consumer waves do not fit next to the tile");
         return FIGH_ERR_UNSUPPORTED;
     }
+    if (RES && fixed + (size_t)ncons * tri + racc > budget) {
+        set_error("fused regressor + TSQR over base columns: the residual accumulators do not fit behind the triangles");
+        return FIGH_ERR_UNSUPPORTED;
+    }
     static bool attr_set = false;
     if (!attr_set) {
-        FIGH_HIP(hipFuncSetAttribute(reinterpret_cast<const void *>(&fused_chain_tsqr_kernel<NJ, TRAJ>),
+        FIGH_HIP(hipFuncSetAttribute(reinterpret_cast<const void *>(&fused_chain_tsqr_kernel<NJ, TRAJ, RES>),
                                      hipFuncAttributeMaxDynamicSharedMemorySize, 160 * 1024));
         attr_set = true;
     }
     plan->P = chain_params<NJ>(m);
     plan->tri = (int)tri;
     plan->ncons = ncons;
-    plan->lds = sizeof(double) * (fixed + (size_t)ncons * tri);
+    plan->lds = sizeof(double) * (fixed + (size_t)ncons * tri + racc);
     return FIGH_OK;
 }
 
-template <int NJ>
+template <int NJ, bool RES = false>
 static int launch_fused(const figh_model_s *m, int flags, long N, const double *q, const double *v, const double *a,
                         double *W, const double *tau, const int *d_kept, int n, double *d_colsq, double **Rws_out,
-                        long *count_out) {
+                        long *count_out, const FusedResid res = FusedResid{}) {
     using G = FusedGeom<NJ>;
-    const int nc = n + (tau ? 1 : 0);
+    const int nc = n + (tau ? 1 : 0), width = G::NC + (RES ? res.nd : 0);
     FusedPlan<NJ> pl;
-    if (int rc = fused_plan<NJ, false>(m, nc, &pl)) return rc;
+    if (int rc = fused_plan<NJ, false, RES>(m, nc, &pl, res.nd)) return rc;
     const int cus = cu_count(), ncons = pl.ncons;
     const long ntiles_s = (N + 63) / 64;
     long grid = cus < ntiles_s / 2 ? cus : ntiles_s / 2;
-    double *part = static_cast<double *>(workspace(sizeof(double) * grid * G::NPROD * G::NC, kWsRegressorNorms));
+    double *part = static_cast<double *>(workspace(sizeof(double) * grid * G::NPROD * width, kWsRegressorNorms));
     double *Rws = static_cast<double *>(workspace(sizeof(double) * (size_t)nc * nc * (grid * ncons + 1), kWsLevel0TriOrWrench));
     if (!part || !Rws) return FIGH_ERR_ALLOC;
     {
         ProfileScope scope("fused_chain_tsqr", true);
-        FIGH_LAUNCH_TIMED((fused_chain_tsqr_kernel<NJ, false>), dim3((unsigned)grid), dim3(64 * (G::NPROD + ncons)), pl.lds,
-                          pl.P, flags, N, q, v, a, W, tau, d_kept, n, nc, part, Rws, ncons, pl.tri, null_pivot_sq());
-    }
-    launch_reduce_partials(part, (int)(grid * G::NPROD), G::NC, d_colsq);
+        FIGH_LAUNCH_TIMED((fused_chain_tsqr_kernel<NJ, false, RES>), dim3((unsigned)grid), dim3(64 * (G::NPROD + ncons)), pl.lds,
+                          pl.P, flags, N, q, v, a, W, tau, d_kept, n, nc, part, Rws, ncons, pl.tri, RES ? 0.0 : null_pivot_sq(),
+                          res);
+    }
+    launch_reduce_partials(part, (int)(grid * G::NPROD), width, d_colsq, G::NC, RES ? res.sums : nullptr);
     FIGH_HIP(hipGetLastError());
     *Rws_out = Rws;
     *count_out = grid * ncons;
@@ -497,7 +542,7 @@
         ProfileScope scope("fused_chain_tsqr_batch", true);
         FIGH_LAUNCH_TIMED((fused_chain_tsqr_kernel<NJ, true>), dim3((unsigned)S, (unsigned)B), dim3(64 * (G::NPROD + ncons)),
                           pl.lds, pl.P, flags, n_per, q, v, a, (double *)nullptr, (const double *)nullptr, d_cols, n, nc,
-                          (double *)nullptr, Rws, ncons, pl.tri, null_pivot_sq());
+                          (double *)nullptr, Rws, ncons, pl.tri, null_pivot_sq(), FusedResid{});
     }
     FIGH_HIP(hipGetLastError());
     const double *cur = Rws, *extra = d_R_stack;
@@ -526,7 +571,7 @@
 
 static int fused_pass_launch(figh_model_t model, int flags, int64_t N, const double *d_q, const double *d_v, const double *d_a,
                              double *d_W, int64_t ldw, double *d_colsq, const int32_t *d_kept, int n, const double *d_tau,
-                             double **Rws, long *count) {
+                             double **Rws, long *count, const FusedResid *res = nullptr) {
     FIGH_REQUIRE(N >= 0 && n >= 1, "bad shape");
     const DevModel &h = model->host;
     const int nc = n + (d_tau ? 1 : 0);
@@ -539,6 +584,19 @@
     }
     if (int rc = ensure_device()) return rc;
     const int f = flags & 7;
+    if (res) {
+        switch (h.nlinks) {
+            case 5:
+                return launch_fused<5, true>(model, f, (long)N, d_q, d_v, d_a, d_W, d_tau, d_kept, n, d_colsq, Rws, count, *res);
+            case 6:
+                return launch_fused<6, true>(model, f, (long)N, d_q, d_v, d_a, d_W, d_tau, d_kept, n, d_colsq, Rws, count, *res);
+            case 7:
+                return launch_fused<7, true>(model, f, (long)N, d_q, d_v, d_a, d_W, d_tau, d_kept, n, d_colsq, Rws, count, *res);
+            default:
+                set_error("fused regressor + TSQR: serial chains of 5 to 7 joints (LDS: two tile buffers + three consumer triangles)");
+                return FIGH_ERR_UNSUPPORTED;
+        }
+    }
     switch (h.nlinks) {
         case 5:
             return launch_fused<5>(model, f, (long)N, d_q, d_v, d_a, d_W, d_tau, d_kept, n, d_colsq, Rws, count);
@@ -596,6 +654,108 @@
     return figh_chain_host_tail(tail);
 }
 
+namespace {
+constexpr int kResidTerms = FIGH_BASE_ONLY_MAX_DEP * 64;
+struct ResidTables {
+    int32_t base[64];
+    int32_t dep[FIGH_BASE_ONLY_MAX_DEP];
+    int32_t ptr[FIGH_BASE_ONLY_MAX_DEP + 2];
+    int32_t col[kResidTerms];
+    double val[kResidTerms];
+};
+ResidTables g_resid_host;
+const ResidTables *g_resid_dev = nullptr;
+}
+
+extern "C" int figh_chain_pass_base_only(figh_model_t model, int flags, int64_t N, const double *d_q, const double *d_v,
+                                         const double *d_a, double *d_W, int64_t ldw, const int32_t *h_kept,
+                                         const double *d_tau, double tol_qr, double tol_e, double *d_pack, double *h_pack,
+                                         size_t pack_bytes, const uint8_t *h_kept_mask, int *status,
+                                         figh_base_tail_t *tail) {
+    FIGH_REQUIRE(model && d_q && d_v && d_a && d_W && h_kept && d_pack && h_pack && h_kept_mask && status && tail,
+                 "NULL pointer");
+    FIGH_REQUIRE(tail->base_pos && tail->dep_pos && tail->coef_ptr && tail->coef_idx && tail->coef_val && tail->bound,
+                 "figh_chain_pass_base_only: NULL table");
+    FIGH_REQUIRE(tol_qr >= 0.0, "figh_chain_pass_base_only: the rank decision needs tol_qr >= 0");
+    const int ncols = 14 * model->host.nlinks, n = tail->n, nd = tail->nd, nb = tail->base.n;
+    const int ncb = nb + (d_tau ? 1 : 0);
+    FIGH_REQUIRE(nd >= 1 && nd <= FIGH_BASE_ONLY_MAX_DEP && nb >= 1 && nb <= 64 && n == nb + nd && n <= ncols,
+                 "figh_chain_pass_base_only: n = base.n + nd kept columns, 1 .. 16 of them dependent, at most 64 base columns");
+    FIGH_REQUIRE((tail->base.with_tau != 0) == (d_tau != nullptr) && !tail->base.null_rule,
+                 "figh_chain_pass_base_only: tail of another shape");
+    const size_t sel_words = (size_t)(2 + 2 * ncols + 1) / 2;
+    const size_t rows_at = (size_t)ncols + sel_words, sums_at = rows_at + (size_t)(ncb + 1) * ncb;
+    const size_t words = sums_at + FIGH_BASE_ONLY_MAX_DEP;
+    FIGH_REQUIRE(pack_bytes >= sizeof(double) * words, "figh_chain_pass_base_only: the pack is [colsq | sel | rows | bounds]");
+    ResidTables tb;
+    std::memset(&tb, 0, sizeof(tb));
+    for (int e = 0; e < n; ++e)
+        FIGH_REQUIRE(h_kept[e] >= 0 && h_kept[e] < ncols && (e == 0 || h_kept[e] > h_kept[e - 1]) && h_kept_mask[h_kept[e]],
+                     "figh_chain_pass_base_only: h_kept is the ascending list of the mask's columns");
+    for (int i = 0; i < nb; ++i) {
+        const int p = tail->base_pos[i];
+        FIGH_REQUIRE(p >= 0 && p < n && (i == 0 || p > tail->base_pos[i - 1]), "figh_chain_pass_base_only: base_pos");
+        tb.base[i] = h_kept[p];
+    }
+    FIGH_REQUIRE(tail->coef_ptr[0] == 0, "figh_chain_pass_base_only: coef_ptr starts at 0");
+    for (int k = 0; k < nd; ++k) {
+        const int p = tail->dep_pos[k];
+        FIGH_REQUIRE(p >= 0 && p < n && (k == 0 || p > tail->dep_pos[k - 1]), "figh_chain_pass_base_only: dep_pos");
+        tb.dep[k] = h_kept[p];
+        const int e0 = tail->coef_ptr[k], e1 = tail->coef_ptr[k + 1];
+        FIGH_REQUIRE(e1 >= e0 && e1 - e0 <= nb && e1 <= kResidTerms, "figh_chain_pass_base_only: coef_ptr");
+        tb.ptr[k + 1] = e1;
+        for (int e = e0; e < e1; ++e) {
+            const int i = tail->coef_idx[e];
+            FIGH_REQUIRE(i >= 0 && i < nb && (e == e0 || i > tail->coef_idx[e - 1]) && tail->base_pos[i] < p,
+                         "figh_chain_pass_base_only: a coefficient belongs to a base column in front of its dependent column");
+            tb.col[e] = tb.base[i];
+            tb.val[e] = tail->coef_val[e];
+        }
+    }
+    if (int rc = ensure_device()) return rc;
+    ResidTables *d_tb = static_cast<ResidTables *>(workspace(sizeof(ResidTables), kWsFusedResid));
+    if (!d_tb) return FIGH_ERR_ALLOC;
+    if (d_tb != g_resid_dev || std::memcmp(&tb, &g_resid_host, sizeof(tb)) != 0) {
+        g_resid_dev = nullptr;
+        FIGH_HIP(hipMemcpyAsync(d_tb, &tb, sizeof(tb), hipMemcpyHostToDevice, stream()));
+        FIGH_HIP(hipStreamSynchronize(stream()));
+        g_resid_host = tb;
+        g_resid_dev = d_tb;
+    }
+    const FusedResid res{d_tb->dep, d_tb->ptr, d_tb->col, d_tb->val, nd, d_pack + sums_at};
+    double *d_colsq = d_pack, *d_rows = d_pack + rows_at;
+    int32_t *d_sel = reinterpret_cast<int32_t *>(d_pack + ncols);
+    double *Rws = nullptr;
+    long count = 0;
+    if (int rc = fused_pass_launch(model, flags, N, d_q, d_v, d_a, d_W, ldw, d_colsq, d_tb->base, nb, d_tau, &Rws, &count, &res))
+        return rc;
+    if (int rc = tsqr_reduce_stack(Rws, count, ncb, nb, tol_qr, d_rows)) return rc;
+    if (int rc = figh_select_columns(d_colsq, ncols, tol_e, 14, d_sel)) return rc;
+    FIGH_HIP(hipMemcpyAsync(h_pack, d_pack, sizeof(double) * words, hipMemcpyDeviceToHost, stream()));
+    FIGH_HIP(hipStreamSynchronize(stream()));
+    const int32_t *mask_now = reinterpret_cast<const int32_t *>(h_pack + ncols) + 2 + ncols;
+    for (int c = 0; c < ncols; ++c)
+        if ((mask_now[c] != 0) != (h_kept_mask[c] != 0)) {
+            *status = FIGH_PASS_CHANGED;
+            return FIGH_OK;
+        }
+    const double *rows_k = h_pack + rows_at, *diag = rows_k + (size_t)ncb * ncb;
+    bool certified = true;
+    for (int k = 0; k < nd; ++k) {
+        tail->bound[k] = std::sqrt(h_pack[sums_at + k]);
+        certified = certified && tail->bound[k] <= tol_qr / 4.0;
+    }
+    for (int i = 0; i < nb; ++i) certified = certified && std::fabs(diag[i]) >= 100.0 * tol_qr;
+    if (!certified) {
+        *status = FIGH_PASS_NOT_CERTIFIED;
+        return FIGH_OK;
+    }
+    *status = FIGH_PASS_OK;
+    tail->base.rows_k = rows_k;
+    return figh_chain_base_tail(tail);
+}
+
 static constexpr int64_t kFusedBatchMinSamples = 64;
 
 extern "C" int figh_regressor_tsqr_batch_fused(figh_model_t model, int flags, int64_t B, int64_t n_per, const double *d_q,
diff --git a/figaroh_plus_amd/csrc/figh_host_tail.hip b/figaroh_plus_amd/csrc/figh_host_tail.hip
--- a/figaroh_plus_amd/csrc/figh_host_tail.hip
+++ b/figaroh_plus_amd/csrc/figh_host_tail.hip
@@ -143,6 +143,51 @@
     return FIGH_OK;
 }
 
+int base_tail(figh_base_tail_t *t) {
+    FIGH_REQUIRE(t && t->base_pos && t->dep_pos && t->coef_ptr && t->coef_idx && t->coef_val && t->bound && t->idx &&
+                     t->absdiag && t->beta,
+                 "figh_chain_base_tail: NULL pointer");
+    const int n = t->n, nd = t->nd, nb = t->base.n;
+    FIGH_REQUIRE(nd >= 0 && nd <= FIGH_BASE_ONLY_MAX_DEP && nb >= 1 && n == nb + nd && n <= kTailMax,
+                 "figh_chain_base_tail: n = base.n + nd kept columns, at most 16 dependent, at most 80 in all");
+    FIGH_REQUIRE(!t->base.null_rule, "figh_chain_base_tail: base-only passes run plain Householder");
+    bool seen[kTailMax] = {false};
+    for (int i = 0; i < nb; ++i) {
+        const int p = t->base_pos[i];
+        FIGH_REQUIRE(p >= 0 && p < n && !seen[p] && (i == 0 || p > t->base_pos[i - 1]), "figh_chain_base_tail: base_pos");
+        seen[p] = true;
+    }
+    FIGH_REQUIRE(t->coef_ptr[0] == 0, "figh_chain_base_tail: coef_ptr starts at 0");
+    for (int k = 0; k < nd; ++k) {
+        const int p = t->dep_pos[k];
+        FIGH_REQUIRE(p >= 0 && p < n && !seen[p] && (k == 0 || p > t->dep_pos[k - 1]), "figh_chain_base_tail: dep_pos");
+        seen[p] = true;
+        FIGH_REQUIRE(t->coef_ptr[k + 1] >= t->coef_ptr[k] && t->coef_ptr[k + 1] - t->coef_ptr[k] <= nb,
+                     "figh_chain_base_tail: coef_ptr");
+        for (int e = t->coef_ptr[k]; e < t->coef_ptr[k + 1]; ++e) {
+            const int i = t->coef_idx[e];
+            FIGH_REQUIRE(i >= 0 && i < nb && (e == t->coef_ptr[k] || i > t->coef_idx[e - 1]) && t->base_pos[i] < p,
+                         "figh_chain_base_tail: a coefficient belongs to a base column in front of its dependent column");
+        }
+    }
+    if (int rc = host_tail(&t->base)) return rc;
+    if (t->base.status != FIGH_TAIL_OK) return FIGH_OK;
+    FIGH_REQUIRE(t->base.n_base == nb, "figh_chain_base_tail: a base pivot is not above tol_qr");
+    for (int i = 0; i < nb; ++i) {
+        t->idx[i] = t->base_pos[i];
+        t->absdiag[t->base_pos[i]] = t->base.absdiag[i];
+    }
+    for (int e = 0; e < nb * nd; ++e) t->beta[e] = 0.0;
+    for (int k = 0; k < nd; ++k) {
+        t->idx[nb + k] = t->dep_pos[k];
+        t->absdiag[t->dep_pos[k]] = t->bound[k];
+        for (int e = t->coef_ptr[k]; e < t->coef_ptr[k + 1]; ++e)
+            t->beta[(size_t)t->coef_idx[e] * nd + k] = round6(t->coef_val[e]);
+    }
+    return FIGH_OK;
+}
+
 }
 
 extern "C" int figh_chain_host_tail(figh_host_tail_t *t) { return figh::host_tail(t); }
+extern "C" int figh_chain_base_tail(figh_base_tail_t *t) { return figh::base_tail(t); }
diff --git a/figaroh_plus_amd/csrc/figh_internal.h b/figaroh_plus_amd/csrc/figh_internal.h
--- a/figaroh_plus_amd/csrc/figh_internal.h
+++ b/figaroh_plus_amd/csrc/figh_internal.h
@@ -109,6 +109,7 @@
     kWsDesignPartials,
     kWsDesignGram,
     kWsDesignFactor,
+    kWsFusedResid,
     kWorkspaceSlots
 };
 
@@ -141,7 +142,7 @@
 int64_t tsqr_level0_capacity(int nc);
 int tile_hint(const int32_t *h_first_col, int nfirst, int64_t rows, int n, int nc, const int **out);
 
-void launch_reduce_partials(const double *part, int nblocks, int ncols, double *out);
+void launch_reduce_partials(const double *part, int nblocks, int ncols, double *out, int split = 0, double *out2 = nullptr);
 
 int launch_regressor_tree(const figh_model_s *m, int mode, int flags, int ft_mask, long N, const double *q,
                           const double *v, const double *a, double *W, long ldw, int ncols, int link_stride,
diff --git a/figaroh_plus_amd/csrc/figh_linalg.hip b/figaroh_plus_amd/csrc/figh_linalg.hip
--- a/figaroh_plus_amd/csrc/figh_linalg.hip
+++ b/figaroh_plus_amd/csrc/figh_linalg.hip
@@ -51,7 +51,8 @@
 }
 
 __global__ __launch_bounds__(256) void reduce_partials_kernel(const double *__restrict__ part, int nblocks, int ncols,
-                                                              double *__restrict__ out) {
+                                                              double *__restrict__ out, int split,
+                                                              double *__restrict__ out2) {
     __shared__ double sm[256];
     const int c = blockIdx.x;
     double s = 0.0;
@@ -62,11 +63,15 @@
         if ((int)threadIdx.x < w) sm[threadIdx.x] += sm[threadIdx.x + w];
         __syncthreads();
     }
-    if (threadIdx.x == 0) out[c] = sm[0];
-}
-
-void launch_reduce_partials(const double *part, int nblocks, int ncols, double *out) {
-    hipLaunchKernelGGL(reduce_partials_kernel, dim3(ncols), dim3(256), 0, stream(), part, nblocks, ncols, out);
+    if (threadIdx.x == 0) {
+        if (c < split) out[c] = sm[0];
+        else out2[c - split] = sm[0];
+    }
+}
+
+void launch_reduce_partials(const double *part, int nblocks, int ncols, double *out, int split, double *out2) {
+    hipLaunchKernelGGL(reduce_partials_kernel, dim3(ncols), dim3(256), 0, stream(), part, nblocks, ncols, out,
+                       out2 ? split : ncols, out2);
 }
 
 __global__ __launch_bounds__(256) void gather_cols_kernel(const double *__restrict__ W, long rows, long ldw,
diff --git a/figaroh_plus_amd/pipeline.py b/figaroh_plus_amd/pipeline.py
--- a/figaroh_plus_amd/pipeline.py
+++ b/figaroh_plus_amd/pipeline.py
@@ -63,9 +63,10 @@
 
     def __init__(self, robot, param, params_std=None, coupling=False, tol_e=1e-6, tol_qr=qrd.TOL_QR, exchange=None,
                  chunk_samples=None, placement_trials=1, structural_zeros="every-pass", w_layout="dense", fuse=True, null_pivots=True,
-                 row_blocks=None, native_tail=True):
+                 row_blocks=None, native_tail=True, base_only=False):
         self.chunk_samples = chunk_samples
         self.native_tail = bool(native_tail)
+        self._base_only_requested = bool(base_only)
         self.row_blocks = None if row_blocks is None else [int(b) for b in row_blocks]
         self._fuse_requested = bool(fuse)
         self._null_pivots_requested = bool(null_pivots)
@@ -90,6 +91,7 @@
         self._strings_memo = self._force_slot_mask = self._ancestors = None
         self._scratch = {}
         self.fused_passes = self.prefix_passes = self.null_rule_fallbacks = self.strings_memo_hits = 0
+        self.base_only_fallbacks = 0
         self.placement_report = self._cert_failed = None
         self._no_force_compact = False
 
@@ -170,6 +172,7 @@
         self._init_samples(N, d_q, d_v, d_a, d_tau, in_flags, repack_ms)
         self._init_layout()
         self._cert_cache = None
+        self._base_split, self._base_only_off = None, not self._base_only_requested
         ncols_ref = self._handle().shape(mode, self._flags()[1])[1] if N > 0 else 0
         self._force_compact_ok = N >= 64 and 3 * N >= 16 * (ncols_ref + 1)
         ex = self.exchange
@@ -465,6 +468,7 @@
     def forget(self):
         self._forget_columns()
         self._fused_kept = self._chunk_kept = self._cert_cache = None
+        self._base_split, self._base_only_off = None, not self._base_only_requested
 
     def _forget_columns(self):
         self._kept_cache = self._mask_expected = self._block_cache = None
@@ -495,6 +499,7 @@
         buf = self._d_kept_buf = _grown(self._d_kept_buf, ncols, lambda k: _lib.DeviceArray((k,), np.int32))
         _lib.check(_lib.load().figh_memcpy_h2d(buf.ptr, kept.ctypes.data, kept.nbytes))
         self._fused_kept = (mask.copy(), buf, len(kept))
+        self._base_split = None
 
     PREFIX_SAMPLES = 4096
 
@@ -511,6 +516,77 @@
             return
         self._remember_fused_kept(mask, W.ref_cols)
         self.prefix_passes += 1
+        n = int(np.count_nonzero(mask))
+        if not self._collective() and self.native_tail and n + (self.d_tau is not None) <= 80 and not self._base_only_off:
+            with _lib.null_pivots(0.0):
+                _lib.tsqr_selected(W.buf, (W.rows // self.N) * n0, W.ld, self._d_colsq, W.ref_cols, self.tol_e, 14,
+                                   self._hint_blocks, n, None, self.tol_qr, self._d_sel, self._d_rows)
+            _, _, mask_now, rows_k = self._fetch_pack(W.ref_cols, n, n)
+            if np.array_equal(mask_now, mask):
+                self._learn_base_split(rows_k, n, False, mask, "prefix")
+
+    BASE_COEF_NOISE = 1e-13
+
+    def _learn_base_split(self, rows_k, n, with_tau, mask, source):
+        nc = n + (1 if with_tau else 0)
+        diag = np.abs(rows_k[nc][:n])
+        base, rest = np.flatnonzero(diag > self.tol_qr), np.flatnonzero(~(diag > self.tol_qr))
+        has_tau = self.d_tau is not None
+        if len(rest) == 0 or len(rest) > _lib.BASE_ONLY_MAX_DEP or len(base) == 0 or len(base) + has_tau > 64:
+            self._base_only_off = True
+            return
+        Rb = rows_k[base]
+        R1, R2 = np.triu(Rb[:, base]), Rb[:, rest]
+        try:
+            with _single_threaded_blas(n):
+                bhat = _solve_upper(np.asfortranarray(R1), np.asfortranarray(R2))
+        except np.linalg.LinAlgError:
+            self._base_only_off = True
+            return
+        bhat = np.where((base[:, None] < rest[None, :]) & (np.abs(bhat) > self.BASE_COEF_NOISE), bhat, 0.0)
+        self._base_split = (mask.copy(), np.flatnonzero(mask).astype(np.int32), _lib.BaseTail(base, rest, bhat, has_tau), source)
+
+    def _run_base_only(self, handle, flags, strings, mask, n, with_tau):
+        ex, W = self.exchange, self.W
+        ncols = W.ref_cols
+        _, kept, tail, _ = self._base_split
+        pin = self._landing()
+        total_rows = W.rows * ex.world_size
+        s = tail.s.base
+        s.tol_qr, s.total_rows, s.pieces = self.tol_qr, int(total_rows), self._level0_pieces(total_rows)
+        status = _lib.chain_pass_base_only(handle, flags, self.N, self.d_q, self.d_v, self.d_a, W.buf, W.ld, kept, self.d_tau,
+                                           self.tol_qr, self.tol_e, self._d_pack, pin.array.ctypes.data, 8 * pin.size,
+                                           mask.view(np.uint8), tail)
+        if status is None:
+            self._base_only_off = True
+            return None
+        if status != _lib.PASS_OK:
+            self.base_only_fallbacks += 1
+            return status
+        if s.status == _lib.TAIL_SINGULAR:
+            raise np.linalg.LinAlgError("Singular matrix")
+        self.fused_passes += 1
+        self._n_expected = n
+        idx_e, params_r = self._kept_lists(mask)
+        r = n - tail.nd
+        idx = tail.idx.tolist()
+        idx_base, idx_regroup = idx[:r], idx[r:]
+        beta = tail.beta[:r * tail.nd].reshape(r, tail.nd).copy()
+        out = {
+            "idx_e": idx_e, "params_r": params_r, "idx_base": idx_base, "beta": beta,
+            "col_norm": pin.array[:ncols].copy(), "absdiagR": tail.absdiag.copy(), "rows": total_rows,
+        }
+        if self.null_pivots:
+            out["null_rule_certified"] = True
+        if strings:
+            out["params_base"] = self._expressions_memo(params_r, tail.idx.tobytes() + bytes((r,)), idx_base, idx_regroup, beta)
+        if with_tau:
+            out["phi_b"] = tail.inner.phi_b[:r].copy()
+            out["phi_ls"] = tail.inner.phi_ls[:r].copy()
+            out["residual_norm"] = float(s.residual_norm)
+        with _single_threaded_blas(n):
+            pass
+        return out
 
     def _run_fused(self, handle, flags, strings):
         ex, W = self.exchange, self.W
@@ -520,7 +596,25 @@
         nc = n + (1 if with_tau else 0)
         local = not self._collective()
         if local and self.native_tail and nc <= 80:
-            return self._run_fused_native(handle, flags, strings, mask, d_kept, n, nc, with_tau)
+            split, refused = self._base_split, False
+            if (split is not None and not self._base_only_off and split[2].with_tau == with_tau
+                    and np.array_equal(split[0], mask)):
+                out = self._run_base_only(handle, flags, strings, mask, n, with_tau)
+                if isinstance(out, dict):
+                    return out
+                if out == _lib.PASS_CHANGED:
+                    self._fused_kept = None
+                    return None
+                refused = out == _lib.PASS_NOT_CERTIFIED
+            out = self._run_fused_native(handle, flags, strings, mask, d_kept, n, nc, with_tau)
+            if out is not None and not self._base_only_off and (refused or self._base_split is None
+                                                                or self._base_split[2].with_tau != with_tau):
+                if refused and split[3] == "pass":
+                    self._base_split, self._base_only_off = None, True
+                else:
+                    rows_k = self._landing().array[ncols + self._sel_words:][:(nc + 1) * nc].reshape(nc + 1, nc)
+                    self._learn_base_split(rows_k, n, with_tau, mask, "pass")
+            return out
         if not _lib.regressor_tsqr_fused(handle, flags, self.N, self.d_q, self.d_v, self.d_a, W.buf, W.ld, self._d_colsq,
                                          d_kept, n, self.d_tau, self.tol_qr if local else -1.0,
                                          self._d_rows if local else self._d_R):
diff --git a/include/figh.h b/include/figh.h
--- a/include/figh.h
+++ b/include/figh.h
@@ -28,7 +28,7 @@
 
 typedef struct figh_model_s *figh_model_t;
 
-#define FIGH_ABI_VERSION 113
+#define FIGH_ABI_VERSION 114
 int figh_version(void);
 const char *figh_last_error(void);
 int figh_device_count(int *count);
@@ -120,6 +120,24 @@
                           double *d_W, int64_t ldw, const int32_t *d_kept, int n, const double *d_tau, double tol_qr,
                           double tol_e, double *d_pack, double *h_pack, size_t pack_bytes, const uint8_t *h_kept_mask,
                           int *changed, figh_host_tail_t *tail);
+#define FIGH_BASE_ONLY_MAX_DEP 16
+typedef struct figh_base_tail_s {
+    figh_host_tail_t base;
+    int32_t n, nd;
+    const int32_t *base_pos, *dep_pos;
+    const int32_t *coef_ptr, *coef_idx;
+    const double *coef_val;
+    double *bound;
+    int32_t *idx;
+    double *absdiag;
+    double *beta;
+} figh_base_tail_t;
+int figh_chain_base_tail(figh_base_tail_t *tail);
+enum { FIGH_PASS_OK = 0, FIGH_PASS_CHANGED = 1, FIGH_PASS_NOT_CERTIFIED = 2 };
+int figh_chain_pass_base_only(figh_model_t model, int flags, int64_t N, const double *d_q, const double *d_v,
+                              const double *d_a, double *d_W, int64_t ldw, const int32_t *h_kept, const double *d_tau,
+                              double tol_qr, double tol_e, double *d_pack, double *h_pack, size_t pack_bytes,
+                              const uint8_t *h_kept_mask, int *status, figh_base_tail_t *tail);
 int figh_tsqr_selected_wrench(const double *d_W, int64_t rows, int64_t ldw, const double *d_colsq, int ncols, double tol_e,
                               int link_stride, int n_expected, int nf_expected, const double *d_tau, double tol_qr,
                               int32_t *d_sel, double *d_R_out, const int32_t *d_link_pos, int64_t ld_force);
```

Result: slower. 700.9 million (-2.3%).
